# Mamo1031/Multimodal-MTRSSM

Measured on AMD Instinct MI355X. Metric: seq-steps/s (BxT) MoPoE-MRSSM train step, higher is better.
Workload: dtype bf16x2-split, fp32 accumulate; 1 GPU; BASELINE configs[1]: MoPoE-MRSSM train step, B=64/GPU T=50 deter=200 stoch=30, vision 1x64x64 + audio 1x128x32 + action 4; global_batch=64, seq_len=50, parallelism=dp1, hidden=200, embed=256, categoricals_x_classes=6x5, residual_blocks=3, activation=ELU, optimizer=AdamW lr 1e-3 + clip 10 (fused HIP), params=4151600, streams=1, launch=eager (host enqueues every launch), backend=none, rccl_ranks=0, collective_ranks=0, noise=uniforms keyed by global batch row (parallel.GlobalRowNoise)

## Files before the change

include/mtrssm.h:

```cpp
#ifndef MTRSSM_H
#define MTRSSM_H

#include <stddef.h>
#include <stdint.h>

#ifdef __cplusplus
extern "C" {
#endif

#define MTRSSM_VERSION 100

#define MTRSSM_OK 0
#define MTRSSM_EINVAL (-1)
#define MTRSSM_ELAUNCH (-2)
#define MTRSSM_ELDS (-3)

#define MTRSSM_ACT_IDENTITY 0
#define MTRSSM_ACT_RELU 1
#define MTRSSM_ACT_ELU 2
#define MTRSSM_ACT_TANH 3

int mtrssm_version(void);
const char* mtrssm_last_error(void);
const char* mtrssm_last_kernel(void);
// ... 261 lines not shown
  float* d_lv;
  float* d_lph;
  float* d_lqh;
  const int32_t* modality;
} MtrssmMmtrssmBwdIO;

int mtrssm_mmtrssm_rollout_bwd(const MtrssmMmtrssmDims* dims, const MtrssmMmtrssmBwdWeights* w,
                               const MtrssmMmtrssmBwdIO* io, void* stream);

int mtrssm_mmtrssm_wide_supported(const MtrssmMmtrssmDims* dims, int32_t pieces);
int64_t mtrssm_mmtrssm_wide_workspace_bytes(const MtrssmMmtrssmDims* dims, int32_t pieces);
int64_t mtrssm_mmtrssm_wide_bwd_workspace_bytes(const MtrssmMmtrssmDims* dims, int32_t pieces);
int mtrssm_mmtrssm_rollout_fwd_wide(const MtrssmMmtrssmDims* dims, const MtrssmMmtrssmFwdWeights* w, const MtrssmMmtrssmFwdIO* io,
                                    int32_t pieces, void* workspace, int64_t workspace_bytes, void* stream);
int mtrssm_mmtrssm_rollout_bwd_wide(const MtrssmMmtrssmDims* dims, const MtrssmMmtrssmBwdWeights* w, const MtrssmMmtrssmBwdIO* io,
                                    int32_t pieces, void* workspace, int64_t workspace_bytes, void* stream);

typedef struct MtrssmConvGeom {
  int32_t N;
  int32_t C, Hs, Ws;
  int32_t C2;
  int32_t Cpad;
  int32_t KH, KW;
  int32_t SS, TS, OFFY, OFFX;
  int32_t Hq, Wq;
  int32_t OS, QY, QX;
  int32_t Ho, Wo;
  int32_t Cout, CoutPad;
  int32_t pre_act;
  int32_t act;
  int32_t mfma_split;
} MtrssmConvGeom;

int mtrssm_conv_gather_gemm(const MtrssmConvGeom* g, const float* src, const float* src2, const float* wp, const uint16_t* wq,
                            const float* bias, const float* actgrad_in, const float* add_in, float* out, void* stream);
int mtrssm_conv_gather_gemm_pair(const MtrssmConvGeom* ga, const float* srca, const float* src2a, const float* wpa, const uint16_t* wqa,
                                 const float* biasa, const float* actgrada, const float* adda, float* outa,
                                 const MtrssmConvGeom* gb, const float* srcb, const float* src2b, const float* wpb, const uint16_t* wqb,
                                 const float* biasb, const float* actgradb, const float* addb, float* outb, void* stream);
int mtrssm_conv_gather_pair_merges(const MtrssmConvGeom* ga, const MtrssmConvGeom* gb, int32_t has_wq);
int mtrssm_residual_block_fwd_supported(const MtrssmConvGeom* g3);
int mtrssm_residual_block_fwd(const MtrssmConvGeom* ga, const float* xa, const uint16_t* wq3a, const float* b3a, const float* w1a,
                              const float* b1a, float* ha, float* ya, const MtrssmConvGeom* gb, const float* xb, const uint16_t* wq3b,
                              const float* b3b, const float* w1b, const float* b1b, float* hb, float* yb, void* stream);
int mtrssm_pack_conv_weight(const float* w, int32_t O, int32_t I, int32_t KH, int32_t KW, int64_t so, int64_t si, int64_t sh,
                            int64_t sw, int32_t OPad, int32_t IPad, int32_t pieces, float* wp, uint16_t* wq, void* stream);
#define MTRSSM_PACK_DESC_WORDS 16
int mtrssm_pack_conv_weights(const int64_t* table, int32_t count, int32_t blocks_per_weight, void* stream);
int mtrssm_conv_weight_grad(const MtrssmConvGeom* g, const float* a, const float* src, const float* src2,
                            int32_t pre_act_a, float* dwp, float* dbias, void* workspace, int64_t workspace_bytes, void* stream);
int mtrssm_conv_weight_grad_deferred(const MtrssmConvGeom* g, const float* a, const float* src, const float* src2,
                                     int32_t pre_act_a, float* dwp, float* dbias, void* workspace, int64_t workspace_bytes, void* stream);
int mtrssm_conv_weight_grad_reduce(void* stream);
int64_t mtrssm_conv_weight_grad_workspace_bytes(const MtrssmConvGeom* g, int32_t pre_act_a);
int mtrssm_unpack_conv_grads(const int64_t* table, int32_t count, int32_t blocks_per_entry, void* stream);
int mtrssm_convt_quad_supported(const MtrssmConvGeom* g4);
int mtrssm_convt_quad(const MtrssmConvGeom* ga4, const float* srca, const uint16_t* const* wqa4, const float* biasa, const float* actgrada,
                      float* outa, const MtrssmConvGeom* gb4, const float* srcb, const uint16_t* const* wqb4, const float* biasb,
                      const float* actgradb, float* outb, void* stream);
int mtrssm_convt_k4s2_thin(int32_t N, int32_t C, int32_t Hs, int32_t Ws, int32_t Cout, const float* src, const float* w,
                           const float* bias, int32_t pre_act, int32_t act, float* out, void* stream);
int mtrssm_convt_k4s2_band_supported(int32_t N, int32_t C, int32_t Hs, int32_t Ws, int32_t Cout);
int mtrssm_convt_k4s2_band(int32_t N, int32_t C, int32_t Hs, int32_t Ws, int32_t Cout, const float* src, const float* w,
                           const float* bias, int32_t pre_act, int32_t act, float* out, void* stream);
int mtrssm_conv_tgather_thin(int32_t N, int32_t O, int32_t Hs, int32_t Ws, int32_t Cout, int32_t KH, int32_t KW, int32_t stride, int32_t pad,
                             int32_t Ho, int32_t Wo, const float* y, const float* w, const float* bias, int32_t pre_act, int32_t act,
                             const float* actgrad_in, const float* add_in, float* out, void* stream);
int mtrssm_channel_sum(const float* x, int32_t N, int32_t C, int32_t HW, float* out, void* stream);

int mtrssm_episode_gather(const float* store, const int64_t* idx, const float* noise, int64_t n_episodes, int64_t B, int64_t T,
                          int64_t Tfull, int64_t E, float std_, float* input, float* target, void* stream);
int mtrssm_episode_gather_window(const float* store, const int64_t* idx, const int32_t* start, const float* noise, int64_t n_episodes,
                                 int64_t B, int64_t T, int64_t Tfull, int64_t E, float std_, float* input, float* target, void* stream);

#define MTRSSM_STATE_MAX 6
typedef struct MtrssmStateTable {
  int32_t count;
  int32_t width[MTRSSM_STATE_MAX];
  int64_t src_stride[MTRSSM_STATE_MAX];
  const float* src[MTRSSM_STATE_MAX];
  const float* alt[MTRSSM_STATE_MAX];
  float* dst[MTRSSM_STATE_MAX];
} MtrssmStateTable;
int mtrssm_state_select(const MtrssmStateTable* table, const uint8_t* reset, int64_t B, void* stream);
int mtrssm_state_save(const MtrssmStateTable* table, int64_t B, int64_t steps, void* stream);

int mtrssm_elbo_combine_fwd(const float* nll_a, const float* nll_v, const float* kl0, const float* kl1, int64_t n, float c0, float c1,
                            float* o_recon, float* o_k0, float* o_k1, float* o_loss, void* stream);
int mtrssm_elbo_combine_bwd(const float* g_recon, const float* g_k0, const float* g_k1, const float* g_loss, int64_t n, float c0, float c1,
                            float* g_nll_a, float* g_nll_v, float* g_kl0, float* g_kl1, void* stream);
int mtrssm_categorical_sample_fwd(const float* logits, const float* u, int64_t rows, int32_t K, int32_t C, float* logp, float* probs,
                                  float* onehot, void* stream);
int mtrssm_categorical_sample_bwd(const float* probs, const float* g_probs, const float* g_logp, int64_t rows, int32_t K, int32_t C,
                                  float* d_logits, void* stream);
int mtrssm_gaussian_nll_fwd(const float* pred, const float* target, int64_t frames, int64_t event, int32_t act,
                            float* out, void* stream);
int mtrssm_gaussian_nll_bwd(const float* pred, const float* target, const float* g_out,
                            int64_t frames, int64_t event, int32_t act, float* g_pred, void* stream);

int mtrssm_gaussian_nll_masked_fwd(const float* pred, const float* target, const float* present, const float* count,
                                   int64_t frames, int64_t event, int32_t act, float* out, void* stream);
int mtrssm_gaussian_nll_masked_bwd(const float* pred, const float* target, const float* present, const float* count,
                                   const float* g_out, int64_t frames, int64_t event, int32_t act, float* g_pred, void* stream);

int mtrssm_modality_dropout(const float* u, int64_t b_global, int64_t steps, int64_t span, float p_audio, float p_vision,
                            int64_t row0, int64_t b_local, int32_t* codes, float* present_audio, float* present_vision,
// ... 34 lines not shown
```

multimodal_mtrssm_amd/_lib.py:

```python

from __future__ import annotations

import ctypes as C
import os
from pathlib import Path

import torch
from torch import Tensor

_HERE = Path(__file__).resolve().parent
LIB_PATH = _HERE / "libmtrssm_hip.so"

ACT_IDS = {"Identity": 0, "ReLU": 1, "ELU": 2, "Tanh": 3}

_f = C.c_float
_i = C.c_int32
_p = C.c_void_p


def _struct(name: str, fields: list[tuple[str, type]]) -> type:
    return type(name, (C.Structure,), {"_fields_": fields})


def _ptrs(*names: str) -> list[tuple[str, type]]:
# ... 39 lines not shown
    "sv_l1", "sv_h1", "sv_la", "sv_lv",
    "g_deter_l", "g_deter_h", "g_hidden_l", "g_hidden_h", "g_post_stoch_l", "g_post_stoch_h", "g_prior_stoch_l",
    "g_prior_stoch_h", "g_post_logits_l", "g_post_logits_h", "g_prior_logits_l", "g_prior_logits_h", "g_kl_l", "g_kl_h",
    "g_deter_l0", "g_deter_h0", "g_hidden_l0", "g_hidden_h0", "g_stoch_l0", "g_stoch_h0",
    "d_ul", "d_uh", "d_zl1", "d_zh1", "d_lpl", "d_la", "d_lv", "d_lph", "d_lqh", "modality"))

ConvGeom = _struct("MtrssmConvGeom", [(n, _i) for n in (
    "N", "C", "Hs", "Ws", "C2", "Cpad", "KH", "KW", "SS", "TS", "OFFY", "OFFX", "Hq", "Wq", "OS", "QY", "QX", "Ho", "Wo",
    "Cout", "CoutPad", "pre_act", "act", "mfma_split")])

Gemm = _struct("MtrssmGemm", _ptrs("A", "B", "C", "bias", "zgrad", "colsum") + [(n, _i) for n in (
    "M", "N", "R", "lda", "ldb", "ldc", "ldz", "a_rmajor", "b_rmajor", "act_a", "act_b", "act_out", "act_z", "accumulate", "split_r")]
    + [("tickets", _p), ("n_tickets", _i), ("mfma_split", _i)])

STATE_MAX = 6
StateTable = _struct("MtrssmStateTable", [
    ("count", _i), ("width", _i * STATE_MAX), ("src_stride", C.c_int64 * STATE_MAX), ("src", _p * STATE_MAX), ("alt", _p * STATE_MAX),
    ("dst", _p * STATE_MAX)])

SYMBOLS: dict[str, tuple[type | None, list[type]]] = {
    "mtrssm_version": (C.c_int, []),
    "mtrssm_last_error": (C.c_char_p, []),
    "mtrssm_last_kernel": (C.c_char_p, []),
    "mtrssm_mrssm_rollout_fwd": (C.c_int, [C.POINTER(MrssmDims), C.POINTER(MrssmFwdWeights), C.POINTER(MrssmFwdIO), _p]),
    "mtrssm_mrssm_cluster_supported": (C.c_int, [C.POINTER(MrssmDims)]),
    "mtrssm_mrssm_cluster_workspace_bytes": (C.c_int64, [C.POINTER(MrssmDims)]),
    "mtrssm_mrssm_rollout_fwd_cluster": (C.c_int, [C.POINTER(MrssmDims), C.POINTER(MrssmClusterWeights), C.POINTER(MrssmFwdIO), _p, C.c_int64, _p]),
    "mtrssm_mrssm_cluster_bwd_workspace_bytes": (C.c_int64, [C.POINTER(MrssmDims)]),
    "mtrssm_mrssm_rollout_bwd_cluster": (C.c_int, [C.POINTER(MrssmDims), C.POINTER(MrssmClusterWeights), C.POINTER(MrssmBwdIO), _p, C.c_int64, _p]),
    "mtrssm_mrssm_wide_supported": (C.c_int, [C.POINTER(MrssmDims), _i]),
    "mtrssm_mrssm_wide_workspace_bytes": (C.c_int64, [C.POINTER(MrssmDims), _i]),
    "mtrssm_mrssm_wide_bwd_workspace_bytes": (C.c_int64, [C.POINTER(MrssmDims), _i]),
    "mtrssm_mrssm_rollout_fwd_wide": (C.c_int, [C.POINTER(MrssmDims), C.POINTER(MrssmClusterWeights), C.POINTER(MrssmFwdIO), _i, _p, C.c_int64, _p]),
    "mtrssm_mrssm_rollout_bwd_wide": (C.c_int, [C.POINTER(MrssmDims), C.POINTER(MrssmClusterWeights), C.POINTER(MrssmBwdIO), _i, _p, C.c_int64, _p]),
    "mtrssm_mrssm_rollout_bwd": (C.c_int, [C.POINTER(MrssmDims), C.POINTER(MrssmBwdWeights), C.POINTER(MrssmBwdIO), _p]),
    "mtrssm_mmtrssm_rollout_fwd": (C.c_int, [C.POINTER(MmtrssmDims), C.POINTER(MmtrssmFwdWeights), C.POINTER(MmtrssmFwdIO), _p]),
    "mtrssm_mmtrssm_rollout_bwd": (C.c_int, [C.POINTER(MmtrssmDims), C.POINTER(MmtrssmBwdWeights), C.POINTER(MmtrssmBwdIO), _p]),
    "mtrssm_mmtrssm_wide_supported": (C.c_int, [C.POINTER(MmtrssmDims), _i]),
    "mtrssm_mmtrssm_wide_workspace_bytes": (C.c_int64, [C.POINTER(MmtrssmDims), _i]),
    "mtrssm_mmtrssm_wide_bwd_workspace_bytes": (C.c_int64, [C.POINTER(MmtrssmDims), _i]),
    "mtrssm_mmtrssm_rollout_fwd_wide": (C.c_int, [C.POINTER(MmtrssmDims), C.POINTER(MmtrssmFwdWeights), C.POINTER(MmtrssmFwdIO), _i, _p, C.c_int64, _p]),
    "mtrssm_mmtrssm_rollout_bwd_wide": (C.c_int, [C.POINTER(MmtrssmDims), C.POINTER(MmtrssmBwdWeights), C.POINTER(MmtrssmBwdIO), _i, _p, C.c_int64, _p]),
    "mtrssm_conv_gather_gemm": (C.c_int, [C.POINTER(ConvGeom), _p, _p, _p, _p, _p, _p, _p, _p, _p]),
    "mtrssm_conv_gather_gemm_pair": (C.c_int, [C.POINTER(ConvGeom), _p, _p, _p, _p, _p, _p, _p, _p,
                                               C.POINTER(ConvGeom), _p, _p, _p, _p, _p, _p, _p, _p, _p]),
    "mtrssm_conv_gather_pair_merges": (C.c_int, [C.POINTER(ConvGeom), C.POINTER(ConvGeom), _i]),
    "mtrssm_residual_block_fwd_supported": (C.c_int, [C.POINTER(ConvGeom)]),
    "mtrssm_residual_block_fwd": (C.c_int, [C.POINTER(ConvGeom), _p, _p, _p, _p, _p, _p, _p, C.POINTER(ConvGeom), _p, _p, _p, _p, _p, _p, _p, _p]),
    "mtrssm_pack_conv_weight": (C.c_int, [_p, _i, _i, _i, _i, C.c_int64, C.c_int64, C.c_int64, C.c_int64, _i, _i, _i, _p, _p, _p]),
    "mtrssm_pack_conv_weights": (C.c_int, [_p, _i, _i, _p]),
    "mtrssm_unpack_conv_grads": (C.c_int, [_p, _i, _i, _p]),
    "mtrssm_conv_weight_grad": (C.c_int, [C.POINTER(ConvGeom), _p, _p, _p, _i, _p, _p, _p, C.c_int64, _p]),
    "mtrssm_conv_weight_grad_deferred": (C.c_int, [C.POINTER(ConvGeom), _p, _p, _p, _i, _p, _p, _p, C.c_int64, _p]),
    "mtrssm_conv_weight_grad_reduce": (C.c_int, [_p]),
    "mtrssm_conv_weight_grad_workspace_bytes": (C.c_int64, [C.POINTER(ConvGeom), _i]),
    "mtrssm_channel_sum": (C.c_int, [_p, _i, _i, _i, _p, _p]),
    "mtrssm_convt_k4s2_thin": (C.c_int, [_i, _i, _i, _i, _i, _p, _p, _p, _i, _i, _p, _p]),
    "mtrssm_convt_k4s2_band_supported": (C.c_int, [_i, _i, _i, _i, _i]),
    "mtrssm_convt_k4s2_band": (C.c_int, [_i, _i, _i, _i, _i, _p, _p, _p, _i, _i, _p, _p]),
    "mtrssm_convt_quad_supported": (C.c_int, [C.POINTER(ConvGeom)]),
    "mtrssm_convt_quad": (C.c_int, [C.POINTER(ConvGeom), _p, C.POINTER(C.c_void_p), _p, _p, _p, C.POINTER(ConvGeom), _p, C.POINTER(C.c_void_p),
                                    _p, _p, _p, _p]),
    "mtrssm_conv_tgather_thin": (C.c_int, [_i] * 11 + [_p, _p, _p, _i, _i, _p, _p, _p, _p]),
    "mtrssm_episode_gather": (C.c_int, [_p, _p, _p, C.c_int64, C.c_int64, C.c_int64, C.c_int64, C.c_int64, _f, _p, _p, _p]),
    "mtrssm_episode_gather_window": (C.c_int, [_p, _p, _p, _p, C.c_int64, C.c_int64, C.c_int64, C.c_int64, C.c_int64, _f, _p, _p, _p]),
    "mtrssm_state_select": (C.c_int, [C.POINTER(StateTable), _p, C.c_int64, _p]),
    "mtrssm_state_save": (C.c_int, [C.POINTER(StateTable), C.c_int64, C.c_int64, _p]),
    "mtrssm_elbo_combine_fwd": (C.c_int, [_p, _p, _p, _p, C.c_int64, C.c_float, C.c_float, _p, _p, _p, _p, _p]),
    "mtrssm_elbo_combine_bwd": (C.c_int, [_p, _p, _p, _p, C.c_int64, C.c_float, C.c_float, _p, _p, _p, _p, _p]),
    "mtrssm_categorical_sample_fwd": (C.c_int, [_p, _p, C.c_int64, _i, _i, _p, _p, _p, _p]),
    "mtrssm_categorical_sample_bwd": (C.c_int, [_p, _p, _p, C.c_int64, _i, _i, _p, _p]),
    "mtrssm_gaussian_nll_fwd": (C.c_int, [_p, _p, C.c_int64, C.c_int64, _i, _p, _p]),
    "mtrssm_gaussian_nll_bwd": (C.c_int, [_p, _p, _p, C.c_int64, C.c_int64, _i, _p, _p]),
    "mtrssm_gaussian_nll_masked_fwd": (C.c_int, [_p, _p, _p, _p, C.c_int64, C.c_int64, _i, _p, _p]),
    "mtrssm_gaussian_nll_masked_bwd": (C.c_int, [_p, _p, _p, _p, _p, C.c_int64, C.c_int64, _i, _p, _p]),
    "mtrssm_modality_dropout": (C.c_int, [_p, C.c_int64, C.c_int64, C.c_int64, _f, _f, C.c_int64, C.c_int64, _p, _p, _p, _p, _p, _p]),
    "mtrssm_sumsq": (C.c_int, [_p, C.c_int64, _p, _p]),
    "mtrssm_adamw_step": (C.c_int, [_p, _p, _p, _p, C.c_int64, _p, _f, _f, _f, _f, _f, _f, _f, _i, _p]),
    "mtrssm_gemm": (C.c_int, [C.POINTER(Gemm), _p]),
    "mtrssm_gemm_group": (C.c_int, [C.POINTER(Gemm), _i, _p]),
    "mtrssm_clear": (C.c_int, [_p, C.c_int64, _p]),
    "mtrssm_adamw_prepare": (C.c_int, [_p, C.c_int64, _p, _p, _p, _f, _f, _p]),
    "mtrssm_adamw_apply": (C.c_int, [_p, _p, _p, _p, _p, C.c_int64, _p, _p, _p, _f, _f, _f, _f, _f, _f, _p]),
}

_LIB: C.CDLL | None = None


class MtrssmLibraryError(RuntimeError):
    """The HIP library is missing or a kernel call failed.  There is no fallback path."""


def load() -> C.CDLL:
    global _LIB
    if _LIB is not None:
        return _LIB
    path = Path(os.environ.get("MTRSSM_LIB", LIB_PATH))
    if not path.exists():
        msg = (f"{path} not found: build it with `make -C multimodal_mtrssm_amd/csrc` (or __graft_entry__.build()). "
               "multimodal_mtrssm_amd has no CPU or eager fallback for the rollout path.")
        raise MtrssmLibraryError(msg)
    lib = C.CDLL(str(path))
    for name, (res, args) in SYMBOLS.items():
        fn = getattr(lib, name)
        fn.restype = res
        fn.argtypes = args
# ... 99 lines not shown
```

multimodal_mtrssm_amd/conv.py:

```python

from __future__ import annotations

import ctypes as C
import os
import weakref

import torch
from torch import Tensor

from multimodal_mtrssm_amd import _lib
from multimodal_mtrssm_amd.linear import grad_target, grad_target_owner


def _pad_to(n: int, m: int) -> int:
    return (n + m - 1) // m * m


def _pads(cout: int, cin: int) -> tuple[int, int]:
    return _pad_to(cout, 64 if cout > 32 else 32), _pad_to(cin, 16)


_PACK_BUFFERS: dict[tuple, tuple[Tensor, Tensor | None]] = {}

PAIR_LAUNCH = os.environ.get("MTRSSM_PAIR_LAUNCH", "1") != "0"
# ... 413 lines not shown
        _PLAN.pinned += 1


def unpin_scratch() -> None:
    _PLAN.pinned = max(0, _PLAN.pinned - 1)


_WGRAD_WS: dict[tuple, Tensor] = {}
_WGRAD_WS_RETIRED: list[Tensor] = []
_WGRAD_NEED: dict[tuple, int] = {}


DEFER_WGRAD_REDUCE = os.environ.get("MTRSSM_DEFER_WGRAD_REDUCE", "1") != "0"
_WGRAD_SLOTS: dict[tuple, list[Tensor]] = {}
_WGRAD_SLOT_NEXT: dict[tuple, int] = {}


def _reduce_deferred() -> None:
    for (device, stream), used in list(_WGRAD_SLOT_NEXT.items()):
        if used:
            _WGRAD_SLOT_NEXT[(device, stream)] = 0
            _lib.check(_lib.TIMERS.call("mtrssm_conv_weight_grad_reduce", _lib.load().mtrssm_conv_weight_grad_reduce, C.c_void_p(stream)),
                       "mtrssm_conv_weight_grad_reduce")


def _wgrad_workspace(geom: C.Structure, pre_act_a: int, device: torch.device, *, own: bool = False) -> Tensor | None:
    gkey = (tuple(getattr(geom, n) for n, _ in geom._fields_), pre_act_a)
    need = _WGRAD_NEED.get(gkey)
    if need is None:
        need = _WGRAD_NEED[gkey] = max(0, int(_lib.load().mtrssm_conv_weight_grad_workspace_bytes(C.byref(geom), pre_act_a)))
    if need == 0:
        return None
    key = (device, torch.cuda.current_stream(device).cuda_stream)
    if own:
        slots = _WGRAD_SLOTS.setdefault(key, [])
        k = _WGRAD_SLOT_NEXT.get(key, 0)
        _WGRAD_SLOT_NEXT[key] = k + 1
        if k == len(slots):
            slots.append(torch.empty((need + 3) // 4 + 64, device=device, dtype=torch.float32))
        elif slots[k].numel() * 4 < need:
            _WGRAD_WS_RETIRED.append(slots[k])
            slots[k] = torch.empty((need + 3) // 4 + 64, device=device, dtype=torch.float32)
        return slots[k]
    ws = _WGRAD_WS.get(key)
    if ws is None or ws.numel() * 4 < need:
        if ws is not None:
            _WGRAD_WS_RETIRED.append(ws)
        ws = _WGRAD_WS[key] = torch.empty((need + 3) // 4 + 64, device=device, dtype=torch.float32)
    return ws


def _weight_grad(a: Tensor, src: Tensor, coords: Tensor | None, kh: int, kw: int, stride: int, pad: int, pre_act_a: bool,
                 pre_act_src: bool, act: int, *, want_bias: bool = False, weight: Tensor | None = None,
                 bias: Tensor | None = None) -> tuple[Tensor | None, Tensor | None]:
    lib = _lib.load()
    n, o, hq, wq = a.shape
    _, c, hs, ws = src.shape
    c2 = 0 if coords is None else coords.shape[0]
    opad, ipad = _pads(o, c + c2)
    sunk = _GRAD_SINK.target(weight, o, c + c2, kh * kw, opad, ipad)
    dwp = sunk if sunk is not None else _zeros(opad * kh * kw * ipad, a.device).view(opad, kh * kw, ipad)
    dbias = bias_sunk = None
    if want_bias:
        bias_sunk = grad_target(bias) if bias is not None and bias.is_contiguous() else None
        dbias = bias_sunk if bias_sunk is not None else _zeros(o, a.device)
    geom = _geom(N=n, C=c, Hs=hs, Ws=ws, C2=c2, Cpad=ipad, KH=kh, KW=kw, SS=stride, TS=1, OFFY=-pad, OFFX=-pad, Hq=hq, Wq=wq,
                 OS=1, QY=0, QX=0, Ho=hq, Wo=wq, Cout=o, CoutPad=opad, pre_act=int(pre_act_src), act=act)
    flops = 2.0 * n * hq * wq * o * kh * kw * (c + c2)
    nbytes = 4.0 * (a.numel() + src.numel())
    defer = DEFER_WGRAD_REDUCE and sunk is not None and (not want_bias or bias_sunk is not None)
    ws = _wgrad_workspace(geom, int(pre_act_a), a.device, own=defer)
    entry = lib.mtrssm_conv_weight_grad_deferred if defer and ws is not None else lib.mtrssm_conv_weight_grad
    _lib.check(_lib.TIMERS.call(
        "mtrssm_conv_weight_grad", entry, C.byref(geom), _lib.ptr(a), _lib.ptr(src), _lib.ptr(coords),
        int(pre_act_a), _lib.ptr(dwp), _lib.ptr(dbias), _lib.raw_ptr(ws), 0 if ws is None else ws.numel() * 4, _lib.stream_ptr(a.device),
        flops=flops, nbytes=nbytes), "mtrssm_conv_weight_grad")
    g_w = None if sunk is not None else dwp[:o, :, : c + c2].reshape(o, kh, kw, c + c2).permute(0, 3, 1, 2)
    return g_w, (None if bias_sunk is not None else dbias)


def _channel_sum(x: Tensor, bias: Tensor | None = None) -> Tensor | None:
    lib = _lib.load()
    n, c, h, w = x.shape
    sunk = grad_target(bias) if bias is not None and bias.is_contiguous() else None
    out = sunk if sunk is not None else _zeros(c, x.device)
    _lib.check(_lib.TIMERS.call("mtrssm_channel_sum", lib.mtrssm_channel_sum, _lib.ptr(x), n, c, h * w, _lib.ptr(out),
                                _lib.stream_ptr(x.device)), "mtrssm_channel_sum")
    return None if sunk is not None else out


class _Conv2d(torch.autograd.Function):
    @staticmethod
    def forward(ctx, x, weight, bias, coords, stride, pad, pre_act, act):
        x, weight = x.contiguous(), weight.contiguous()
        bias = None if bias is None else bias.contiguous()
        coords = None if coords is None else coords.contiguous()
        out = _conv_forward_gather(x, coords, weight, bias, stride, pad, pre_act, act)
        ctx.save_for_backward(x, weight, coords if coords is not None else x.new_zeros(0))
        ctx.cfg = (stride, pad, pre_act, act, coords is not None, bias is not None)
        ctx.bias = bias
        return out

    @staticmethod
    def backward(ctx, g_out):
        x, weight, coords = ctx.saved_tensors
        stride, pad, pre_act, act, has_coords, has_bias = ctx.cfg
        coords = coords if has_coords else None
        g_out = g_out.contiguous()
        kh, kw = weight.shape[2:]
        c = x.shape[1]
        g_x = None
        if ctx.needs_input_grad[0]:
            g_x = _conv_transposed_gather(g_out, weight[:, :c], None, stride, pad, (x.shape[2], x.shape[3]), False, act,
                                          actgrad_in=x if pre_act else None)
        g_w = g_b = None
        want_b = has_bias and ctx.needs_input_grad[2]
        if ctx.needs_input_grad[1]:
            g_w, g_b = _weight_grad(g_out, x, coords, kh, kw, stride, pad, False, pre_act, act, want_bias=want_b, weight=weight,
                                    bias=ctx.bias)
        elif want_b:
            g_b = _channel_sum(g_out, ctx.bias)
        return g_x, g_w, g_b, None, None, None, None, None


class _ConvTranspose2d(torch.autograd.Function):
    @staticmethod
    def forward(ctx, x, weight, bias, stride, pad, out_pad, pre_act, act):
        x, weight = x.contiguous(), weight.contiguous()
        bias = None if bias is None else bias.contiguous()
        kh, kw = weight.shape[2:]
        ho = (x.shape[2] - 1) * stride - 2 * pad + kh + out_pad
        wo = (x.shape[3] - 1) * stride - 2 * pad + kw + out_pad
        out = _conv_transposed_gather(x, weight, bias, stride, pad, (ho, wo), pre_act, act)
        ctx.save_for_backward(x, weight)
        ctx.cfg = (stride, pad, pre_act, act, bias is not None)
        ctx.bias = bias
        return out

    @staticmethod
    def backward(ctx, g_out):
        x, weight = ctx.saved_tensors
        stride, pad, pre_act, act, has_bias = ctx.cfg
        g_out = g_out.contiguous()
        kh, kw = weight.shape[2:]
        g_x = None
        if ctx.needs_input_grad[0]:
            g_x = _conv_forward_gather(g_out, None, weight, None, stride, pad, False, act, actgrad_in=x if pre_act else None)
        g_w = None
        if ctx.needs_input_grad[1]:
            g_w, _ = _weight_grad(x, g_out, None, kh, kw, stride, pad, pre_act, False, act, weight=weight)
        g_b = _channel_sum(g_out, ctx.bias) if has_bias and ctx.needs_input_grad[2] else None
        return g_x, g_w, g_b, None, None, None, None, None


RESBLOCK_FUSE = True


def _residual_job(x: Tensor, w3: Tensor, b3: Tensor, w1: Tensor, b1: Tensor, act: int, sub: int = 0) -> tuple | None:
    if not RESBLOCK_FUSE or w3.shape[2:] != (3, 3) or w1.shape[2:] != (1, 1) or w1.shape[:2] != (x.shape[1], w3.shape[0]):
        return None
    n, c, hs, ws = x.shape
    o = w3.shape[0]
    wp, wq = pack_weight(w3, sub)
    if wq is None:
        return None
    geom = _geom(N=n, C=c, Hs=hs, Ws=ws, C2=0, Cpad=wp.shape[2], KH=3, KW=3, SS=1, TS=1, OFFY=-1, OFFX=-1, Hq=hs, Wq=ws, OS=1, QY=0,
                 QX=0, Ho=hs, Wo=ws, Cout=o, CoutPad=wp.shape[0], pre_act=1, act=act)
    if not _lib.load().mtrssm_residual_block_fwd_supported(C.byref(geom)):
        return None
    h = torch.empty(n, o, hs, ws, device=x.device, dtype=torch.float32)
    return (geom, x, wq, b3, w1, b1, h, torch.empty_like(x))


def _residual_launch(ja: tuple, jb: tuple | None) -> None:
    def work(job: tuple) -> tuple[float, float]:
        g = job[0]
        pixels = g.N * g.Hq * g.Wq
        return 2.0 * pixels * g.Cout * (9 * g.C + g.C), 4.0 * pixels * (2 * g.C + g.Cout)

    def args(job: tuple | None) -> tuple:
        if job is None:
            return (None,) * 8
        geom, x, wq, b3, w1, b1, h, y = job
        return (C.byref(geom), _lib.ptr(x), _lib.raw_ptr(wq), _lib.ptr(b3), _lib.ptr(w1), _lib.ptr(b1), _lib.ptr(h), _lib.ptr(y))

    fa, ba = work(ja)
    fb, bb = work(jb) if jb is not None else (0.0, 0.0)
    lib = _lib.load()
    _lib.check(_lib.TIMERS.call("mtrssm_residual_block_fwd", lib.mtrssm_residual_block_fwd, *args(ja), *args(jb),
                                _lib.stream_ptr(ja[1].device), flops=fa + fb, nbytes=ba + bb), "mtrssm_residual_block_fwd")


class _ResidualBlock(torch.autograd.Function):

    @staticmethod
    def forward(ctx, x, w3, b3, w1, b1, act):
        x, w3, b3, w1, b1 = (t.contiguous() for t in (x, w3, b3, w1, b1))
        p3, p1 = w3.shape[2] // 2, w1.shape[2] // 2
        job = _residual_job(x, w3, b3, w1, b1, act)
        if job is not None:
            _residual_launch(job, None)
            h, y = job[6], job[7]
        else:
            h = _conv_forward_gather(x, None, w3, b3, 1, p3, True, act)
            y = _conv_forward_gather(h, None, w1, b1, 1, p1, True, act, add_in=x)
        ctx.save_for_backward(x, h, w3, w1)
        ctx.act, ctx.biases = act, (b3, b1)
        return y

    @staticmethod
    def backward(ctx, g_y):
        x, h, w3, w1 = ctx.saved_tensors
        act = ctx.act
        g_y = g_y.contiguous()
        p3, p1 = w3.shape[2] // 2, w1.shape[2] // 2
        g_h = _conv_transposed_gather(g_y, w1, None, 1, p1, (h.shape[2], h.shape[3]), False, act, actgrad_in=h)
        b3, b1 = ctx.biases
        g_w1, g_b1 = _weight_grad(g_y, h, None, w1.shape[2], w1.shape[3], 1, p1, False, True, act, want_bias=True, weight=w1, bias=b1)
        g_x = None
        if ctx.needs_input_grad[0]:
            g_x = _conv_transposed_gather(g_h, w3, None, 1, p3, (x.shape[2], x.shape[3]), False, act, actgrad_in=x, add_in=g_y)
        g_w3, g_b3 = _weight_grad(g_h, x, None, w3.shape[2], w3.shape[3], 1, p3, False, True, act, want_bias=True, weight=w3, bias=b3)
        return g_x, g_w3, g_b3, g_w1, g_b1, None


class _PairResidualBlock(torch.autograd.Function):

    @staticmethod
    def forward(ctx, xa, w3a, b3a, w1a, b1a, xv, w3v, b3v, w1v, b1v, act):
        xa, w3a, b3a, w1a, b1a, xv, w3v, b3v, w1v, b1v = (t.contiguous() for t in (xa, w3a, b3a, w1a, b1a, xv, w3v, b3v, w1v, b1v))
        p3, p1 = w3a.shape[2] // 2, w1a.shape[2] // 2
        ja = _residual_job(xa, w3a, b3a, w1a, b1a, act)
        jv = _residual_job(xv, w3v, b3v, w1v, b1v, act, sub=1) if ja is not None else None
        if ja is not None and jv is not None:
            _residual_launch(ja, jv)
            ha, ya, hv, yv = ja[6], ja[7], jv[6], jv[7]
        else:
            ha, hv = paired(lambda: _conv_forward_gather(xa, None, w3a, b3a, 1, p3, True, act),
                            lambda: _conv_forward_gather(xv, None, w3v, b3v, 1, p3, True, act))
            ya, yv = paired(lambda: _conv_forward_gather(ha, None, w1a, b1a, 1, p1, True, act, add_in=xa),
                            lambda: _conv_forward_gather(hv, None, w1v, b1v, 1, p1, True, act, add_in=xv))
        ctx.save_for_backward(xa, ha, w3a, w1a, xv, hv, w3v, w1v)
        ctx.act, ctx.biases = act, (b3a, b1a, b3v, b1v)
        return ya, yv

    @staticmethod
    def backward(ctx, g_ya, g_yv):
        xa, ha, w3a, w1a, xv, hv, w3v, w1v = ctx.saved_tensors
        act = ctx.act
        g_ya, g_yv = g_ya.contiguous(), g_yv.contiguous()
        p3, p1 = w3a.shape[2] // 2, w1a.shape[2] // 2
        g_ha, g_hv = paired(lambda: _conv_transposed_gather(g_ya, w1a, None, 1, p1, (ha.shape[2], ha.shape[3]), False, act, actgrad_in=ha),
                            lambda: _conv_transposed_gather(g_yv, w1v, None, 1, p1, (hv.shape[2], hv.shape[3]), False, act, actgrad_in=hv))
        b3a, b1a, b3v, b1v = ctx.biases
        g_w1a, g_b1a = _weight_grad(g_ya, ha, None, w1a.shape[2], w1a.shape[3], 1, p1, False, True, act, want_bias=True, weight=w1a, bias=b1a)
        g_w1v, g_b1v = _weight_grad(g_yv, hv, None, w1v.shape[2], w1v.shape[3], 1, p1, False, True, act, want_bias=True, weight=w1v, bias=b1v)
        g_xa, g_xv = paired(
            lambda: _conv_transposed_gather(g_ha, w3a, None, 1, p3, (xa.shape[2], xa.shape[3]), False, act, actgrad_in=xa, add_in=g_ya),
            lambda: _conv_transposed_gather(g_hv, w3v, None, 1, p3, (xv.shape[2], xv.shape[3]), False, act, actgrad_in=xv, add_in=g_yv))
        g_w3a, g_b3a = _weight_grad(g_ha, xa, None, w3a.shape[2], w3a.shape[3], 1, p3, False, True, act, want_bias=True, weight=w3a, bias=b3a)
        g_w3v, g_b3v = _weight_grad(g_hv, xv, None, w3v.shape[2], w3v.shape[3], 1, p3, False, True, act, want_bias=True, weight=w3v, bias=b3v)
        return g_xa, g_w3a, g_b3a, g_w1a, g_b1a, g_xv, g_w3v, g_b3v, g_w1v, g_b1v, None


def residual_block_pair(xa: Tensor, pa: tuple[Tensor, Tensor, Tensor, Tensor], xv: Tensor, pv: tuple[Tensor, Tensor, Tensor, Tensor],
                        *, act: int) -> tuple[Tensor, Tensor]:
    return _PairResidualBlock.apply(xa, *pa, xv, *pv, int(act))


def residual_block(x: Tensor, w3: Tensor, b3: Tensor, w1: Tensor, b1: Tensor, *, act: int) -> Tensor:
    return _ResidualBlock.apply(x, w3, b3, w1, b1, int(act))


class _BranchCtx:

    def __init__(self, needs: tuple = ()) -> None:
        self.needs_input_grad = needs
        self.saved_tensors: tuple = ()
        self.cfg: tuple = ()

    def save_for_backward(self, *tensors: Tensor) -> None:
        self.saved_tensors = tensors


def _pair_function(base: type) -> type:

    class _Pair(torch.autograd.Function):
        @staticmethod
        def forward(ctx, n, *args):
            ca, cb = _BranchCtx(), _BranchCtx()
            ya, yb = paired(lambda: base.forward(ca, *args[:n]), lambda: base.forward(cb, *args[n:]))
            ctx.n, ctx.na, ctx.cfgs = n, len(ca.saved_tensors), (ca.cfg, cb.cfg)
            ctx.biases = (getattr(ca, "bias", None), getattr(cb, "bias", None))
            ctx.save_for_backward(*ca.saved_tensors, *cb.saved_tensors)
            return ya, yb

        @staticmethod
        def backward(ctx, ga, gb):
            saved, needs = ctx.saved_tensors, ctx.needs_input_grad[1:]
            ca, cb = _BranchCtx(needs[: ctx.n]), _BranchCtx(needs[ctx.n :])
            ca.saved_tensors, cb.saved_tensors = saved[: ctx.na], saved[ctx.na :]
            ca.cfg, cb.cfg = ctx.cfgs
            ca.bias, cb.bias = ctx.biases
            ra, rb = paired(lambda: base.backward(ca, ga), lambda: base.backward(cb, gb))
            return (None, *ra, *rb)

    _Pair.__name__ = f"_Pair{base.__name__}"
    return _Pair

# ... 26 lines not shown
```

multimodal_mtrssm_amd/csrc/capi.hip:

```cpp
#include <stdarg.h>
#include <stdio.h>

#include "scan_common.h"

namespace mtrssm {

static thread_local char g_err[512] = "";
static thread_local const char* g_kernel = "";

void set_last_kernel(const char* name) { g_kernel = name; }

void set_error(const char* fmt, ...) {
  va_list ap;
  va_start(ap, fmt);
  vsnprintf(g_err, sizeof(g_err), fmt, ap);
  va_end(ap);
}

int mrssm_fwd_launch(const MtrssmMrssmDims*, const MtrssmMrssmFwdWeights*, const MtrssmMrssmFwdIO*, hipStream_t);
int mrssm_bwd_launch(const MtrssmMrssmDims*, const MtrssmMrssmBwdWeights*, const MtrssmMrssmBwdIO*, hipStream_t);
int mmtrssm_fwd_launch(const MtrssmMmtrssmDims*, const MtrssmMmtrssmFwdWeights*, const MtrssmMmtrssmFwdIO*, hipStream_t);
int mmtrssm_bwd_launch(const MtrssmMmtrssmDims*, const MtrssmMmtrssmBwdWeights*, const MtrssmMmtrssmBwdIO*, hipStream_t);
int conv_gather_gemm_launch(const MtrssmConvGeom*, const float*, const float*, const float*, const unsigned short*, const float*, const float*, const float*, float*, hipStream_t);
int episode_gather_launch(const float*, const int64_t*, const float*, int64_t, int64_t, int64_t, int64_t, int64_t, float, float*, float*, hipStream_t);
int episode_gather_window_launch(const float*, const int64_t*, const int32_t*, const float*, int64_t, int64_t, int64_t, int64_t, int64_t, float, float*,
                                 float*, hipStream_t);
int state_select_launch(const MtrssmStateTable*, const unsigned char*, int64_t, hipStream_t);
int state_save_launch(const MtrssmStateTable*, int64_t, int64_t, hipStream_t);
int conv_gather_gemm_pair_launch(const MtrssmConvGeom*, const float*, const float*, const float*, const unsigned short*, const float*, const float*, const float*, float*,
                                 const MtrssmConvGeom*, const float*, const float*, const float*, const unsigned short*, const float*, const float*, const float*, float*, hipStream_t);
int conv_residual_fwd_supported(const MtrssmConvGeom*);
int conv_residual_fwd_launch(const MtrssmConvGeom*, const float*, const unsigned short*, const float*, const float*, const float*, float*, float*,
                             const MtrssmConvGeom*, const float*, const unsigned short*, const float*, const float*, const float*, float*, float*, hipStream_t);
int pack_conv_weight_launch(const float*, int, int, int, int, long, long, long, long, int, int, int, float*, unsigned short*, hipStream_t);
int pack_conv_weights_launch(const int64_t*, int, int, hipStream_t);
int conv_gather_pair_merges(const MtrssmConvGeom*, const MtrssmConvGeom*, bool);
int conv_weight_grad_launch(const MtrssmConvGeom*, const float*, const float*, const float*, int, float*, float*, void*, size_t, size_t*, hipStream_t);
int conv_weight_grad_deferred_launch(const MtrssmConvGeom*, const float*, const float*, const float*, int, float*, float*, void*, size_t, hipStream_t);
int conv_weight_grad_reduce_flush(hipStream_t);
int channel_sum_launch(const float*, int, int, int, float*, hipStream_t);
int convt_k4s2_band_supported(int, int, int, int, int);
int convt_k4s2_band_launch(int, int, int, int, int, const float*, const float*, const float*, int, int, float*, hipStream_t);
int convt_k4s2_thin_launch(int, int, int, int, int, const float*, const float*, const float*, int, int, float*, hipStream_t);
int conv_convt_quad_supported(const MtrssmConvGeom*);
int conv_convt_quad_launch(const MtrssmConvGeom*, const float*, const unsigned short* const*, const float*, const float*, float*,
                           const MtrssmConvGeom*, const float*, const unsigned short* const*, const float*, const float*, float*, hipStream_t);
int conv_tgather_thin_launch(int, int, int, int, int, int, int, int, int, int, int, const float*, const float*, const float*, int, int, const float*,
                             const float*, float*, hipStream_t);
int categorical_sample_fwd_launch(const float*, const float*, int64_t, int, int, float*, float*, float*, hipStream_t);
int categorical_sample_bwd_launch(const float*, const float*, const float*, int64_t, int, int, float*, hipStream_t);
int elbo_combine_fwd_launch(const float*, const float*, const float*, const float*, int64_t, float, float, float*, float*, float*, float*, hipStream_t);
int elbo_combine_bwd_launch(const float*, const float*, const float*, const float*, int64_t, float, float, float*, float*, float*, float*, hipStream_t);
int nll_fwd_launch(const float*, const float*, int64_t, int64_t, int, float*, hipStream_t);
int nll_bwd_launch(const float*, const float*, const float*, int64_t, int64_t, int, float*, hipStream_t);
int nll_masked_fwd_launch(const float*, const float*, const float*, const float*, int64_t, int64_t, int, float*, hipStream_t);
int nll_masked_bwd_launch(const float*, const float*, const float*, const float*, const float*, int64_t, int64_t, int, float*, hipStream_t);
int modality_dropout_launch(const float*, int64_t, int64_t, int64_t, float, float, int64_t, int64_t, int32_t*, float*, float*, unsigned char*, float*,
                            hipStream_t);
int sumsq_launch(const float*, int64_t, float*, hipStream_t);
int adamw_launch(float*, const float*, float*, float*, int64_t, const float*, float, float, float, float, float, float, float, int, hipStream_t);
int gemm_launch(const MtrssmGemm*, hipStream_t);
int gemm_group_launch(const MtrssmGemm*, int, hipStream_t);
int debug_set_cluster_profile(void*);
int debug_set_resident_profile(void*);
int debug_set_wide_profile(void*);
int debug_set_mmt_profile(void*);
int mrssm_cluster_supported(const MtrssmMrssmDims*);
size_t mrssm_cluster_workspace_bytes(const MtrssmMrssmDims*);
size_t mrssm_cluster_bwd_workspace_bytes(const MtrssmMrssmDims*);
int mrssm_bwd_cluster_launch(const MtrssmMrssmDims*, const MtrssmMrssmClusterWeights*, const MtrssmMrssmBwdIO*, void*, size_t, hipStream_t);
int mrssm_fwd_cluster_launch(const MtrssmMrssmDims*, const MtrssmMrssmClusterWeights*, const MtrssmMrssmFwdIO*, void*, size_t, hipStream_t);
int unpack_conv_grads_launch(const int64_t*, int, int, hipStream_t);
int mrssm_wide_supported(const MtrssmMrssmDims*, int);
size_t mrssm_wide_workspace_bytes(const MtrssmMrssmDims*, int);
size_t mrssm_wide_bwd_workspace_bytes(const MtrssmMrssmDims*, int);
int mrssm_wide_fwd_launch(const MtrssmMrssmDims*, const MtrssmMrssmClusterWeights*, const MtrssmMrssmFwdIO*, int, void*, size_t, hipStream_t);
int mrssm_wide_bwd_launch(const MtrssmMrssmDims*, const MtrssmMrssmClusterWeights*, const MtrssmMrssmBwdIO*, int, void*, size_t, hipStream_t);
int adamw_prepare_launch(const float*, int64_t, float*, float*, const int*, float, float, hipStream_t);
int adamw_apply_launch(float*, const float*, float*, float*, const unsigned char*, int64_t, const float*, const float*, const int*, float, float, float,
                       float, float, float, hipStream_t);

int mmtrssm_wide_supported(const MtrssmMmtrssmDims*, int);
size_t mmtrssm_wide_workspace_bytes(const MtrssmMmtrssmDims*, int);
size_t mmtrssm_wide_bwd_workspace_bytes(const MtrssmMmtrssmDims*, int);
int mmtrssm_wide_fwd_launch(const MtrssmMmtrssmDims*, const MtrssmMmtrssmFwdWeights*, const MtrssmMmtrssmFwdIO*, int, void*, size_t, hipStream_t);
int mmtrssm_wide_bwd_launch(const MtrssmMmtrssmDims*, const MtrssmMmtrssmBwdWeights*, const MtrssmMmtrssmBwdIO*, int, void*, size_t, hipStream_t);

int device_cu_count() {
  static int cached[64] = {0};
  int dev = 0;
  if (hipGetDevice(&dev) != hipSuccess) { (void)hipGetLastError(); return 0; }
  if (dev < 0 || dev >= 64) return 0;
// ... 133 lines not shown
                            weight_decay, static_cast<hipStream_t>(stream));
}
MTRSSM_API int mtrssm_conv_gather_gemm(const MtrssmConvGeom* g, const float* src, const float* src2, const float* wp, const uint16_t* wq,
                                       const float* bias, const float* actgrad_in, const float* add_in, float* out, void* stream) {
  return conv_gather_gemm_launch(g, src, src2, wp, wq, bias, actgrad_in, add_in, out, static_cast<hipStream_t>(stream));
}
MTRSSM_API int mtrssm_episode_gather(const float* store, const int64_t* idx, const float* noise, int64_t n_episodes, int64_t B, int64_t T,
                                     int64_t Tfull, int64_t E, float std_, float* input, float* target, void* stream) {
  return episode_gather_launch(store, idx, noise, n_episodes, B, T, Tfull, E, std_, input, target, static_cast<hipStream_t>(stream));
}
MTRSSM_API int mtrssm_episode_gather_window(const float* store, const int64_t* idx, const int32_t* start, const float* noise, int64_t n_episodes,
                                            int64_t B, int64_t T, int64_t Tfull, int64_t E, float std_, float* input, float* target, void* stream) {
  return episode_gather_window_launch(store, idx, start, noise, n_episodes, B, T, Tfull, E, std_, input, target, static_cast<hipStream_t>(stream));
}
MTRSSM_API int mtrssm_state_select(const MtrssmStateTable* table, const uint8_t* reset, int64_t B, void* stream) {
  return state_select_launch(table, reset, B, static_cast<hipStream_t>(stream));
}
MTRSSM_API int mtrssm_state_save(const MtrssmStateTable* table, int64_t B, int64_t steps, void* stream) {
  return state_save_launch(table, B, steps, static_cast<hipStream_t>(stream));
}
MTRSSM_API int mtrssm_conv_gather_gemm_pair(const MtrssmConvGeom* ga, const float* srca, const float* src2a, const float* wpa, const uint16_t* wqa,
                                            const float* biasa, const float* actgrada, const float* adda, float* outa,
                                            const MtrssmConvGeom* gb, const float* srcb, const float* src2b, const float* wpb, const uint16_t* wqb,
                                            const float* biasb, const float* actgradb, const float* addb, float* outb, void* stream) {
  return conv_gather_gemm_pair_launch(ga, srca, src2a, wpa, wqa, biasa, actgrada, adda, outa, gb, srcb, src2b, wpb, wqb, biasb, actgradb, addb,
                                      outb, static_cast<hipStream_t>(stream));
}
MTRSSM_API int mtrssm_residual_block_fwd_supported(const MtrssmConvGeom* g3) { return conv_residual_fwd_supported(g3) != 0; }
MTRSSM_API int mtrssm_residual_block_fwd(const MtrssmConvGeom* ga, const float* xa, const uint16_t* wq3a, const float* b3a, const float* w1a,
                                         const float* b1a, float* ha, float* ya, const MtrssmConvGeom* gb, const float* xb, const uint16_t* wq3b,
                                         const float* b3b, const float* w1b, const float* b1b, float* hb, float* yb, void* stream) {
  return conv_residual_fwd_launch(ga, xa, wq3a, b3a, w1a, b1a, ha, ya, gb, xb, wq3b, b3b, w1b, b1b, hb, yb, static_cast<hipStream_t>(stream));
}
MTRSSM_API int mtrssm_pack_conv_weight(const float* w, int32_t O, int32_t I, int32_t KH, int32_t KW, int64_t so, int64_t si, int64_t sh,
                                       int64_t sw, int32_t OPad, int32_t IPad, int32_t pieces, float* wp, uint16_t* wq, void* stream) {
  return pack_conv_weight_launch(w, O, I, KH, KW, so, si, sh, sw, OPad, IPad, pieces, wp, wq, static_cast<hipStream_t>(stream));
}
MTRSSM_API int mtrssm_conv_gather_pair_merges(const MtrssmConvGeom* ga, const MtrssmConvGeom* gb, int32_t has_wq) {
  return conv_gather_pair_merges(ga, gb, has_wq != 0);
}
MTRSSM_API int mtrssm_pack_conv_weights(const int64_t* table, int32_t count, int32_t blocks_per_weight, void* stream) {
  return pack_conv_weights_launch(table, count, blocks_per_weight, static_cast<hipStream_t>(stream));
}
MTRSSM_API int mtrssm_conv_weight_grad(const MtrssmConvGeom* g, const float* a, const float* src, const float* src2, int32_t pre_act_a,
                                       float* dwp, float* dbias, void* workspace, int64_t workspace_bytes, void* stream) {
  return conv_weight_grad_launch(g, a, src, src2, pre_act_a, dwp, dbias, workspace, workspace_bytes < 0 ? 0 : (size_t)workspace_bytes, nullptr,
                                 static_cast<hipStream_t>(stream));
}
MTRSSM_API int mtrssm_conv_weight_grad_deferred(const MtrssmConvGeom* g, const float* a, const float* src, const float* src2, int32_t pre_act_a,
                                               float* dwp, float* dbias, void* workspace, int64_t workspace_bytes, void* stream) {
  return conv_weight_grad_deferred_launch(g, a, src, src2, pre_act_a, dwp, dbias, workspace, workspace_bytes < 0 ? 0 : (size_t)workspace_bytes,
                                          static_cast<hipStream_t>(stream));
}
MTRSSM_API int mtrssm_conv_weight_grad_reduce(void* stream) { return conv_weight_grad_reduce_flush(static_cast<hipStream_t>(stream)); }
MTRSSM_API int64_t mtrssm_conv_weight_grad_workspace_bytes(const MtrssmConvGeom* g, int32_t pre_act_a) {
  size_t need = 0;
  if (conv_weight_grad_launch(g, nullptr, nullptr, nullptr, pre_act_a, nullptr, nullptr, nullptr, 0, &need, nullptr) != MTRSSM_OK) return -1;
  return (int64_t)need;
}
MTRSSM_API int mtrssm_channel_sum(const float* x, int32_t N, int32_t C, int32_t HW, float* out, void* stream) {
  return channel_sum_launch(x, N, C, HW, out, static_cast<hipStream_t>(stream));
}
MTRSSM_API int mtrssm_conv_tgather_thin(int32_t N, int32_t O, int32_t Hs, int32_t Ws, int32_t Cout, int32_t KH, int32_t KW, int32_t stride,
                                        int32_t pad, int32_t Ho, int32_t Wo, const float* y, const float* w, const float* bias, int32_t pre_act,
                                        int32_t act, const float* actgrad_in, const float* add_in, float* out, void* stream) {
  return conv_tgather_thin_launch(N, O, Hs, Ws, Cout, KH, KW, stride, pad, Ho, Wo, y, w, bias, pre_act, act, actgrad_in, add_in, out,
                                  static_cast<hipStream_t>(stream));
}
MTRSSM_API int mtrssm_convt_quad_supported(const MtrssmConvGeom* g4) { return conv_convt_quad_supported(g4); }
MTRSSM_API int mtrssm_convt_quad(const MtrssmConvGeom* ga4, const float* srca, const uint16_t* const* wqa4, const float* biasa,
                                 const float* actgrada, float* outa, const MtrssmConvGeom* gb4, const float* srcb,
                                 const uint16_t* const* wqb4, const float* biasb, const float* actgradb, float* outb, void* stream) {
  return conv_convt_quad_launch(ga4, srca, reinterpret_cast<const unsigned short* const*>(wqa4), biasa, actgrada, outa, gb4, srcb,
                                reinterpret_cast<const unsigned short* const*>(wqb4), biasb, actgradb, outb,
                                static_cast<hipStream_t>(stream));
}
MTRSSM_API int mtrssm_convt_k4s2_band_supported(int32_t N, int32_t C, int32_t Hs, int32_t Ws, int32_t Cout) {
  return convt_k4s2_band_supported(N, C, Hs, Ws, Cout);
}
MTRSSM_API int mtrssm_convt_k4s2_band(int32_t N, int32_t C, int32_t Hs, int32_t Ws, int32_t Cout, const float* src, const float* w,
                                     const float* bias, int32_t pre_act, int32_t act, float* out, void* stream) {
  return convt_k4s2_band_launch(N, C, Hs, Ws, Cout, src, w, bias, pre_act, act, out, static_cast<hipStream_t>(stream));
}
MTRSSM_API int mtrssm_convt_k4s2_thin(int32_t N, int32_t C, int32_t Hs, int32_t Ws, int32_t Cout, const float* src, const float* w,
                                      const float* bias, int32_t pre_act, int32_t act, float* out, void* stream) {
  return convt_k4s2_thin_launch(N, C, Hs, Ws, Cout, src, w, bias, pre_act, act, out, static_cast<hipStream_t>(stream));
}
```

multimodal_mtrssm_amd/csrc/conv.hip:

```cpp
#include <map>
#include <mutex>
#include <unordered_map>
#include <utility>

#include "scan_common.h"

namespace mtrssm {

void set_error(const char* fmt, ...);
void set_last_kernel(const char* name);

using f32x16 = __attribute__((ext_vector_type(16))) float;

constexpr int kKC = 16;
constexpr int kTP = 128;
constexpr int kConvThreads = 256;

__device__ __forceinline__ float act_grad_from_in(float x, int act) {
  switch (act) {
    case MTRSSM_ACT_RELU: return x > 0.f ? 1.f : 0.f;
    case MTRSSM_ACT_ELU: return x > 0.f ? 1.f : expf(x);
    case MTRSSM_ACT_TANH: { const float t = tanhf(x); return 1.f - t * t; }
    default: return 1.f;
  }
// ... 534 lines not shown
      const int n = (int)(pe / plane_q);
      const int rem = (int)(pe - (long)n * plane_q);
      const int oy = rem / g.Wq, ox = rem - oy * g.Wq;
      const size_t plane_o = (size_t)g.Ho * g.Wo;
      const size_t base = (size_t)n * g.Cout * plane_o + (size_t)(oy * g.OS + g.QY) * g.Wo + (ox * g.OS + g.QX);
#pragma unroll
      for (int j = 0; j < NT; ++j) {
#pragma unroll
        for (int r = 0; r < 16; ++r) {
          const int co = co0 + j * 32 + (r & 3) + 8 * (r >> 2) + 4 * kl;
          if (co < g.Cout) {
            float v = acc[i][j][r] + (bias ? bias[co] : 0.f);
            const size_t o = base + (size_t)co * plane_o;
            if (actgrad_in) v *= act_grad_from_in(actgrad_in[o], g.act);
            if (add_in) v += add_in[o];
            out[o] = v;
          }
        }
      }
    }
  }
}

}
#include "conv_split.h"
#include "conv_resident.h"
#include "conv_s2_band.h"
#include "conv_wgrad_resident.h"

namespace mtrssm {

static int launched(const char* who);
enum ReduceVariant { kRedRes64, kRedRes32, kRed1x1_64, kRed1x1_128, kRedThin, kRedThinT, kRedS2, kRedT4, kRedT4b, kRedS2c };
struct ReduceJob {
  const float4* part;
  float* dwp;
  float* dbias;
  int S, cpad, variant, gx, gy;
  __host__ int variant_gy() const { return gy; }
};
constexpr int kReduceBatchMax = 48;
struct ReduceBatch {
  int count;
  int first[kReduceBatchMax + 1];
  ReduceJob job[kReduceBatchMax];
};
__device__ __forceinline__ void wgrad_reduce_dispatch(const ReduceJob& j, int bx, int by) {
  switch (j.variant) {
    case kRedRes64: wgrad_reduce_partials_body<64>(j.part, j.S, j.cpad, j.dwp, j.dbias, bx, by); break;
    case kRedRes32: wgrad_reduce_partials_body<32>(j.part, j.S, j.cpad, j.dwp, j.dbias, bx, by); break;
    case kRed1x1_64: wgrad_reduce_partials1x1_body<64>(j.part, j.S, j.cpad, j.dwp, j.dbias, bx, by); break;
    case kRed1x1_128: wgrad_reduce_partials1x1_body<128>(j.part, j.S, j.cpad, j.dwp, j.dbias, bx, by); break;
    case kRedThin: wgrad_reduce_partials_thin_body(j.part, j.S, j.cpad, j.dwp, j.dbias, bx, by); break;
    case kRedThinT: wgrad_reduce_partials_thint_body(j.part, j.S, j.cpad, j.dwp, bx, by); break;
    case kRedS2: wgrad_reduce_partials_s2_body(j.part, j.S, j.cpad, j.dwp, j.dbias, bx, by); break;
    case kRedT4: wgrad_reduce_partials_t4_body(j.part, j.S, j.cpad, j.dwp, bx, by); break;
    case kRedT4b: wgrad_reduce_partials_t4b_body(j.part, j.S, j.cpad, j.dwp, bx, by); break;
    default: wgrad_reduce_partials_s2c_body(j.part, j.S, j.cpad, j.dwp, j.dbias, bx, by); break;
  }
}
__global__ __launch_bounds__(256) void wgrad_reduce_batch_kernel(const ReduceBatch b) {
  int j = 0;
  while (j + 1 < b.count && (int)blockIdx.x >= b.first[j + 1]) ++j;
  const int lb = (int)blockIdx.x - b.first[j], gx = b.job[j].gx;
  wgrad_reduce_dispatch(b.job[j], lb % gx, lb / gx);
}

static thread_local bool tl_defer_reduce = false;
static std::mutex g_reduce_mutex;
static std::map<std::pair<int, hipStream_t>, std::vector<ReduceJob>> g_reduce_jobs;
static std::pair<int, hipStream_t> reduce_key(hipStream_t stream) {
  int dev = 0;
  (void)hipGetDevice(&dev);
  return {dev, stream};
}

static int reduce_flush_locked(std::vector<ReduceJob>& jobs, hipStream_t stream) {
  size_t at = 0;
  while (at < jobs.size()) {
    ReduceBatch b{};
    int blocks = 0;
    while (at < jobs.size() && b.count < kReduceBatchMax) {
      b.first[b.count] = blocks;
      b.job[b.count] = jobs[at];
      blocks += jobs[at].gx * jobs[at].variant_gy();
      ++b.count;
      ++at;
    }
    b.first[b.count] = blocks;
    set_last_kernel("mtrssm::wgrad_reduce_batch_kernel");
    hipLaunchKernelGGL(wgrad_reduce_batch_kernel, dim3((unsigned)blocks), dim3(256), 0, stream, b);
  }
  jobs.clear();
  return launched("conv_weight_grad_reduce");
}

int conv_weight_grad_reduce_flush(hipStream_t stream) {
  std::lock_guard<std::mutex> lock(g_reduce_mutex);
  auto it = g_reduce_jobs.find(reduce_key(stream));
  if (it == g_reduce_jobs.end() || it->second.empty()) return MTRSSM_OK;
  return reduce_flush_locked(it->second, stream);
}

static int reduce_now_or_later(int variant, dim3 rgrid, const float* part, int S, int cpad, float* dwp, float* dbias, hipStream_t stream) {
  ReduceJob j{reinterpret_cast<const float4*>(part), dwp, dbias, S, cpad, variant, (int)rgrid.x, (int)rgrid.y};
  if (tl_defer_reduce) {
    std::lock_guard<std::mutex> lock(g_reduce_mutex);
    auto& jobs = g_reduce_jobs[reduce_key(stream)];
    for (const ReduceJob& o : jobs)
      if (o.dwp == dwp || o.part == j.part) {
// ... 1057 lines not shown
    GatherProblem p{};
    p.g = *g; p.src = x; p.wq = wq; p.bias = b3; p.out = h; p.w1 = w1; p.b1 = b1; p.out2 = y;
    p.nx = g->N;
    return p;
  };
  const GatherProblem pa = problem(ga, xa, wq3a, b3a, w1a, b1a, ha, ya);
  GatherProblem none{};
  none.nx = 0;
  if (!gb) return residual_fwd_one_grid(pa, none, ka, stream);
  const GatherProblem pb = problem(gb, xb, wq3b, b3b, w1b, b1b, hb, yb);
  if (ka == kb) return residual_fwd_one_grid(pa, pb, ka, stream);
  if (int rc = residual_fwd_one_grid(pa, none, ka, stream)) return rc;
  return residual_fwd_one_grid(pb, none, kb, stream);
}

int channel_sum_launch(const float* x, int N, int C, int HW, float* out, hipStream_t stream);

static bool wgrad_resident_enabled() {
  static const bool on = [] { const char* e = getenv("MTRSSM_WGRAD_RESIDENT"); return !(e && e[0] == '0'); }();
  return on;
}
static bool wgrad_resident_c32() {
  static const bool on = [] { const char* e = getenv("MTRSSM_WGRAD_RESIDENT_C32"); return !(e && e[0] == '0'); }();
  return on;
}
static bool wgrad_1x1_staged_enabled() {
  static const bool on = [] { const char* e = getenv("MTRSSM_WGRAD_1X1_STAGED"); return !(e && e[0] == '0'); }();
  return on;
}
static bool wgrad_s2_staged_enabled() {
  static const bool on = [] { const char* e = getenv("MTRSSM_WGRAD_S2_STAGED"); return !(e && e[0] == '0'); }();
  return on;
}
static bool wgrad_partials_enabled() {
  static const bool on = [] { const char* e = getenv("MTRSSM_WGRAD_PARTIALS"); return !(e && e[0] == '0'); }();
  return on;
}
#define MTRSSM_WGRAD_PART(bytes_expr)                                                                                              \
  float* part = nullptr;                                                                                                         \
  {                                                                                                                              \
    const size_t need_ = (bytes_expr);                                                                                           \
    if (query) { *query = wgrad_partials_enabled() ? need_ : 0; return MTRSSM_OK; }                                              \
    if (wgrad_partials_enabled() && workspace && workspace_bytes >= need_) part = static_cast<float*>(workspace);                \
  }
#define MTRSSM_WGRAD_NO_PART \
  if (query) { *query = 0; return MTRSSM_OK; }
static bool no_direct_wgrad() {
  static const bool off = getenv("MTRSSM_NO_DIRECT_WGRAD") != nullptr;
  return off;
}

int conv_weight_grad_launch(const MtrssmConvGeom* g, const float* a, const float* src, const float* src2, int pre_act_a,
                            float* dwp, float* dbias, void* workspace, size_t workspace_bytes, size_t* query, hipStream_t stream);
int conv_weight_grad_deferred_launch(const MtrssmConvGeom* g, const float* a, const float* src, const float* src2, int pre_act_a,
                                     float* dwp, float* dbias, void* workspace, size_t workspace_bytes, hipStream_t stream) {
  tl_defer_reduce = true;
  const int rc = conv_weight_grad_launch(g, a, src, src2, pre_act_a, dwp, dbias, workspace, workspace_bytes, nullptr, stream);
  tl_defer_reduce = false;
  return rc;
}

int conv_weight_grad_launch(const MtrssmConvGeom* g, const float* a, const float* src, const float* src2, int pre_act_a,
                            float* dwp, float* dbias, void* workspace, size_t workspace_bytes, size_t* query, hipStream_t stream) {
  if (int rc = check_geom(g, "conv_weight_grad")) return rc;
  if (!query && (!a || !src || !dwp || (g->C2 > 0 && !src2))) { set_error("conv_weight_grad: null pointer"); return MTRSSM_EINVAL; }
  if (workspace && ((uintptr_t)workspace & 255)) { set_error("conv_weight_grad: workspace must be 256-byte aligned"); return MTRSSM_EINVAL; }
  if (dbias && pre_act_a) { set_error("conv_weight_grad: the fused bias gradient sums the RAW a tensor; pass dbias only with pre_act_a = 0"); return MTRSSM_EINVAL; }
  if (g->OS != 1 || g->QY != 0 || g->QX != 0 || g->KH * g->KW <= 0) { set_error("conv_weight_grad: needs a plain (OS=1) geometry with taps"); return MTRSSM_EINVAL; }
  const long ptot = (long)g->N * g->Hq * g->Wq;
  const int taps = g->KH * g->KW;
  const int ctot = g->C + g->C2;
  if ((g->mfma_split == 1 || g->mfma_split == 2) && taps == 1 && g->SS == 1 && g->OFFY == 0 && g->OFFX == 0 && g->C2 == 0 && g->Hs == g->Hq &&
      g->Ws == g->Wq && g->Hq * g->Wq == 64 && (g->C == 64 || g->C == 128) && g->Cout % 64 == 0 && g->Cout <= 65535 * 64 && g->Cpad >= g->C &&
      !pre_act_a && (g->act == MTRSSM_ACT_IDENTITY || g->act == MTRSSM_ACT_ELU || g->act == MTRSSM_ACT_RELU) && !((uintptr_t)a & 15) &&
      !((uintptr_t)src & 15) && wgrad_1x1_staged_enabled()) {
    const int cogroups = g->Cout / 64;
    int wgs = cu_count() / cogroups;
    if (wgs < 1) wgs = 1;
    if (wgs > g->N) wgs = g->N;
    const int per = (g->N + wgs - 1) / wgs;
    const dim3 grid((unsigned)((g->N + per - 1) / per), cogroups);
    MTRSSM_WGRAD_PART((size_t)grid.x * cogroups * kWg1x1SetFloats * sizeof(float))
#define MTRSSM_WG1_LAUNCH(SP_, C_)                                                                                              \
  {                                                                                                                             \
    static bool attr_done_dev[64] = {}; bool& attr_done = attr_done_dev[device_slot()];        \
    constexpr int lds_b = wg1x1_lds_bytes<SP_, C_>();                                                                           \
    if (!attr_done) {                                                                                                           \
      (void)hipFuncSetAttribute(reinterpret_cast<const void*>(conv1x1_wgrad_staged_kernel<SP_, C_>),                            \
                                hipFuncAttributeMaxDynamicSharedMemorySize, lds_b);                                             \
      attr_done = true;                                                                                                         \
    }                                                                                                                           \
    set_last_kernel("mtrssm::conv1x1_wgrad_staged_kernel<" #SP_ ", " #C_ ">");                                                  \
    hipLaunchKernelGGL((conv1x1_wgrad_staged_kernel<SP_, C_>), grid, dim3(512), lds_b, stream, *g, a, src, dwp, part, dbias,    \
                       per);                                                                                                    \
  }
    const int sp = g->mfma_split;
    if (g->C == 64) { if (sp == 2) MTRSSM_WG1_LAUNCH(2, 64) else MTRSSM_WG1_LAUNCH(1, 64) }
    else { if (sp == 2) MTRSSM_WG1_LAUNCH(2, 128) else MTRSSM_WG1_LAUNCH(1, 128) }
#undef MTRSSM_WG1_LAUNCH
    if (part) {
      const dim3 rgrid((unsigned)(2 * (g->C / 32) * 256 / 32 + (dbias ? 1 : 0)), cogroups);
      if (int rc = reduce_now_or_later(g->C == 64 ? kRed1x1_64 : kRed1x1_128, rgrid, part, (int)grid.x, g->Cpad, dwp, dbias, stream)) return rc;
    }
    return launched("conv_weight_grad(1x1 staged)");
  }
  if (g->mfma_split >= 1 && taps == 1 && g->SS == 1 && g->OFFY == 0 && g->OFFX == 0 && g->C2 == 0 && g->Hs == g->Hq && g->Ws == g->Wq &&
      (g->Hq * g->Wq) % 16 == 0 && g->Cout <= 128 && g->C <= 128 && g->C >= 8 && !((uintptr_t)a & 15) && !((uintptr_t)src & 15) &&
      ptot < (1L << 31)) {
    MTRSSM_WGRAD_NO_PART
    const int tiles_co = (g->Cout + 31) / 32, tiles_ci = (g->C + 31) / 32;
    const int total = (int)(ptot / 16);
    int splits = 256;
    if (splits > total) splits = total;
    const int per = (total + splits - 1) / splits;
    const dim3 grid((unsigned)((total + per - 1) / per));
    const dim3 block(64 * tiles_co * tiles_ci);
// ... 58 lines not shown
    if (splits > total) splits = total;
    const int per = (total + splits - 1) / splits;
    const dim3 grid((unsigned)((total + per - 1) / per), cogroups);
    const dim3 block(64 * nt);
    const int sp = g->mfma_split;
#define MTRSSM_W33_LAUNCH(SP_, W_)                                                                                               \
  {                                                                                                                             \
    set_last_kernel("mtrssm::conv3x3_weight_grad_split_kernel<" #SP_ ", " #W_ ">");                                              \
    hipLaunchKernelGGL((conv3x3_weight_grad_split_kernel<SP_, W_>), grid, block, 0, stream, *g, a, src, pre_act_a, dwp, dbias, tiles_ci, per); \
  }
    if (g->Wq == 8) { if (sp == 3) MTRSSM_W33_LAUNCH(3, 8) else if (sp == 2) MTRSSM_W33_LAUNCH(2, 8) else MTRSSM_W33_LAUNCH(1, 8) }
    else { if (sp == 3) MTRSSM_W33_LAUNCH(3, 4) else if (sp == 2) MTRSSM_W33_LAUNCH(2, 4) else MTRSSM_W33_LAUNCH(1, 4) }
#undef MTRSSM_W33_LAUNCH
    return launched("conv_weight_grad(3x3 split)");
  }
  if ((g->mfma_split == 1 || g->mfma_split == 2) && g->KH == 3 && g->KW == 3 && g->SS == 2 && g->TS == 1 && g->OFFY == -1 && g->OFFX == -1 &&
      g->C == 1 && g->C2 == 2 && g->Cout == 8 && g->Hq * g->Wq == 1024 && (g->Wq == 32 || g->Wq == 16) && g->Hs == 2 * g->Hq && g->Ws == 2 * g->Wq &&
      g->Cpad >= 3 && !pre_act_a && (g->act == MTRSSM_ACT_IDENTITY || g->act == MTRSSM_ACT_ELU || g->act == MTRSSM_ACT_RELU || !g->pre_act) &&
      !((uintptr_t)a & 15) && !((uintptr_t)src & 15) && !((uintptr_t)src2 & 15) && wgrad_s2_staged_enabled()) {
    int wgs = cu_count();
    if (wgs > g->N) wgs = g->N;
    const int per = (g->N + wgs - 1) / wgs;
    const dim3 grid((unsigned)((g->N + per - 1) / per));
    MTRSSM_WGRAD_PART((size_t)grid.x * kWgThinSetFloats * sizeof(float))
#define MTRSSM_WGTHIN_LAUNCH(SP_, W_)                                                                                            \
  {                                                                                                                             \
    static bool attr_done_dev[64] = {}; bool& attr_done = attr_done_dev[device_slot()];        \
    constexpr int lds_b = wgthin_lds_bytes<SP_, W_>();                                                                          \
    if (!attr_done) {                                                                                                           \
      (void)hipFuncSetAttribute(reinterpret_cast<const void*>(conv3x3s2_thin_wgrad_staged_kernel<SP_, W_>),                      \
                                hipFuncAttributeMaxDynamicSharedMemorySize, lds_b);                                             \
      attr_done = true;                                                                                                         \
    }                                                                                                                           \
    set_last_kernel("mtrssm::conv3x3s2_thin_wgrad_staged_kernel<" #SP_ ", " #W_ ">");                                            \
    hipLaunchKernelGGL((conv3x3s2_thin_wgrad_staged_kernel<SP_, W_>), grid, dim3(512), lds_b, stream, *g, a, src, src2, dwp,     \
                       part, dbias, per);                                                                                       \
  }
    const int sp = g->mfma_split;
    if (g->Wq == 32) { if (sp == 2) MTRSSM_WGTHIN_LAUNCH(2, 32) else MTRSSM_WGTHIN_LAUNCH(1, 32) }
    else { if (sp == 2) MTRSSM_WGTHIN_LAUNCH(2, 16) else MTRSSM_WGTHIN_LAUNCH(1, 16) }
#undef MTRSSM_WGTHIN_LAUNCH
    if (part)
      if (int rc = reduce_now_or_later(kRedThin, dim3(dbias ? 9 : 8), part, (int)grid.x, g->Cpad, dwp, dbias, stream)) return rc;
    return launched("conv_weight_grad(3x3 s2 thin staged)");
  }
  if ((g->mfma_split == 1 || g->mfma_split == 2) && g->KH == 4 && g->KW == 4 && g->SS == 2 && g->TS == 1 && g->OFFY == -1 && g->OFFX == -1 &&
      g->C == 1 && g->C2 == 0 && g->Cout == 16 && g->Hq * g->Wq == 1024 && (g->Wq == 32 || g->Wq == 16) && g->Hs == 2 * g->Hq && g->Ws == 2 * g->Wq &&
      g->Cpad >= 1 && !g->pre_act && !dbias && (g->act == MTRSSM_ACT_IDENTITY || g->act == MTRSSM_ACT_ELU || g->act == MTRSSM_ACT_RELU || !pre_act_a) &&
      !((uintptr_t)a & 15) && !((uintptr_t)src & 15) && wgrad_s2_staged_enabled()) {
    int wgs = cu_count();
    if (wgs > g->N) wgs = g->N;
    const int per = (g->N + wgs - 1) / wgs;
    const dim3 grid((unsigned)((g->N + per - 1) / per));
    MTRSSM_WGRAD_PART((size_t)grid.x * kWgThinTSetFloats * sizeof(float))
#define MTRSSM_WGTHINT_LAUNCH(SP_, W_)                                                                                           \
  {                                                                                                                             \
    static bool attr_done_dev[64] = {}; bool& attr_done = attr_done_dev[device_slot()];        \
    constexpr int lds_b = wgthint_lds_bytes<SP_, W_>();                                                                         \
    if (!attr_done) {                                                                                                           \
      (void)hipFuncSetAttribute(reinterpret_cast<const void*>(convt4s2_thin_wgrad_staged_kernel<SP_, W_>),                       \
                                hipFuncAttributeMaxDynamicSharedMemorySize, lds_b);                                             \
      attr_done = true;                                                                                                         \
    }                                                                                                                           \
    set_last_kernel("mtrssm::convt4s2_thin_wgrad_staged_kernel<" #SP_ ", " #W_ ">");                                             \
    hipLaunchKernelGGL((convt4s2_thin_wgrad_staged_kernel<SP_, W_>), grid, dim3(512), lds_b, stream, *g, a, src, pre_act_a, dwp, \
                       part, per);                                                                                              \
  }
    const int sp = g->mfma_split;
    if (g->Wq == 32) { if (sp == 2) MTRSSM_WGTHINT_LAUNCH(2, 32) else MTRSSM_WGTHINT_LAUNCH(1, 32) }
    else { if (sp == 2) MTRSSM_WGTHINT_LAUNCH(2, 16) else MTRSSM_WGTHINT_LAUNCH(1, 16) }
#undef MTRSSM_WGTHINT_LAUNCH
    if (part)
      if (int rc = reduce_now_or_later(kRedThinT, dim3(16), part, (int)grid.x, g->Cpad, dwp, nullptr, stream)) return rc;
    return launched("conv_weight_grad(k4 s2 thin staged)");
  }
  if (g->mfma_split >= 1 && g->Cout <= 32 && taps * ctot <= 32 && g->Wq >= 8 && (g->Wq & (g->Wq - 1)) == 0 && (g->Hq * g->Wq) % 16 == 0 &&
      !((uintptr_t)a & 15) && ptot < (1L << 31) && (long)g->N * g->C * g->Hs * g->Ws < (1L << 40) && !no_direct_wgrad()) {
    MTRSSM_WGRAD_NO_PART
    int log2_wq = 0;
    while ((1 << log2_wq) < g->Wq) ++log2_wq;
    const int total = (int)(ptot / 16);
    int waves = 4096;
    if (waves > total) waves = total;
    const int per = (total + waves - 1) / waves;
    waves = (total + per - 1) / per;
    const dim3 grid((unsigned)((waves + 15) / 16));
    const int sp = g->mfma_split;
    set_last_kernel(sp == 3 ? "mtrssm::conv_weight_grad_thin_split_kernel<3>" : sp == 2 ? "mtrssm::conv_weight_grad_thin_split_kernel<2>" : "mtrssm::conv_weight_grad_thin_split_kernel<1>");
    if (sp == 3) hipLaunchKernelGGL((conv_weight_grad_thin_split_kernel<3>), grid, dim3(1024), 0, stream, *g, a, src, src2, pre_act_a, dwp, dbias, per, log2_wq);
    else if (sp == 2) hipLaunchKernelGGL((conv_weight_grad_thin_split_kernel<2>), grid, dim3(1024), 0, stream, *g, a, src, src2, pre_act_a, dwp, dbias, per, log2_wq);
    else hipLaunchKernelGGL((conv_weight_grad_thin_split_kernel<1>), grid, dim3(1024), 0, stream, *g, a, src, src2, pre_act_a, dwp, dbias, per, log2_wq);
    return launched("conv_weight_grad(thin split)");
  }
  if ((g->mfma_split == 1 || g->mfma_split == 2) && g->KH == 3 && g->KW == 3 && g->SS == 2 && g->TS == 1 && g->OFFY == -1 && g->OFFX == -1 &&
      g->C2 == 0 && g->C == 8 && g->Cout == 16 && g->Hq * g->Wq == 256 && (g->Wq == 16 || g->Wq == 8) && g->Hs == 2 * g->Hq && g->Ws == 2 * g->Wq &&
      g->Cpad >= 8 && !pre_act_a && (g->act == MTRSSM_ACT_IDENTITY || g->act == MTRSSM_ACT_ELU || g->act == MTRSSM_ACT_RELU) &&
      !((uintptr_t)a & 15) && !((uintptr_t)src & 15) && wgrad_s2_staged_enabled()) {
    int wgs = cu_count();
    if (wgs > g->N) wgs = g->N;
    const int per = (g->N + wgs - 1) / wgs;
    const dim3 grid((unsigned)((g->N + per - 1) / per));
    MTRSSM_WGRAD_PART((size_t)grid.x * kWgS2SetFloats * sizeof(float))
#define MTRSSM_WGS2_LAUNCH(SP_, W_)                                                                                              \
  {                                                                                                                             \
    static bool attr_done_dev[64] = {}; bool& attr_done = attr_done_dev[device_slot()];        \
    constexpr int lds_b = wgs2_lds_bytes<SP_, W_>();                                                                            \
    if (!attr_done) {                                                                                                           \
      (void)hipFuncSetAttribute(reinterpret_cast<const void*>(conv3x3s2_wgrad_staged_kernel<SP_, W_>),                           \
                                hipFuncAttributeMaxDynamicSharedMemorySize, lds_b);                                             \
      attr_done = true;                                                                                                         \
    }                                                                                                                           \
    set_last_kernel("mtrssm::conv3x3s2_wgrad_staged_kernel<" #SP_ ", " #W_ ">");                                                 \
    hipLaunchKernelGGL((conv3x3s2_wgrad_staged_kernel<SP_, W_>), grid, dim3(512), lds_b, stream, *g, a, src, dwp, part, dbias,   \
                       per);                                                                                                    \
  }
    const int sp = g->mfma_split;
    if (g->Wq == 16) { if (sp == 2) MTRSSM_WGS2_LAUNCH(2, 16) else MTRSSM_WGS2_LAUNCH(1, 16) }
    else { if (sp == 2) MTRSSM_WGS2_LAUNCH(2, 8) else MTRSSM_WGS2_LAUNCH(1, 8) }
#undef MTRSSM_WGS2_LAUNCH
    if (part)
      if (int rc = reduce_now_or_later(kRedS2, dim3(dbias ? 49 : 48), part, (int)grid.x, g->Cpad, dwp, dbias, stream)) return rc;
    return launched("conv_weight_grad(3x3 s2 staged)");
  }
  if ((g->mfma_split == 1 || g->mfma_split == 2) && g->KH == 4 && g->KW == 4 && g->SS == 2 && g->TS == 1 && g->OFFY == -1 && g->OFFX == -1 &&
      g->C2 == 0 && g->C == 16 && g->Cout == 32 && g->Hq * g->Wq == 256 && (g->Wq == 16 || g->Wq == 8) && g->Hs == 2 * g->Hq && g->Ws == 2 * g->Wq &&
      g->Cpad >= 16 && !g->pre_act && !dbias && (g->act == MTRSSM_ACT_IDENTITY || g->act == MTRSSM_ACT_ELU || g->act == MTRSSM_ACT_RELU || !pre_act_a) &&
      !((uintptr_t)a & 15) && !((uintptr_t)src & 15) && wgrad_s2_staged_enabled()) {
    int wgs = cu_count();
    if (wgs > g->N) wgs = g->N;
    const int per = (g->N + wgs - 1) / wgs;
    const dim3 grid((unsigned)((g->N + per - 1) / per));
    MTRSSM_WGRAD_PART((size_t)grid.x * kWgT4SetFloats * sizeof(float))
#define MTRSSM_WGT4_LAUNCH(SP_, W_)                                                                                              \
  {                                                                                                                             \
    static bool attr_done_dev[64] = {}; bool& attr_done = attr_done_dev[device_slot()];        \
    constexpr int lds_b = wgt4_lds_bytes<SP_, W_>();                                                                            \
    if (!attr_done) {                                                                                                           \
      (void)hipFuncSetAttribute(reinterpret_cast<const void*>(convt4s2_wgrad_staged_kernel<SP_, W_>),                            \
                                hipFuncAttributeMaxDynamicSharedMemorySize, lds_b);                                             \
      attr_done = true;                                                                                                         \
    }                                                                                                                           \
    set_last_kernel("mtrssm::convt4s2_wgrad_staged_kernel<" #SP_ ", " #W_ ">");                                                  \
    hipLaunchKernelGGL((convt4s2_wgrad_staged_kernel<SP_, W_>), grid, dim3(512), lds_b, stream, *g, a, src, pre_act_a, dwp,      \
                       part, per);                                                                                              \
  }
    const int sp = g->mfma_split;
    if (g->Wq == 16) { if (sp == 2) MTRSSM_WGT4_LAUNCH(2, 16) else MTRSSM_WGT4_LAUNCH(1, 16) }
    else { if (sp == 2) MTRSSM_WGT4_LAUNCH(2, 8) else MTRSSM_WGT4_LAUNCH(1, 8) }
#undef MTRSSM_WGT4_LAUNCH
    if (part)
      if (int rc = reduce_now_or_later(kRedT4, dim3(kWgT4SetFloats / 4 / 8), part, (int)grid.x, g->Cpad, dwp, nullptr, stream)) return rc;
    return launched("conv_weight_grad(k4 s2 staged)");
  }
  if ((g->mfma_split == 1 || g->mfma_split == 2) && g->KH == 4 && g->KW == 4 && g->SS == 2 && g->TS == 1 && g->OFFY == -1 && g->OFFX == -1 &&
      g->C2 == 0 && g->C == 32 && g->Cout == 64 && g->Hq * g->Wq == 64 && (g->Wq == 8 || g->Wq == 4) && g->Hs == 2 * g->Hq && g->Ws == 2 * g->Wq &&
      g->Cpad >= 32 && !g->pre_act && !dbias && (g->act == MTRSSM_ACT_IDENTITY || g->act == MTRSSM_ACT_ELU || g->act == MTRSSM_ACT_RELU || !pre_act_a) &&
      !((uintptr_t)a & 15) && !((uintptr_t)src & 15) && wgrad_s2_staged_enabled()) {
    int wgs = cu_count();
    if (wgs > g->N) wgs = g->N;
    const int per = (g->N + wgs - 1) / wgs;
    const dim3 grid((unsigned)((g->N + per - 1) / per));
    MTRSSM_WGRAD_PART((size_t)grid.x * kWgT4bSetFloats * sizeof(float))
#define MTRSSM_WGT4B_LAUNCH(SP_, W_)                                                                                             \
  {                                                                                                                             \
    static bool attr_done_dev[64] = {}; bool& attr_done = attr_done_dev[device_slot()];        \
    constexpr int lds_b = wgt4b_lds_bytes<SP_, W_>();                                                                           \
    if (!attr_done) {                                                                                                           \
      (void)hipFuncSetAttribute(reinterpret_cast<const void*>(convt4s2b_wgrad_staged_kernel<SP_, W_>),                           \
                                hipFuncAttributeMaxDynamicSharedMemorySize, lds_b);                                             \
      attr_done = true;                                                                                                         \
    }                                                                                                                           \
    set_last_kernel("mtrssm::convt4s2b_wgrad_staged_kernel<" #SP_ ", " #W_ ">");                                                 \
    hipLaunchKernelGGL((convt4s2b_wgrad_staged_kernel<SP_, W_>), grid, dim3(512), lds_b, stream, *g, a, src, pre_act_a, dwp,     \
                       part, per);                                                                                              \
  }
    const int sp = g->mfma_split;
    if (g->Wq == 8) { if (sp == 2) MTRSSM_WGT4B_LAUNCH(2, 8) else MTRSSM_WGT4B_LAUNCH(1, 8) }
    else { if (sp == 2) MTRSSM_WGT4B_LAUNCH(2, 4) else MTRSSM_WGT4B_LAUNCH(1, 4) }
#undef MTRSSM_WGT4B_LAUNCH
    if (part)
      if (int rc = reduce_now_or_later(kRedT4b, dim3(kWgT4bSetFloats / 4 / 8), part, (int)grid.x, g->Cpad, dwp, nullptr, stream)) return rc;
    return launched("conv_weight_grad(k4 s2 staged, 64 rows)");
  }
  if ((g->mfma_split == 1 || g->mfma_split == 2) && g->KH == 3 && g->KW == 3 && g->SS == 2 && g->TS == 1 && g->OFFY == -1 && g->OFFX == -1 &&
      g->C2 == 0 && g->C == 16 && g->Cout == 32 && g->Hq * g->Wq == 64 && (g->Wq == 8 || g->Wq == 4) && g->Hs == 2 * g->Hq && g->Ws == 2 * g->Wq &&
      g->Cpad >= 16 && !pre_act_a && (g->act == MTRSSM_ACT_IDENTITY || g->act == MTRSSM_ACT_ELU || g->act == MTRSSM_ACT_RELU) &&
      !((uintptr_t)a & 15) && !((uintptr_t)src & 15) && wgrad_s2_staged_enabled()) {
    int wgs = cu_count();
    if (wgs > g->N) wgs = g->N;
    const int per = (g->N + wgs - 1) / wgs;
    const dim3 grid((unsigned)((g->N + per - 1) / per));
    MTRSSM_WGRAD_PART((size_t)grid.x * kWgS2cSetFloats * sizeof(float))
#define MTRSSM_WGS2C_LAUNCH(SP_, W_)                                                                                             \
  {                                                                                                                             \
    set_last_kernel("mtrssm::conv3x3s2c_wgrad_staged_kernel<" #SP_ ", " #W_ ">");                                                \
    hipLaunchKernelGGL((conv3x3s2c_wgrad_staged_kernel<SP_, W_>), grid, dim3(512), wgs2c_lds_bytes<SP_>(), stream, *g, a, src,   \
                       dwp, part, dbias, per);                                                                                  \
  }
    const int sp = g->mfma_split;
    if (g->Wq == 8) { if (sp == 2) MTRSSM_WGS2C_LAUNCH(2, 8) else MTRSSM_WGS2C_LAUNCH(1, 8) }
    else { if (sp == 2) MTRSSM_WGS2C_LAUNCH(2, 4) else MTRSSM_WGS2C_LAUNCH(1, 4) }
#undef MTRSSM_WGS2C_LAUNCH
    if (part)
      if (int rc = reduce_now_or_later(kRedS2c, dim3(dbias ? 161 : 160), part, (int)grid.x, g->Cpad, dwp, dbias, stream)) return rc;
    return launched("conv_weight_grad(3x3 s2 staged, 16 -> 32)");
  }
  MTRSSM_WGRAD_NO_PART
  if (g->TS == 1 && g->Wq <= kGP && kGP % g->Wq == 0) {
    const PatchGeom pg(*g, kGP);
    const bool tiles = (g->Hq % pg.rpg == 0) || (pg.rpg % g->Hq == 0);
    const int nq = (taps * ctot + 31) / 32;
    const int tco = g->Cout > 32 ? 64 : 32;
    const size_t lds = (2 * ((size_t)tco * kLDA + (size_t)ctot * pg.ps) + kGP) * sizeof(float);
    const int n_out = g->Cout * taps * ctot;
    const size_t lds_thin = (2 * ((size_t)g->Cout * kLDA + (size_t)ctot * pg.ps) + kGP + ((pg.ps_raw + 63) & ~63)) * sizeof(float);
    const bool mfma_ok = nq <= 4 * kMaxQ && lds <= 150 * 1024;
    (void)mfma_ok;
    if (tiles && n_out <= kThinOut * kConvThreads && lds_thin <= 64 * 1024 && ptot < (1L << 31) && pg.ps_raw < 1024 && pg.ipg < 1024 &&
        !(g->mfma_split >= 1 && ctot >= 8 && (g->Hq * g->Wq) % 8 == 0)) {
      const long groups = (ptot + kGP - 1) / kGP;
      long splits = 2048;
      if (splits > groups) splits = groups;
      { set_last_kernel("mtrssm::conv_weight_grad_thin_kernel"); hipLaunchKernelGGL(conv_weight_grad_thin_kernel, dim3((unsigned)splits), dim3(kConvThreads), lds_thin, stream, *g, a, src, src2, pre_act_a, dwp, dbias); }
      return launched("conv_weight_grad(thin)");
    }
    if (tiles && g->mfma_split >= 1 && (g->Hq * g->Wq) % 8 == 0 && ctot <= 128 && !((uintptr_t)a & 15)) {
      const int sp = g->mfma_split;
      int cp2 = 16;
      while (cp2 < ctot) cp2 *= 2;
      const int nhalf = taps * (cp2 / 16);
      const int tco_s = g->Cout > 32 ? 64 : 32;
      const int nblk = (pg.ps_raw + 63) / 64;
      const size_t lds_1 = (size_t)sp * ((size_t)tco_s * kWgLdaB + (size_t)pg.ps_raw * cp2 * 2);
      const int nbuf = 2 * lds_1 + (size_t)nblk * 64 * sizeof(int) <= 156 * 1024 || nblk * (cp2 / 8) <= 16 ? 2 : 1;
// ... 265 lines not shown
```

multimodal_mtrssm_amd/csrc/conv_wgrad_resident.h:

```cpp
#pragma once

namespace mtrssm {

template <int W>
__host__ __device__ constexpr int wgres_pitch() { return (64 / W + 1) * 2 * W; }
constexpr int kWgresAPitch = 144;
template <int SPLIT, int C, int W>
__host__ __device__ constexpr int wgres_xbuf_bytes() { return SPLIT * C * wgres_pitch<W>() + 16; }
template <int SPLIT>
__host__ __device__ constexpr int wgres_abuf_bytes() { return SPLIT * 64 * kWgresAPitch; }
template <int SPLIT, int C, int W>
__host__ __device__ constexpr int wgres_lds_bytes() { return 2 * (wgres_xbuf_bytes<SPLIT, C, W>() + wgres_abuf_bytes<SPLIT>()); }
__host__ __device__ constexpr int wgres_tile_floats(int c) { return 2 * (c / 32) * 9 * 1024; }
__host__ __device__ constexpr int wgres_set_floats(int c) { return wgres_tile_floats(c) + 64; }
constexpr int kWg1x1SetFloats = 8 * 1024 + 64;

using wg_bf16x2 = __attribute__((ext_vector_type(2))) __bf16;
using wg_f32x2 = __attribute__((ext_vector_type(2))) float;
using wg_f32x4 = __attribute__((ext_vector_type(4))) float;
template <int SPLIT>
__device__ __forceinline__ void wg_split_pair(const float f0, const float f1, unsigned (&d)[SPLIT]) {
  d[0] = __builtin_bit_cast(unsigned, __builtin_convertvector(wg_f32x2{f0, f1}, wg_bf16x2));
  if constexpr (SPLIT >= 2) {
    const float r0 = f0 - __builtin_bit_cast(float, d[0] << 16), r1 = f1 - __builtin_bit_cast(float, d[0] & 0xffff0000u);
// ... 445 lines not shown
                                                                       float* __restrict__ dwp, float* __restrict__ dbias, const int bx, const int by) {
  constexpr int NTILE = 2 * (C / 32), KS = 8 / NTILE, TILE4 = 256, SET4 = kWg1x1SetFloats / 4;
  constexpr int NL = 32, NG = 8;
  __shared__ float4 red[NG][NL];
  const int li = threadIdx.x & (NL - 1), sg = threadIdx.x / NL;
  const int f = bx * NL + li;
  const bool bias = f >= NTILE * TILE4;
  const int tile = f / TILE4, ft = f - tile * TILE4;
  const float4* const p = part + (size_t)by * S * SET4 + (bias ? (size_t)(8 * TILE4 + (f - NTILE * TILE4 < 16 ? f - NTILE * TILE4 : 15)) : (size_t)tile * TILE4 + ft);
  float4 acc4[4];
#pragma unroll
  for (int u = 0; u < 4; ++u) acc4[u] = make_float4(0.f, 0.f, 0.f, 0.f);
  const int ks = bias ? 1 : KS;
  const int slices = S * ks;
  int i = sg;
  for (; i + 3 * NG < slices; i += 4 * NG) {
#pragma unroll
    for (int u = 0; u < 4; ++u) {
      const int ii = i + NG * u;
      const float4 v = p[(size_t)(ii / ks) * SET4 + (size_t)(ii % ks) * (NTILE * TILE4)];
      acc4[u].x += v.x; acc4[u].y += v.y; acc4[u].z += v.z; acc4[u].w += v.w;
    }
  }
  for (; i < slices; i += NG) {
    const float4 v = p[(size_t)(i / ks) * SET4 + (size_t)(i % ks) * (NTILE * TILE4)];
    acc4[0].x += v.x; acc4[0].y += v.y; acc4[0].z += v.z; acc4[0].w += v.w;
  }
  red[sg][li] = make_float4((acc4[0].x + acc4[1].x) + (acc4[2].x + acc4[3].x), (acc4[0].y + acc4[1].y) + (acc4[2].y + acc4[3].y),
                            (acc4[0].z + acc4[1].z) + (acc4[2].z + acc4[3].z), (acc4[0].w + acc4[1].w) + (acc4[2].w + acc4[3].w));
  __syncthreads();
  if (sg == 0) {
    float4 v = red[0][li];
#pragma unroll
    for (int k = 1; k < NG; ++k) { v.x += red[k][li].x; v.y += red[k][li].y; v.z += red[k][li].z; v.w += red[k][li].w; }
    if (bias) {
      if (f - NTILE * TILE4 < 16) {
        float* const o = dbias + by * 64 + 4 * (f - NTILE * TILE4);
        o[0] += v.x; o[1] += v.y; o[2] += v.z; o[3] += v.w;
      }
      return;
    }
    const int lane = ft & 63, gq = ft >> 6, il = lane & 31, kl = lane >> 5;
    const int tco = tile & 1, tci = tile >> 1;
    float* const o = dwp + (size_t)(by * 64 + tco * 32 + 8 * gq + 4 * kl) * cpad + tci * 32 + il;
    o[0] += v.x; o[cpad] += v.y; o[2 * (size_t)cpad] += v.z; o[3 * (size_t)cpad] += v.w;
  }
}
template <int C>
__global__ __launch_bounds__(256) void wgrad_reduce_partials1x1_kernel(const float4* __restrict__ part, const int S, const int cpad,
                                                                       float* __restrict__ dwp, float* __restrict__ dbias) {
  wgrad_reduce_partials1x1_body<C>(part, S, cpad, dwp, dbias, (int)blockIdx.x, (int)blockIdx.y);
}

constexpr int kWgS2SetFloats = 8 * 2 * 64 * 4 + 16;
template <int WO>
__host__ __device__ constexpr int wgs2_cip() { return (((256 / WO * 2 + 1) * (2 * WO)) / 16 | 1) * 16; }
template <int SPLIT, int WO>
__host__ __device__ constexpr int wgs2_lds_bytes() { return 2 * SPLIT * (2 * 8 * wgs2_cip<WO>() + 16 * 528); }

template <int SPLIT, int WO>
__global__ __launch_bounds__(512, 1) void conv3x3s2_wgrad_staged_kernel(
    const MtrssmConvGeom g, const float* __restrict__ a, const float* __restrict__ src, float* __restrict__ dwp,
    float* __restrict__ part, float* __restrict__ dbias, const int frames_per_wg) {
  static_assert(SPLIT == 1 || SPLIT == 2, "one or two bf16 pieces");
  static_assert(WO == 16 || WO == 8, "output plane 16x16 or 32x8");
  constexpr int NT = 512, C = 8, CO = 16, HO = 256 / WO, HS = 2 * HO, WS = 2 * WO;
  constexpr int ROWB = WS;
  constexpr int CIP = wgs2_cip<WO>();
  constexpr int XCOPY = C * CIP;
  constexpr int AP = 528, APB = CO * AP;
  constexpr int BUFB = SPLIT * (2 * XCOPY + APB);
  constexpr int XI = C * HS * WS / 4 / NT, AI = CO * 256 / 4 / NT, NI = XI + AI;
  extern __shared__ __attribute__((aligned(16))) unsigned char wgs2_lds[];
  unsigned char* const lds = wgs2_lds;
  const int tid = threadIdx.x, lane = tid & 63, wave = tid >> 6;
  const int il = lane & 31, kl = lane >> 5;
  const int ct = wave & 3, kh = wave >> 2;
  const int n0 = blockIdx.x * frames_per_wg;
  const int n1 = n0 + frames_per_wg < g.N ? n0 + frames_per_wg : g.N;
  if (n0 >= n1) return;
  const int nlast = n1 - 1;

  const bool act_elu = g.act == MTRSSM_ACT_ELU, act_relu = g.act == MTRSSM_ACT_RELU, pre = g.pre_act != 0;
  auto act_sel = [&](float x) __attribute__((always_inline)) {
    float e = __expf(x) - 1.f;
    asm volatile("" : "+v"(e));
    const float neg = act_elu ? e : (act_relu ? 0.f : x);
    return (x > 0.f || !pre) ? x : neg;
  };

  for (int o = tid * 16; o < 2 * BUFB; o += NT * 16) *reinterpret_cast<uint4*>(lds + o) = make_uint4(0u, 0u, 0u, 0u);

  const float4* const xsrc = reinterpret_cast<const float4*>(src) + tid;
  const float4* const asrc = reinterpret_cast<const float4*>(a) + tid;
  constexpr size_t xfr = (size_t)C * HS * WS / 4, afr = (size_t)CO * 256 / 4;
  float bsum[AI];
#pragma unroll
  for (int j = 0; j < AI; ++j) bsum[j] = 0.f;
  wg_f32x4 raw[3][NI];
  auto raw_load = [&](const int rs, const int n) __attribute__((always_inline)) {
#pragma unroll
    for (int it = 0; it < NI; ++it) {
      const float4* const ptr = it < AI ? asrc + (size_t)n * afr + NT * it : xsrc + (size_t)n * xfr + NT * (it - AI);
      asm volatile("global_load_dwordx4 %0, %1, off" : "=v"(raw[rs][it]) : "v"(ptr));
    }
  };
// ... 119 lines not shown
  __shared__ float4 red[NG][NL];
  const int li = threadIdx.x & (NL - 1), sg = threadIdx.x / NL;
  const int f = bx * NL + li;
  const bool bias = f >= 384;
  if (bias && f >= 388) {
    red[sg][li] = make_float4(0.f, 0.f, 0.f, 0.f);
  }
  const int ct = f >> 7, rem = f & 127;
  float4 acc4[2];
  acc4[0] = acc4[1] = make_float4(0.f, 0.f, 0.f, 0.f);
  if (!(bias && f >= 388)) {
    const int ks = bias ? 1 : 2;
    const int slices = S * ks;
    const float4* const p = part + (bias ? (size_t)(8 * 128 + (f - 384)) : (size_t)ct * 128 + rem);
    int i = sg;
    for (; i + NG < slices; i += 2 * NG) {
#pragma unroll
      for (int u = 0; u < 2; ++u) {
        const int ii = i + NG * u;
        const float4 v = p[(size_t)(ii / ks) * SET4 + (size_t)(ii % ks) * (4 * 128)];
        acc4[u].x += v.x; acc4[u].y += v.y; acc4[u].z += v.z; acc4[u].w += v.w;
      }
    }
    for (; i < slices; i += NG) {
      const float4 v = p[(size_t)(i / ks) * SET4 + (size_t)(i % ks) * (4 * 128)];
      acc4[0].x += v.x; acc4[0].y += v.y; acc4[0].z += v.z; acc4[0].w += v.w;
    }
    red[sg][li] = make_float4(acc4[0].x + acc4[1].x, acc4[0].y + acc4[1].y, acc4[0].z + acc4[1].z, acc4[0].w + acc4[1].w);
  }
  __syncthreads();
  if (sg == 0) {
    float4 v = red[0][li];
#pragma unroll
    for (int k = 1; k < NG; ++k) { v.x += red[k][li].x; v.y += red[k][li].y; v.z += red[k][li].z; v.w += red[k][li].w; }
    if (bias) {
      if (f < 388) { float* const o = dbias + 4 * (f - 384); o[0] += v.x; o[1] += v.y; o[2] += v.z; o[3] += v.w; }
      return;
    }
    const int half = rem >> 6, lane = rem & 63, il = lane & 31, kl = lane >> 5;
    const int col = ct * 32 + il;
    if (col < 72) {
      const int tap = col >> 3, ci = col & 7, row = 8 * half + 4 * kl;
      float* const o = dwp + ((size_t)row * 9 + tap) * cpad + ci;
      const size_t rs = (size_t)9 * cpad;
      o[0] += v.x; o[rs] += v.y; o[2 * rs] += v.z; o[3 * rs] += v.w;
    }
  }
}
__global__ __launch_bounds__(256) void wgrad_reduce_partials_s2_kernel(const float4* __restrict__ part, const int S, const int cpad,
                                                                       float* __restrict__ dwp, float* __restrict__ dbias) {
  wgrad_reduce_partials_s2_body(part, S, cpad, dwp, dbias, (int)blockIdx.x, (int)blockIdx.y);
}

constexpr int kWgT4SetFloats = 8 * 4 * 64 * 4;
template <int WO>
__host__ __device__ constexpr int wgt4_cip() { return (((256 / WO * 2 + 2) * (2 * WO)) / 16 | 1) * 16; }
template <int SPLIT, int WO>
__host__ __device__ constexpr int wgt4_lds_bytes() { return SPLIT * (2 * 16 * wgt4_cip<WO>() + 32 * 528); }

template <int SPLIT, int WO>
__global__ __launch_bounds__(512, 1) void convt4s2_wgrad_staged_kernel(
    const MtrssmConvGeom g, const float* __restrict__ a, const float* __restrict__ src, const int pre_act_a, float* __restrict__ dwp,
    float* __restrict__ part, const int frames_per_wg) {
  static_assert(SPLIT == 1 || SPLIT == 2, "one or two bf16 pieces");
  static_assert(WO == 16 || WO == 8, "input plane 16x16 or 32x8");
  constexpr int NT = 512, C = 16, CO = 32, HO = 256 / WO, HS = 2 * HO, WS = 2 * WO;
  constexpr int ROWB = WS;
  constexpr int CIP = wgt4_cip<WO>();
  constexpr int XCOPY = C * CIP;
  constexpr int AP = 528, APB = CO * AP;
  constexpr int XI = C * HS * WS / 4 / NT, AI = CO * 256 / 4 / NT, NI = XI + AI;
  extern __shared__ __attribute__((aligned(16))) unsigned char wgt4_lds[];
  unsigned char* const lds = wgt4_lds;
  const int tid = threadIdx.x, lane = tid & 63, wave = tid >> 6;
  const int il = lane & 31, kl = lane >> 5;
  const int n0 = blockIdx.x * frames_per_wg;
  const int n1 = n0 + frames_per_wg < g.N ? n0 + frames_per_wg : g.N;
  if (n0 >= n1) return;
  const int nlast = n1 - 1;

  const bool act_elu = g.act == MTRSSM_ACT_ELU, act_relu = g.act == MTRSSM_ACT_RELU, pre = pre_act_a != 0;
  auto act_sel = [&](float x) __attribute__((always_inline)) {
    float e = __expf(x) - 1.f;
    asm volatile("" : "+v"(e));
    const float neg = act_elu ? e : (act_relu ? 0.f : x);
    return (x > 0.f || !pre) ? x : neg;
  };

  for (int o = tid * 16; o < wgt4_lds_bytes<SPLIT, WO>(); o += NT * 16) *reinterpret_cast<uint4*>(lds + o) = make_uint4(0u, 0u, 0u, 0u);

  const float4* const xsrc = reinterpret_cast<const float4*>(src) + tid;
  const float4* const asrc = reinterpret_cast<const float4*>(a) + tid;
  constexpr size_t xfr = (size_t)C * HS * WS / 4, afr = (size_t)CO * 256 / 4;
  wg_f32x4 raw[3][NI];
  auto raw_load = [&](const int rs, const int n) __attribute__((always_inline)) {
#pragma unroll
    for (int it = 0; it < NI; ++it) {
      const float4* const ptr = it < AI ? asrc + (size_t)n * afr + NT * it : xsrc + (size_t)n * xfr + NT * (it - AI);
      asm volatile("global_load_dwordx4 %0, %1, off" : "=v"(raw[rs][it]) : "v"(ptr));
    }
  };
  auto raw_wait = [&](const int rs) __attribute__((always_inline)) {
    static_assert(NI == 12, "twelve items");
    asm volatile("s_waitcnt vmcnt(24)" : "+v"(raw[rs][0]), "+v"(raw[rs][1]), "+v"(raw[rs][2]), "+v"(raw[rs][3]), "+v"(raw[rs][4]), "+v"(raw[rs][5]),
                 "+v"(raw[rs][6]), "+v"(raw[rs][7]), "+v"(raw[rs][8]), "+v"(raw[rs][9]), "+v"(raw[rs][10]), "+v"(raw[rs][11]));
  };
  auto stage = [&](const int rs) __attribute__((always_inline)) {
#pragma unroll
    for (int it = 0; it < NI; ++it) {
      const wg_f32x4 v = raw[rs][it];
      if (it < AI) {
        unsigned d0[SPLIT], d1[SPLIT];
        wg_split_pair<SPLIT>(act_sel(v.x), act_sel(v.y), d0);
        wg_split_pair<SPLIT>(act_sel(v.z), act_sel(v.w), d1);
        const int f = tid + NT * it;
        const unsigned o = (unsigned)(SPLIT * 2 * XCOPY) + (unsigned)((f >> 6) * AP + (f & 63) * 8);
#pragma unroll
        for (int p = 0; p < SPLIT; ++p) *reinterpret_cast<uint2*>(lds + o + p * APB) = make_uint2(d0[p], d1[p]);
      } else {
        unsigned de[SPLIT], dd[SPLIT];
        wg_split_pair<SPLIT>(v.x, v.z, de);
        wg_split_pair<SPLIT>(v.y, v.w, dd);
        const int f = tid + NT * (it - AI);
        const int co = f / (HS * WS / 4), rem = f - co * (HS * WS / 4), row = rem / (WS / 4), c4 = rem - row * (WS / 4);
        const unsigned o = (unsigned)(co * CIP + (row + 1) * ROWB + c4 * 4);
#pragma unroll
        for (int p = 0; p < SPLIT; ++p) {
          *reinterpret_cast<unsigned*>(lds + o + p * 2 * XCOPY) = de[p];
          *reinterpret_cast<unsigned*>(lds + o + p * 2 * XCOPY + XCOPY) = dd[p];
        }
      }
    }
  };

  const int col = wave * 32 + il;
  const int tap = col >> 4, co = col & 15, ky = tap >> 2, kx = tap & 3;
  const bool odd = kx == 0 || kx == 2;
  const unsigned lane_b = (unsigned)((odd ? XCOPY : 0) + co * CIP + ky * ROWB + (WO == 16 ? kl * 16 : kl * 2 * ROWB));
  constexpr unsigned kStepB = WO == 16 ? 2 * ROWB : 4 * ROWB;
  const unsigned lane_a = (unsigned)(SPLIT * 2 * XCOPY + il * AP + kl * 16);
  f32x16 acc;
#pragma unroll
  for (int r = 0; r < 16; ++r) acc[r] = 0.f;

  raw_load(0, n0);
  raw_load(1, n0 + 1 < nlast ? n0 + 1 : nlast);
  auto frame = [&](const int n, const int rs) __attribute__((always_inline)) {
    raw_load((rs + 2) % 3, n + 2 < nlast ? n + 2 : nlast);
    raw_wait(rs);
    lds_barrier();
    stage(rs);
    lds_barrier();
#pragma unroll
    for (int s = 0; s < 16; ++s) {
      u32x4 qa[SPLIT], qb[SPLIT];
#pragma unroll
      for (int p = 0; p < SPLIT; ++p) {
        qa[p] = *reinterpret_cast<const u32x4*>(lds + lane_a + (unsigned)(p * APB) + (unsigned)(s * 32));
        const unsigned bo = lane_b + (unsigned)(p * 2 * XCOPY) + (unsigned)s * kStepB;
        const u32x4 f = *reinterpret_cast<const u32x4*>(lds + bo);
        unsigned prev = 0u, next = 0u;
        if (WO == 16) {
          prev = kl ? (unsigned)*reinterpret_cast<const unsigned short*>(lds + bo - 2) : 0u;
          next = kl ? 0u : (unsigned)*reinterpret_cast<const unsigned short*>(lds + bo + 16);
        }
        const u32x4 shr = u32x4{(f.x << 16) | prev, __builtin_amdgcn_alignbit(f.y, f.x, 16), __builtin_amdgcn_alignbit(f.z, f.y, 16), __builtin_amdgcn_alignbit(f.w, f.z, 16)};
        const u32x4 shl = u32x4{__builtin_amdgcn_alignbit(f.y, f.x, 16), __builtin_amdgcn_alignbit(f.z, f.y, 16), __builtin_amdgcn_alignbit(f.w, f.z, 16), (f.w >> 16) | (next << 16)};
        qb[p] = kx == 0 ? shr : (kx == 3 ? shl : f);
      }
#pragma unroll
      for (int ord = SPLIT - 1; ord >= 0; --ord)
#pragma unroll
        for (int sa = 0; sa <= ord; ++sa)
          acc = __builtin_amdgcn_mfma_f32_32x32x16_bf16(__builtin_bit_cast(bf16x8, qa[sa]), __builtin_bit_cast(bf16x8, qb[ord - sa]), acc, 0, 0, 0);
    }
  };
#pragma unroll 1
  for (int n = n0; n < n1; n += 3) {
    frame(n, 0);
    if (n + 1 < n1) frame(n + 1, 1);
    if (n + 2 < n1) frame(n + 2, 2);
  }
  asm volatile("s_waitcnt vmcnt(0)" ::: "memory");

  if (part) {
    float4* const ps = reinterpret_cast<float4*>(part) + (size_t)blockIdx.x * (kWgT4SetFloats / 4) + (size_t)wave * 256 + lane;
#pragma unroll
    for (int gq = 0; gq < 4; ++gq) ps[gq * 64] = make_float4(acc[4 * gq], acc[4 * gq + 1], acc[4 * gq + 2], acc[4 * gq + 3]);
  } else {
#pragma unroll
    for (int r = 0; r < 16; ++r) {
      const int row = (r & 3) + 8 * (r >> 2) + 4 * kl;
      atomicAdd(&dwp[((size_t)row * 16 + tap) * g.Cpad + co], acc[r]);
    }
  }
}

__device__ __forceinline__ void wgrad_reduce_partials_t4_body(const float4* __restrict__ part, const int S, const int cpad,
                                                                       float* __restrict__ dwp, const int bx, const int by) {
  constexpr int SET4 = kWgT4SetFloats / 4, NL = 8, NG = 32;
  __shared__ float4 red[NG][NL];
  const int li = threadIdx.x & (NL - 1), sg = threadIdx.x / NL;
  const int f = bx * NL + li;
  const float4* const p = part + f;
  float4 acc4[4];
#pragma unroll
  for (int u = 0; u < 4; ++u) acc4[u] = make_float4(0.f, 0.f, 0.f, 0.f);
  int s = sg;
  for (; s + 3 * NG < S; s += 4 * NG) {
#pragma unroll
    for (int u = 0; u < 4; ++u) {
      const float4 v = p[(size_t)(s + NG * u) * SET4];
      acc4[u].x += v.x; acc4[u].y += v.y; acc4[u].z += v.z; acc4[u].w += v.w;
    }
  }
  for (; s < S; s += NG) {
    const float4 v = p[(size_t)s * SET4];
    acc4[0].x += v.x; acc4[0].y += v.y; acc4[0].z += v.z; acc4[0].w += v.w;
  }
  red[sg][li] = make_float4((acc4[0].x + acc4[1].x) + (acc4[2].x + acc4[3].x), (acc4[0].y + acc4[1].y) + (acc4[2].y + acc4[3].y),
                            (acc4[0].z + acc4[1].z) + (acc4[2].z + acc4[3].z), (acc4[0].w + acc4[1].w) + (acc4[2].w + acc4[3].w));
  __syncthreads();
  if (sg == 0) {
    float4 v = red[0][li];
#pragma unroll
    for (int k = 1; k < NG; ++k) { v.x += red[k][li].x; v.y += red[k][li].y; v.z += red[k][li].z; v.w += red[k][li].w; }
    const int lane = f & 63, gq = (f >> 6) & 3, wave = f >> 8, il = lane & 31, kl = lane >> 5;
    const int col = wave * 32 + il, tap = col >> 4, co = col & 15, row = 8 * gq + 4 * kl;
    float* const o = dwp + ((size_t)row * 16 + tap) * cpad + co;
    const size_t rs = (size_t)16 * cpad;
    o[0] += v.x; o[rs] += v.y; o[2 * rs] += v.z; o[3 * rs] += v.w;
  }
}
__global__ __launch_bounds__(256) void wgrad_reduce_partials_t4_kernel(const float4* __restrict__ part, const int S, const int cpad,
                                                                       float* __restrict__ dwp) {
  wgrad_reduce_partials_t4_body(part, S, cpad, dwp, (int)blockIdx.x, (int)blockIdx.y);
}

constexpr int kWgT4bSetFloats = 8 * 4 * 4 * 64 * 4;
template <int WO>
__host__ __device__ constexpr int wgt4b_cip() { return (((64 / WO * 2 + 2) * (2 * WO)) / 16 | 1) * 16; }
template <int SPLIT, int WO>
__host__ __device__ constexpr int wgt4b_lds_bytes() { return SPLIT * (2 * 32 * wgt4b_cip<WO>() + 64 * kWgresAPitch); }

template <int SPLIT, int WO>
__global__ __launch_bounds__(512, 1) void convt4s2b_wgrad_staged_kernel(
    const MtrssmConvGeom g, const float* __restrict__ a, const float* __restrict__ src, const int pre_act_a, float* __restrict__ dwp,
    float* __restrict__ part, const int frames_per_wg) {
  static_assert(SPLIT == 1 || SPLIT == 2, "one or two bf16 pieces");
  static_assert(WO == 8 || WO == 4, "input plane 8x8 or 16x4");
  constexpr int NT = 512, C = 32, CO = 64, HO = 64 / WO, HS = 2 * HO, WS = 2 * WO;
  constexpr int ROWB = WS;
  constexpr int CIP = wgt4b_cip<WO>();
  constexpr int XCOPY = C * CIP;
  constexpr int AP = kWgresAPitch, APB = CO * AP;
  constexpr int XI = C * HS * WS / 4 / NT, AI = CO * 64 / 4 / NT, NI = XI + AI;
  extern __shared__ __attribute__((aligned(16))) unsigned char wgt4b_lds[];
  unsigned char* const lds = wgt4b_lds;
  const int tid = threadIdx.x, lane = tid & 63, wave = tid >> 6;
  const int il = lane & 31, kl = lane >> 5;
  const int n0 = blockIdx.x * frames_per_wg;
  const int n1 = n0 + frames_per_wg < g.N ? n0 + frames_per_wg : g.N;
  if (n0 >= n1) return;
  const int nlast = n1 - 1;

  const bool act_elu = g.act == MTRSSM_ACT_ELU, act_relu = g.act == MTRSSM_ACT_RELU, pre = pre_act_a != 0;
  auto act_sel = [&](float x) __attribute__((always_inline)) {
    float e = __expf(x) - 1.f;
    asm volatile("" : "+v"(e));
    const float neg = act_elu ? e : (act_relu ? 0.f : x);
    return (x > 0.f || !pre) ? x : neg;
  };

  for (int o = tid * 16; o < wgt4b_lds_bytes<SPLIT, WO>(); o += NT * 16) *reinterpret_cast<uint4*>(lds + o) = make_uint4(0u, 0u, 0u, 0u);

  const float4* const xsrc = reinterpret_cast<const float4*>(src) + tid;
  const float4* const asrc = reinterpret_cast<const float4*>(a) + tid;
  constexpr size_t xfr = (size_t)C * HS * WS / 4, afr = (size_t)CO * 64 / 4;
  wg_f32x4 raw[3][NI];
  auto raw_load = [&](const int rs, const int n) __attribute__((always_inline)) {
#pragma unroll
    for (int it = 0; it < NI; ++it) {
      const float4* const ptr = it < AI ? asrc + (size_t)n * afr + NT * it : xsrc + (size_t)n * xfr + NT * (it - AI);
      asm volatile("global_load_dwordx4 %0, %1, off" : "=v"(raw[rs][it]) : "v"(ptr));
    }
  };
  auto raw_wait = [&](const int rs) __attribute__((always_inline)) {
    static_assert(NI == 6, "six items");
    asm volatile("s_waitcnt vmcnt(12)" : "+v"(raw[rs][0]), "+v"(raw[rs][1]), "+v"(raw[rs][2]), "+v"(raw[rs][3]), "+v"(raw[rs][4]), "+v"(raw[rs][5]));
  };
  auto stage = [&](const int rs) __attribute__((always_inline)) {
#pragma unroll
    for (int it = 0; it < NI; ++it) {
      const wg_f32x4 v = raw[rs][it];
      if (it < AI) {
        unsigned d0[SPLIT], d1[SPLIT];
        wg_split_pair<SPLIT>(act_sel(v.x), act_sel(v.y), d0);
        wg_split_pair<SPLIT>(act_sel(v.z), act_sel(v.w), d1);
        const int f = tid + NT * it;
        const unsigned o = (unsigned)(SPLIT * 2 * XCOPY) + (unsigned)((f >> 4) * AP + (f & 15) * 8);
#pragma unroll
        for (int p = 0; p < SPLIT; ++p) *reinterpret_cast<uint2*>(lds + o + p * APB) = make_uint2(d0[p], d1[p]);
      } else {
        unsigned de[SPLIT], dd[SPLIT];
        wg_split_pair<SPLIT>(v.x, v.z, de);
        wg_split_pair<SPLIT>(v.y, v.w, dd);
        const int f = tid + NT * (it - AI);
        const int co = f / (HS * WS / 4), rem = f - co * (HS * WS / 4), row = rem / (WS / 4), c4 = rem - row * (WS / 4);
        const unsigned o = (unsigned)(co * CIP + (row + 1) * ROWB + c4 * 4);
#pragma unroll
        for (int p = 0; p < SPLIT; ++p) {
          *reinterpret_cast<unsigned*>(lds + o + p * 2 * XCOPY) = de[p];
          *reinterpret_cast<unsigned*>(lds + o + p * 2 * XCOPY + XCOPY) = dd[p];
        }
      }
    }
  };

  const int ky = wave >> 1;
  const bool hi = (wave & 1) != 0;
  const unsigned lane_b = (unsigned)(il * CIP + ky * ROWB + kl * (WO == 8 ? 2 * ROWB : 4 * ROWB));
  constexpr unsigned kStepB = WO == 8 ? 4 * ROWB : 8 * ROWB;
  const unsigned lane_a = (unsigned)(SPLIT * 2 * XCOPY + il * AP + kl * 16);
  f32x16 acc[4];
#pragma unroll
  for (int t = 0; t < 4; ++t)
#pragma unroll
    for (int r = 0; r < 16; ++r) acc[t][r] = 0.f;
  auto ab = [](const unsigned h, const unsigned l) __attribute__((always_inline)) { return __builtin_amdgcn_alignbit(h, l, 16); };
  auto shr1 = [&](const u32x4 f) __attribute__((always_inline)) {
    return WO == 8 ? u32x4{f.x << 16, ab(f.y, f.x), ab(f.z, f.y), ab(f.w, f.z)} : u32x4{f.x << 16, ab(f.y, f.x), f.z << 16, ab(f.w, f.z)};
  };
  auto shl1 = [&](const u32x4 f) __attribute__((always_inline)) {
    return WO == 8 ? u32x4{ab(f.y, f.x), ab(f.z, f.y), ab(f.w, f.z), f.w >> 16} : u32x4{ab(f.y, f.x), f.y >> 16, ab(f.w, f.z), f.w >> 16};
  };
  auto read_frag = [&](const unsigned off) __attribute__((always_inline)) {
    if (WO == 8) return *reinterpret_cast<const u32x4*>(lds + off);
    const uint2 r0 = *reinterpret_cast<const uint2*>(lds + off), r1 = *reinterpret_cast<const uint2*>(lds + off + 2 * ROWB);
    return u32x4{r0.x, r0.y, r1.x, r1.y};
  };

  raw_load(0, n0);
  raw_load(1, n0 + 1 < nlast ? n0 + 1 : nlast);
  auto frame = [&](const int n, const int rs) __attribute__((always_inline)) {
    raw_load((rs + 2) % 3, n + 2 < nlast ? n + 2 : nlast);
    raw_wait(rs);
    lds_barrier();
    stage(rs);
    lds_barrier();
#pragma unroll
    for (int s = 0; s < 4; ++s) {
      u32x4 qa[2][SPLIT], qb[2][SPLIT];
#pragma unroll
      for (int p = 0; p < SPLIT; ++p) {
        qa[0][p] = *reinterpret_cast<const u32x4*>(lds + lane_a + (unsigned)(p * APB) + (unsigned)(s * 32));
        qa[1][p] = *reinterpret_cast<const u32x4*>(lds + lane_a + (unsigned)(32 * AP + p * APB) + (unsigned)(s * 32));
        const unsigned bo = lane_b + (unsigned)(p * 2 * XCOPY) + (unsigned)s * kStepB;
        const u32x4 fe = read_frag(bo), fo = read_frag(bo + XCOPY);
        const u32x4 fos = shr1(fo), fes = shl1(fe);
        qb[0][p] = hi ? fo : fos;
        qb[1][p] = hi ? fes : fe;
      }
#pragma unroll
      for (int ord = SPLIT - 1; ord >= 0; --ord)
#pragma unroll
        for (int sa = 0; sa <= ord; ++sa)
#pragma unroll
          for (int t = 0; t < 4; ++t)
            acc[t] = __builtin_amdgcn_mfma_f32_32x32x16_bf16(__builtin_bit_cast(bf16x8, qa[t >> 1][sa]), __builtin_bit_cast(bf16x8, qb[t & 1][ord - sa]), acc[t], 0, 0, 0);
    }
  };
#pragma unroll 1
  for (int n = n0; n < n1; n += 3) {
    frame(n, 0);
    if (n + 1 < n1) frame(n + 1, 1);
    if (n + 2 < n1) frame(n + 2, 2);
  }
  asm volatile("s_waitcnt vmcnt(0)" ::: "memory");

  if (part) {
    float4* const ps = reinterpret_cast<float4*>(part) + (size_t)blockIdx.x * (kWgT4bSetFloats / 4) + (size_t)wave * 1024 + lane;
#pragma unroll
    for (int t = 0; t < 4; ++t)
#pragma unroll
      for (int gq = 0; gq < 4; ++gq) ps[(t * 4 + gq) * 64] = make_float4(acc[t][4 * gq], acc[t][4 * gq + 1], acc[t][4 * gq + 2], acc[t][4 * gq + 3]);
  } else {
#pragma unroll
    for (int t = 0; t < 4; ++t)
#pragma unroll
      for (int r = 0; r < 16; ++r) {
        const int row = (t >> 1) * 32 + (r & 3) + 8 * (r >> 2) + 4 * kl;
        atomicAdd(&dwp[((size_t)row * 16 + 2 * wave + (t & 1)) * g.Cpad + il], acc[t][r]);
      }
  }
}

__device__ __forceinline__ void wgrad_reduce_partials_t4b_body(const float4* __restrict__ part, const int S, const int cpad,
                                                                        float* __restrict__ dwp, const int bx, const int by) {
  constexpr int SET4 = kWgT4bSetFloats / 4, NL = 8, NG = 32;
  __shared__ float4 red[NG][NL];
  const int li = threadIdx.x & (NL - 1), sg = threadIdx.x / NL;
  const int f = bx * NL + li;
  const float4* const p = part + f;
  float4 acc4[4];
#pragma unroll
  for (int u = 0; u < 4; ++u) acc4[u] = make_float4(0.f, 0.f, 0.f, 0.f);
  int s = sg;
  for (; s + 3 * NG < S; s += 4 * NG) {
#pragma unroll
    for (int u = 0; u < 4; ++u) {
      const float4 v = p[(size_t)(s + NG * u) * SET4];
      acc4[u].x += v.x; acc4[u].y += v.y; acc4[u].z += v.z; acc4[u].w += v.w;
    }
  }
  for (; s < S; s += NG) {
    const float4 v = p[(size_t)s * SET4];
    acc4[0].x += v.x; acc4[0].y += v.y; acc4[0].z += v.z; acc4[0].w += v.w;
  }
  red[sg][li] = make_float4((acc4[0].x + acc4[1].x) + (acc4[2].x + acc4[3].x), (acc4[0].y + acc4[1].y) + (acc4[2].y + acc4[3].y),
                            (acc4[0].z + acc4[1].z) + (acc4[2].z + acc4[3].z), (acc4[0].w + acc4[1].w) + (acc4[2].w + acc4[3].w));
  __syncthreads();
  if (sg == 0) {
    float4 v = red[0][li];
#pragma unroll
    for (int k = 1; k < NG; ++k) { v.x += red[k][li].x; v.y += red[k][li].y; v.z += red[k][li].z; v.w += red[k][li].w; }
    const int lane = f & 63, gq = (f >> 6) & 3, t = (f >> 8) & 3, wave = f >> 10, il = lane & 31, kl = lane >> 5;
    const int tap = 2 * wave + (t & 1), row = (t >> 1) * 32 + 8 * gq + 4 * kl;
    float* const o = dwp + ((size_t)row * 16 + tap) * cpad + il;
    const size_t rs = (size_t)16 * cpad;
    o[0] += v.x; o[rs] += v.y; o[2 * rs] += v.z; o[3 * rs] += v.w;
  }
}
__global__ __launch_bounds__(256) void wgrad_reduce_partials_t4b_kernel(const float4* __restrict__ part, const int S, const int cpad,
                                                                        float* __restrict__ dwp) {
  wgrad_reduce_partials_t4b_body(part, S, cpad, dwp, (int)blockIdx.x, (int)blockIdx.y);
}

constexpr int kWgThinSetFloats = 8 * 64 * 4 + 8;
template <int WO>
__host__ __device__ constexpr int wgthin_cip() { return (((1024 / WO * 2 + 1) * (2 * WO)) / 16 | 1) * 16; }
template <int SPLIT, int WO>
__host__ __device__ constexpr int wgthin_lds_bytes() { return SPLIT * (2 * 3 * wgthin_cip<WO>() + 8 * 2064) + 128; }

template <int SPLIT, int WO>
__global__ __launch_bounds__(512, 1) void conv3x3s2_thin_wgrad_staged_kernel(
    const MtrssmConvGeom g, const float* __restrict__ a, const float* __restrict__ src, const float* __restrict__ coords,
    float* __restrict__ dwp, float* __restrict__ part, float* __restrict__ dbias, const int frames_per_wg) {
  static_assert(SPLIT == 1 || SPLIT == 2, "one or two bf16 pieces");
  static_assert(WO == 32 || WO == 16, "output plane 32x32 or 64x16");
  constexpr int NT = 512, CH = 3, CO = 8, HO = 1024 / WO, HS = 2 * HO, WS = 2 * WO;
  constexpr int ROWB = WS;
  constexpr int CIP = wgthin_cip<WO>();
  constexpr int XCOPY = CH * CIP;
  constexpr int AP = 2064, APB = CO * AP;
  constexpr int XI = HS * WS / 4 / NT, AI = CO * 1024 / 4 / NT, NI = XI + AI;
  constexpr int LDSB = SPLIT * (2 * XCOPY + APB);
  extern __shared__ __attribute__((aligned(16))) unsigned char wgthin_lds[];
  unsigned char* const lds = wgthin_lds;
  const int tid = threadIdx.x, lane = tid & 63, wave = tid >> 6;
  const int il = lane & 31, kl = lane >> 5;
  const int n0 = blockIdx.x * frames_per_wg;
  const int n1 = n0 + frames_per_wg < g.N ? n0 + frames_per_wg : g.N;
  if (n0 >= n1) return;
  const int nlast = n1 - 1;

  const bool act_elu = g.act == MTRSSM_ACT_ELU, act_relu = g.act == MTRSSM_ACT_RELU, pre = g.pre_act != 0;
  auto act_sel = [&](float x) __attribute__((always_inline)) {
    float e = __expf(x) - 1.f;
    asm volatile("" : "+v"(e));
    const float neg = act_elu ? e : (act_relu ? 0.f : x);
    return (x > 0.f || !pre) ? x : neg;
  };

  for (int o = tid * 16; o < wgthin_lds_bytes<SPLIT, WO>(); o += NT * 16) *reinterpret_cast<uint4*>(lds + o) = make_uint4(0u, 0u, 0u, 0u);

  auto stage_src = [&](const float4 v, const int ch, const int f) __attribute__((always_inline)) {
    unsigned de[SPLIT], dd[SPLIT];
    wg_split_pair<SPLIT>(act_sel(v.x), act_sel(v.z), de);
    wg_split_pair<SPLIT>(act_sel(v.y), act_sel(v.w), dd);
    const int row = f / (WS / 4), c4 = f - row * (WS / 4);
    const unsigned o = (unsigned)(ch * CIP + (row + 1) * ROWB + c4 * 4);
#pragma unroll
    for (int p = 0; p < SPLIT; ++p) {
      *reinterpret_cast<unsigned*>(lds + o + p * 2 * XCOPY) = de[p];
      *reinterpret_cast<unsigned*>(lds + o + p * 2 * XCOPY + XCOPY) = dd[p];
    }
  };

// ... 117 lines not shown
}

__device__ __forceinline__ void wgrad_reduce_partials_thin_body(const float4* __restrict__ part, const int S, const int cpad,
                                                                         float* __restrict__ dwp, float* __restrict__ dbias, const int bx, const int by) {
  constexpr int SET4 = kWgThinSetFloats / 4, NL = 8, NG = 32;
  __shared__ float4 red[NG][NL];
  const int li = threadIdx.x & (NL - 1), sg = threadIdx.x / NL;
  const int f = bx * NL + li;
  const bool bias = f >= 64;
  float4 acc4[2];
  acc4[0] = acc4[1] = make_float4(0.f, 0.f, 0.f, 0.f);
  if (!(bias && f >= 66)) {
    const int ks = bias ? 1 : 8;
    const int slices = S * ks;
    const float4* const p = part + (bias ? (size_t)(8 * 64 + (f - 64)) : (size_t)f);
    int i = sg;
    for (; i + NG < slices; i += 2 * NG) {
#pragma unroll
      for (int u = 0; u < 2; ++u) {
        const int ii = i + NG * u;
        const float4 v = p[(size_t)(ii / ks) * SET4 + (size_t)(ii % ks) * 64];
        acc4[u].x += v.x; acc4[u].y += v.y; acc4[u].z += v.z; acc4[u].w += v.w;
      }
    }
    for (; i < slices; i += NG) {
      const float4 v = p[(size_t)(i / ks) * SET4 + (size_t)(i % ks) * 64];
      acc4[0].x += v.x; acc4[0].y += v.y; acc4[0].z += v.z; acc4[0].w += v.w;
    }
  }
  red[sg][li] = make_float4(acc4[0].x + acc4[1].x, acc4[0].y + acc4[1].y, acc4[0].z + acc4[1].z, acc4[0].w + acc4[1].w);
  __syncthreads();
  if (sg == 0) {
    float4 v = red[0][li];
#pragma unroll
    for (int k = 1; k < NG; ++k) { v.x += red[k][li].x; v.y += red[k][li].y; v.z += red[k][li].z; v.w += red[k][li].w; }
    if (bias) {
      if (f < 66) { float* const o = dbias + 4 * (f - 64); o[0] += v.x; o[1] += v.y; o[2] += v.z; o[3] += v.w; }
      return;
    }
    const int il = f & 31, kl = f >> 5;
    if (il < 27) {
      const int tap = il / 3, ch = il - 3 * tap;
      float* const o = dwp + ((size_t)(4 * kl) * 9 + tap) * cpad + ch;
      const size_t rs = (size_t)9 * cpad;
      o[0] += v.x; o[rs] += v.y; o[2 * rs] += v.z; o[3 * rs] += v.w;
    }
  }
}
__global__ __launch_bounds__(256) void wgrad_reduce_partials_thin_kernel(const float4* __restrict__ part, const int S, const int cpad,
                                                                         float* __restrict__ dwp, float* __restrict__ dbias) {
  wgrad_reduce_partials_thin_body(part, S, cpad, dwp, dbias, (int)blockIdx.x, (int)blockIdx.y);
}

constexpr int kWgThinTSetFloats = 8 * 2 * 64 * 4;
template <int WO>
__host__ __device__ constexpr int wgthint_cip() { return (((1024 / WO * 2 + 2) * (2 * WO)) / 16 | 1) * 16; }
template <int SPLIT, int WO>
__host__ __device__ constexpr int wgthint_lds_bytes() { return SPLIT * (2 * wgthint_cip<WO>() + 16 * 2064); }

template <int SPLIT, int WO>
__global__ __launch_bounds__(512, 1) void convt4s2_thin_wgrad_staged_kernel(
    const MtrssmConvGeom g, const float* __restrict__ a, const float* __restrict__ src, const int pre_act_a, float* __restrict__ dwp,
    float* __restrict__ part, const int frames_per_wg) {
  static_assert(SPLIT == 1 || SPLIT == 2, "one or two bf16 pieces");
  static_assert(WO == 32 || WO == 16, "input plane 32x32 or 64x16");
  constexpr int NT = 512, CO = 16, HO = 1024 / WO, HS = 2 * HO, WS = 2 * WO;
  constexpr int ROWB = WS;
  constexpr int XCOPY = wgthint_cip<WO>();
  constexpr int AP = 2064, APB = CO * AP;
  constexpr int XI = HS * WS / 4 / NT, AI = CO * 1024 / 4 / NT, NI = XI + AI;
  extern __shared__ __attribute__((aligned(16))) unsigned char wgthint_lds[];
  unsigned char* const lds = wgthint_lds;
  const int tid = threadIdx.x, lane = tid & 63, wave = tid >> 6;
  const int il = lane & 31, kl = lane >> 5;
  const int n0 = blockIdx.x * frames_per_wg;
  const int n1 = n0 + frames_per_wg < g.N ? n0 + frames_per_wg : g.N;
  if (n0 >= n1) return;
  const int nlast = n1 - 1;

  const bool act_elu = g.act == MTRSSM_ACT_ELU, act_relu = g.act == MTRSSM_ACT_RELU, pre = pre_act_a != 0;
  auto act_sel = [&](float x) __attribute__((always_inline)) {
    float e = __expf(x) - 1.f;
    asm volatile("" : "+v"(e));
    const float neg = act_elu ? e : (act_relu ? 0.f : x);
    return (x > 0.f || !pre) ? x : neg;
  };

  for (int o = tid * 16; o < wgthint_lds_bytes<SPLIT, WO>(); o += NT * 16) *reinterpret_cast<uint4*>(lds + o) = make_uint4(0u, 0u, 0u, 0u);

  const float4* const xsrc = reinterpret_cast<const float4*>(src) + tid;
  const float4* const asrc = reinterpret_cast<const float4*>(a) + tid;
  constexpr size_t xfr = (size_t)HS * WS / 4, afr = (size_t)CO * 1024 / 4;
  wg_f32x4 raw[3][NI];
  auto raw_load = [&](const int rs, const int n) __attribute__((always_inline)) {
#pragma unroll
    for (int it = 0; it < NI; ++it) {
      const float4* const ptr = it < AI ? asrc + (size_t)n * afr + NT * it : xsrc + (size_t)n * xfr + NT * (it - AI);
      asm volatile("global_load_dwordx4 %0, %1, off" : "=v"(raw[rs][it]) : "v"(ptr));
    }
  };
  auto raw_wait = [&](const int rs) __attribute__((always_inline)) {
    static_assert(NI == 10, "ten items");
    asm volatile("s_waitcnt vmcnt(20)" : "+v"(raw[rs][0]), "+v"(raw[rs][1]), "+v"(raw[rs][2]), "+v"(raw[rs][3]), "+v"(raw[rs][4]), "+v"(raw[rs][5]),
                 "+v"(raw[rs][6]), "+v"(raw[rs][7]), "+v"(raw[rs][8]), "+v"(raw[rs][9]));
  };
  auto stage = [&](const int rs) __attribute__((always_inline)) {
#pragma unroll
    for (int it = 0; it < NI; ++it) {
      const wg_f32x4 v = raw[rs][it];
      if (it < AI) {
        unsigned d0[SPLIT], d1[SPLIT];
        wg_split_pair<SPLIT>(act_sel(v.x), act_sel(v.y), d0);
        wg_split_pair<SPLIT>(act_sel(v.z), act_sel(v.w), d1);
        const int f = tid + NT * it;
        const unsigned o = (unsigned)(SPLIT * 2 * XCOPY) + (unsigned)((f >> 8) * AP + (f & 255) * 8);
#pragma unroll
        for (int p = 0; p < SPLIT; ++p) *reinterpret_cast<uint2*>(lds + o + p * APB) = make_uint2(d0[p], d1[p]);
      } else {
        unsigned de[SPLIT], dd[SPLIT];
        wg_split_pair<SPLIT>(v.x, v.z, de);
        wg_split_pair<SPLIT>(v.y, v.w, dd);
        const int f = tid + NT * (it - AI);
        const int row = f / (WS / 4), c4 = f - row * (WS / 4);
        const unsigned o = (unsigned)((row + 1) * ROWB + c4 * 4);
#pragma unroll
        for (int p = 0; p < SPLIT; ++p) {
          *reinterpret_cast<unsigned*>(lds + o + p * 2 * XCOPY) = de[p];
          *reinterpret_cast<unsigned*>(lds + o + p * 2 * XCOPY + XCOPY) = dd[p];
        }
      }
    }
  };

  const int tap = il & 15, ky = tap >> 2, kx = tap & 3;
  const bool odd = kx == 0 || kx == 2;
  const unsigned lane_b = (unsigned)((odd ? XCOPY : 0) + ky * ROWB + kl * 16);
  const unsigned lane_a = (unsigned)(SPLIT * 2 * XCOPY + (il & 15) * AP + kl * 16);
  f32x16 acc;
#pragma unroll
  for (int r = 0; r < 16; ++r) acc[r] = 0.f;

  raw_load(0, n0);
  raw_load(1, n0 + 1 < nlast ? n0 + 1 : nlast);
  auto frame = [&](const int n, const int rs) __attribute__((always_inline)) {
    raw_load((rs + 2) % 3, n + 2 < nlast ? n + 2 : nlast);
    raw_wait(rs);
    lds_barrier();
    stage(rs);
    lds_barrier();
#pragma unroll
    for (int ss = 0; ss < 8; ++ss) {
      const int s = wave * 8 + ss;
      const unsigned soff = WO == 32 ? (unsigned)((s >> 1) * 2 * ROWB + (s & 1) * 32) : (unsigned)(s * 2 * ROWB);
      const bool has_prev = WO == 32 ? ((s & 1) | kl) != 0 : kl != 0;
      const bool has_next = WO == 32 ? ((s & 1) & kl) == 0 : kl == 0;
      u32x4 qa[SPLIT], qb[SPLIT];
#pragma unroll
      for (int p = 0; p < SPLIT; ++p) {
        qa[p] = *reinterpret_cast<const u32x4*>(lds + lane_a + (unsigned)(p * APB) + (unsigned)(s * 32));
        const unsigned bo = lane_b + (unsigned)(p * 2 * XCOPY) + soff;
        const u32x4 f = *reinterpret_cast<const u32x4*>(lds + bo);
        const unsigned prev = has_prev ? (unsigned)*reinterpret_cast<const unsigned short*>(lds + bo - 2) : 0u;
        const unsigned next = has_next ? (unsigned)*reinterpret_cast<const unsigned short*>(lds + bo + 16) : 0u;
        const u32x4 shr = u32x4{(f.x << 16) | prev, __builtin_amdgcn_alignbit(f.y, f.x, 16), __builtin_amdgcn_alignbit(f.z, f.y, 16), __builtin_amdgcn_alignbit(f.w, f.z, 16)};
        const u32x4 shl = u32x4{__builtin_amdgcn_alignbit(f.y, f.x, 16), __builtin_amdgcn_alignbit(f.z, f.y, 16), __builtin_amdgcn_alignbit(f.w, f.z, 16), (f.w >> 16) | (next << 16)};
        qb[p] = kx == 0 ? shr : (kx == 3 ? shl : f);
      }
#pragma unroll
      for (int ord = SPLIT - 1; ord >= 0; --ord)
#pragma unroll
        for (int sa = 0; sa <= ord; ++sa)
          acc = __builtin_amdgcn_mfma_f32_32x32x16_bf16(__builtin_bit_cast(bf16x8, qa[sa]), __builtin_bit_cast(bf16x8, qb[ord - sa]), acc, 0, 0, 0);
    }
  };
#pragma unroll 1
  for (int n = n0; n < n1; n += 3) {
    frame(n, 0);
    if (n + 1 < n1) frame(n + 1, 1);
    if (n + 2 < n1) frame(n + 2, 2);
  }
  asm volatile("s_waitcnt vmcnt(0)" ::: "memory");

  if (part) {
    float4* const ps = reinterpret_cast<float4*>(part) + (size_t)blockIdx.x * (kWgThinTSetFloats / 4) + (size_t)wave * 128 + lane;
    ps[0] = make_float4(acc[0], acc[1], acc[2], acc[3]);
    ps[64] = make_float4(acc[4], acc[5], acc[6], acc[7]);
  } else if (il < 16) {
#pragma unroll
    for (int r = 0; r < 8; ++r) atomicAdd(&dwp[((size_t)((r & 3) + 8 * (r >> 2) + 4 * kl) * 16 + tap) * g.Cpad], acc[r]);
  }
}

__device__ __forceinline__ void wgrad_reduce_partials_thint_body(const float4* __restrict__ part, const int S, const int cpad,
                                                                          float* __restrict__ dwp, const int bx, const int by) {
  constexpr int SET4 = kWgThinTSetFloats / 4, NL = 8, NG = 32;
  __shared__ float4 red[NG][NL];
  const int li = threadIdx.x & (NL - 1), sg = threadIdx.x / NL;
  const int f = bx * NL + li;
  const float4* const p = part + f;
  float4 acc4[2];
  acc4[0] = acc4[1] = make_float4(0.f, 0.f, 0.f, 0.f);
  const int slices = S * 8;
  int i = sg;
  for (; i + NG < slices; i += 2 * NG) {
#pragma unroll
    for (int u = 0; u < 2; ++u) {
      const int ii = i + NG * u;
      const float4 v = p[(size_t)(ii >> 3) * SET4 + (size_t)(ii & 7) * 128];
      acc4[u].x += v.x; acc4[u].y += v.y; acc4[u].z += v.z; acc4[u].w += v.w;
    }
  }
  for (; i < slices; i += NG) {
    const float4 v = p[(size_t)(i >> 3) * SET4 + (size_t)(i & 7) * 128];
    acc4[0].x += v.x; acc4[0].y += v.y; acc4[0].z += v.z; acc4[0].w += v.w;
  }
  red[sg][li] = make_float4(acc4[0].x + acc4[1].x, acc4[0].y + acc4[1].y, acc4[0].z + acc4[1].z, acc4[0].w + acc4[1].w);
  __syncthreads();
  if (sg == 0) {
    float4 v = red[0][li];
#pragma unroll
    for (int k = 1; k < NG; ++k) { v.x += red[k][li].x; v.y += red[k][li].y; v.z += red[k][li].z; v.w += red[k][li].w; }
    const int half = f >> 6, lane = f & 63, il = lane & 31, kl = lane >> 5;
    if (il < 16) {
      float* const o = dwp + ((size_t)(8 * half + 4 * kl) * 16 + il) * cpad;
      const size_t rs = (size_t)16 * cpad;
      o[0] += v.x; o[rs] += v.y; o[2 * rs] += v.z; o[3 * rs] += v.w;
    }
  }
}
__global__ __launch_bounds__(256) void wgrad_reduce_partials_thint_kernel(const float4* __restrict__ part, const int S, const int cpad,
                                                                          float* __restrict__ dwp) {
  wgrad_reduce_partials_thint_body(part, S, cpad, dwp, (int)blockIdx.x, (int)blockIdx.y);
}

constexpr int kWgS2cSetFloats = 8 * 4 * 64 * 4 + 32;
template <int SPLIT>
__host__ __device__ constexpr int wgs2c_lds_bytes() { return SPLIT * (2 * 16 * 272 + 32 * kWgresAPitch); }

template <int SPLIT, int WO>
__global__ __launch_bounds__(512, 1) void conv3x3s2c_wgrad_staged_kernel(
    const MtrssmConvGeom g, const float* __restrict__ a, const float* __restrict__ src, float* __restrict__ dwp,
    float* __restrict__ part, float* __restrict__ dbias, const int frames_per_wg) {
  static_assert(SPLIT == 1 || SPLIT == 2, "one or two bf16 pieces");
  static_assert(WO == 8 || WO == 4, "output plane 8x8 or 16x4");
  constexpr int NT = 512, C = 16, CO = 32, HO = 64 / WO, HS = 2 * HO, WS = 2 * WO;
  constexpr int ROWB = WS;
  constexpr int CIP = 272;
  static_assert((HS + 1) * ROWB <= CIP, "channel pitch");
  constexpr int XCOPY = C * CIP;
  constexpr int AP = kWgresAPitch, APB = CO * AP;
  constexpr int XI = C * HS * WS / 4 / NT, AI = CO * 64 / 4 / NT, NI = XI + AI;
  extern __shared__ __attribute__((aligned(16))) unsigned char wgs2c_lds[];
  unsigned char* const lds = wgs2c_lds;
  const int tid = threadIdx.x, lane = tid & 63, wave = tid >> 6;
  const int il = lane & 31, kl = lane >> 5;
  const int n0 = blockIdx.x * frames_per_wg;
  const int n1 = n0 + frames_per_wg < g.N ? n0 + frames_per_wg : g.N;
  if (n0 >= n1) return;
  const int nlast = n1 - 1;

  const bool act_elu = g.act == MTRSSM_ACT_ELU, act_relu = g.act == MTRSSM_ACT_RELU, pre = g.pre_act != 0;
  auto act_sel = [&](float x) __attribute__((always_inline)) {
    float e = __expf(x) - 1.f;
    asm volatile("" : "+v"(e));
    const float neg = act_elu ? e : (act_relu ? 0.f : x);
    return (x > 0.f || !pre) ? x : neg;
  };

  for (int o = tid * 16; o < wgs2c_lds_bytes<SPLIT>(); o += NT * 16) *reinterpret_cast<uint4*>(lds + o) = make_uint4(0u, 0u, 0u, 0u);

  const float4* const xsrc = reinterpret_cast<const float4*>(src) + tid;
  const float4* const asrc = reinterpret_cast<const float4*>(a) + tid;
  constexpr size_t xfr = (size_t)C * HS * WS / 4, afr = (size_t)CO * 64 / 4;
  float bsum = 0.f;
  wg_f32x4 raw[3][NI];
  auto raw_load = [&](const int rs, const int n) __attribute__((always_inline)) {
#pragma unroll
    for (int it = 0; it < NI; ++it) {
      const float4* const ptr = it < AI ? asrc + (size_t)n * afr + NT * it : xsrc + (size_t)n * xfr + NT * (it - AI);
      asm volatile("global_load_dwordx4 %0, %1, off" : "=v"(raw[rs][it]) : "v"(ptr));
    }
  };
  auto raw_wait = [&](const int rs) __attribute__((always_inline)) {
    static_assert(NI == 3, "three items");
    asm volatile("s_waitcnt vmcnt(6)" : "+v"(raw[rs][0]), "+v"(raw[rs][1]), "+v"(raw[rs][2]));
// ... 156 lines not shown
```

Before: 355,700 seq-steps/s.

## Fuse residual 1x1 backward and convT bias reduction into weight-grad kernels

Adds a fused residual-block 1x1 backward kernel that produces the input gradient, weight gradient and bias gradient in one launch, replacing a transposed-gather conv plus a separate weight-grad call. The transposed-conv weight-grad staged kernels also accumulate per-channel sums of the source tensor while staging it, and write them into extra slots of the partials buffer. This removes the separate channel_sum pass over the output gradient and the extra launches. In exchange the partials layouts and reducers become more complex and the change touches several kernels.

```diff
diff --git a/include/mtrssm.h b/include/mtrssm.h
--- a/include/mtrssm.h
+++ b/include/mtrssm.h
@@ -337,6 +337,12 @@
 int mtrssm_conv_weight_grad_deferred(const MtrssmConvGeom* g, const float* a, const float* src, const float* src2,
                                      int32_t pre_act_a, float* dwp, float* dbias, void* workspace, int64_t workspace_bytes, void* stream);
 int mtrssm_conv_weight_grad_reduce(void* stream);
+int mtrssm_conv_weight_grad_src_bias_supported(const MtrssmConvGeom* g, int32_t pre_act_a);
+int mtrssm_residual_bwd1x1_supported(const MtrssmConvGeom* g);
+int mtrssm_residual_bwd1x1(const MtrssmConvGeom* g, const float* gy, const float* h, const uint16_t* wq1t, float* gh, float* dwp,
+                           float* dbias, void* workspace, int64_t workspace_bytes, int32_t defer, void* stream);
+int mtrssm_conv_weight_grad_src_bias(const MtrssmConvGeom* g, const float* a, const float* src, int32_t pre_act_a, float* dwp,
+                                     float* dsrc_bias, void* workspace, int64_t workspace_bytes, int32_t defer, void* stream);
 int64_t mtrssm_conv_weight_grad_workspace_bytes(const MtrssmConvGeom* g, int32_t pre_act_a);
 int mtrssm_unpack_conv_grads(const int64_t* table, int32_t count, int32_t blocks_per_entry, void* stream);
 int mtrssm_convt_quad_supported(const MtrssmConvGeom* g4);
diff --git a/multimodal_mtrssm_amd/_lib.py b/multimodal_mtrssm_amd/_lib.py
--- a/multimodal_mtrssm_amd/_lib.py
+++ b/multimodal_mtrssm_amd/_lib.py
@@ -115,6 +115,10 @@
     "mtrssm_unpack_conv_grads": (C.c_int, [_p, _i, _i, _p]),
     "mtrssm_conv_weight_grad": (C.c_int, [C.POINTER(ConvGeom), _p, _p, _p, _i, _p, _p, _p, C.c_int64, _p]),
     "mtrssm_conv_weight_grad_deferred": (C.c_int, [C.POINTER(ConvGeom), _p, _p, _p, _i, _p, _p, _p, C.c_int64, _p]),
+    "mtrssm_residual_bwd1x1_supported": (C.c_int, [C.POINTER(ConvGeom)]),
+    "mtrssm_residual_bwd1x1": (C.c_int, [C.POINTER(ConvGeom), _p, _p, _p, _p, _p, _p, _p, C.c_int64, _i, _p]),
+    "mtrssm_conv_weight_grad_src_bias_supported": (C.c_int, [C.POINTER(ConvGeom), _i]),
+    "mtrssm_conv_weight_grad_src_bias": (C.c_int, [C.POINTER(ConvGeom), _p, _p, _i, _p, _p, _p, C.c_int64, _i, _p]),
     "mtrssm_conv_weight_grad_reduce": (C.c_int, [_p]),
     "mtrssm_conv_weight_grad_workspace_bytes": (C.c_int64, [C.POINTER(ConvGeom), _i]),
     "mtrssm_channel_sum": (C.c_int, [_p, _i, _i, _i, _p, _p]),
diff --git a/multimodal_mtrssm_amd/conv.py b/multimodal_mtrssm_amd/conv.py
--- a/multimodal_mtrssm_amd/conv.py
+++ b/multimodal_mtrssm_amd/conv.py
@@ -489,7 +489,7 @@
 
 def _weight_grad(a: Tensor, src: Tensor, coords: Tensor | None, kh: int, kw: int, stride: int, pad: int, pre_act_a: bool,
                  pre_act_src: bool, act: int, *, want_bias: bool = False, weight: Tensor | None = None,
-                 bias: Tensor | None = None) -> tuple[Tensor | None, Tensor | None]:
+                 bias: Tensor | None = None, want_src_bias: bool = False) -> tuple[Tensor | None, Tensor | None]:
     lib = _lib.load()
     n, o, hq, wq = a.shape
     _, c, hs, ws = src.shape
@@ -497,22 +497,34 @@
     opad, ipad = _pads(o, c + c2)
     sunk = _GRAD_SINK.target(weight, o, c + c2, kh * kw, opad, ipad)
     dwp = sunk if sunk is not None else _zeros(opad * kh * kw * ipad, a.device).view(opad, kh * kw, ipad)
+    fuse_src_bias = want_src_bias and CONVT_BIAS_FUSE and coords is None and a.data_ptr() % 16 == 0 and src.data_ptr() % 16 == 0
     dbias = bias_sunk = None
-    if want_bias:
+    if want_bias or fuse_src_bias:
         bias_sunk = grad_target(bias) if bias is not None and bias.is_contiguous() else None
-        dbias = bias_sunk if bias_sunk is not None else _zeros(o, a.device)
     geom = _geom(N=n, C=c, Hs=hs, Ws=ws, C2=c2, Cpad=ipad, KH=kh, KW=kw, SS=stride, TS=1, OFFY=-pad, OFFX=-pad, Hq=hq, Wq=wq,
                  OS=1, QY=0, QX=0, Ho=hq, Wo=wq, Cout=o, CoutPad=opad, pre_act=int(pre_act_src), act=act)
     flops = 2.0 * n * hq * wq * o * kh * kw * (c + c2)
     nbytes = 4.0 * (a.numel() + src.numel())
-    defer = DEFER_WGRAD_REDUCE and sunk is not None and (not want_bias or bias_sunk is not None)
+    fuse_src_bias = fuse_src_bias and bool(lib.mtrssm_conv_weight_grad_src_bias_supported(C.byref(geom), int(pre_act_a)))
+    if want_bias or fuse_src_bias:
+        dbias = bias_sunk if bias_sunk is not None else _zeros(c if fuse_src_bias else o, a.device)
+    defer = DEFER_WGRAD_REDUCE and sunk is not None and (dbias is None or bias_sunk is not None)
     ws = _wgrad_workspace(geom, int(pre_act_a), a.device, own=defer)
+    if fuse_src_bias:
+        _lib.check(_lib.TIMERS.call(
+            "mtrssm_conv_weight_grad", lib.mtrssm_conv_weight_grad_src_bias, C.byref(geom), _lib.ptr(a), _lib.ptr(src), int(pre_act_a),
+            _lib.ptr(dwp), _lib.ptr(dbias), _lib.raw_ptr(ws), 0 if ws is None else ws.numel() * 4, int(defer and ws is not None),
+            _lib.stream_ptr(a.device), flops=flops, nbytes=nbytes), "mtrssm_conv_weight_grad_src_bias")
+        g_w = None if sunk is not None else dwp[:o, :, : c + c2].reshape(o, kh, kw, c + c2).permute(0, 3, 1, 2)
+        return g_w, (None if bias_sunk is not None else dbias)
     entry = lib.mtrssm_conv_weight_grad_deferred if defer and ws is not None else lib.mtrssm_conv_weight_grad
     _lib.check(_lib.TIMERS.call(
         "mtrssm_conv_weight_grad", entry, C.byref(geom), _lib.ptr(a), _lib.ptr(src), _lib.ptr(coords),
         int(pre_act_a), _lib.ptr(dwp), _lib.ptr(dbias), _lib.raw_ptr(ws), 0 if ws is None else ws.numel() * 4, _lib.stream_ptr(a.device),
         flops=flops, nbytes=nbytes), "mtrssm_conv_weight_grad")
     g_w = None if sunk is not None else dwp[:o, :, : c + c2].reshape(o, kh, kw, c + c2).permute(0, 3, 1, 2)
+    if want_src_bias:
+        return g_w, _channel_sum(src, bias)
     return g_w, (None if bias_sunk is not None else dbias)
 
 
@@ -583,13 +595,17 @@
         g_x = None
         if ctx.needs_input_grad[0]:
             g_x = _conv_forward_gather(g_out, None, weight, None, stride, pad, False, act, actgrad_in=x if pre_act else None)
-        g_w = None
+        g_w = g_b = None
+        want_b = has_bias and ctx.needs_input_grad[2]
         if ctx.needs_input_grad[1]:
-            g_w, _ = _weight_grad(x, g_out, None, kh, kw, stride, pad, pre_act, False, act, weight=weight)
-        g_b = _channel_sum(g_out, ctx.bias) if has_bias and ctx.needs_input_grad[2] else None
+            g_w, g_b = _weight_grad(x, g_out, None, kh, kw, stride, pad, pre_act, False, act, weight=weight, bias=ctx.bias,
+                                    want_src_bias=want_b)
+        elif want_b:
+            g_b = _channel_sum(g_out, ctx.bias)
         return g_x, g_w, g_b, None, None, None, None, None
 
 
+CONVT_BIAS_FUSE = True
 RESBLOCK_FUSE = True
 
 
@@ -628,6 +644,43 @@
                                 _lib.stream_ptr(ja[1].device), flops=fa + fb, nbytes=ba + bb), "mtrssm_residual_block_fwd")
 
 
+RESBLOCK_BWD1X1_FUSE = True
+
+
+def _bwd1x1_geom(g_y: Tensor, h: Tensor, w1: Tensor, act: int) -> C.Structure | None:
+    if not RESBLOCK_BWD1X1_FUSE or _MFMA_SPLIT != 2 or w1.shape[2:] != (1, 1) or not g_y.is_cuda:
+        return None
+    n, o, hq, wq = g_y.shape
+    c = h.shape[1]
+    if w1.shape[:2] != (o, c) or h.shape != (n, c, hq, wq) or g_y.data_ptr() % 16 or h.data_ptr() % 16:
+        return None
+    opad, ipad = _pads(o, c)
+    geom = _geom(N=n, C=c, Hs=hq, Ws=wq, C2=0, Cpad=ipad, KH=1, KW=1, SS=1, TS=1, OFFY=0, OFFX=0, Hq=hq, Wq=wq, OS=1, QY=0, QX=0,
+                 Ho=hq, Wo=wq, Cout=o, CoutPad=opad, pre_act=1, act=act)
+    return geom if _lib.load().mtrssm_residual_bwd1x1_supported(C.byref(geom)) else None
+
+
+def _bwd1x1_fused(geom: C.Structure, g_y: Tensor, h: Tensor, w1: Tensor, b1: Tensor) -> tuple[Tensor, Tensor | None, Tensor | None]:
+    lib = _lib.load()
+    n, o, hq, wq = g_y.shape
+    c = h.shape[1]
+    _, wq1t = pack_weight(w1.permute(1, 0, 2, 3))
+    sunk = _GRAD_SINK.target(w1, o, c, 1, geom.CoutPad, geom.Cpad)
+    dwp = sunk if sunk is not None else _zeros(geom.CoutPad * geom.Cpad, g_y.device).view(geom.CoutPad, 1, geom.Cpad)
+    bias_sunk = grad_target(b1) if b1.is_contiguous() else None
+    dbias = bias_sunk if bias_sunk is not None else _zeros(o, g_y.device)
+    defer = DEFER_WGRAD_REDUCE and sunk is not None and bias_sunk is not None
+    ws = _wgrad_workspace(geom, 0, g_y.device, own=defer)
+    g_h = torch.empty_like(h)
+    pixels = n * hq * wq
+    _lib.check(_lib.TIMERS.call(
+        "mtrssm_residual_bwd1x1", lib.mtrssm_residual_bwd1x1, C.byref(geom), _lib.ptr(g_y), _lib.ptr(h), _lib.raw_ptr(wq1t), _lib.ptr(g_h),
+        _lib.ptr(dwp), _lib.ptr(dbias), _lib.raw_ptr(ws), 0 if ws is None else ws.numel() * 4, int(defer and ws is not None),
+        _lib.stream_ptr(g_y.device), flops=2.0 * 2.0 * pixels * o * c, nbytes=4.0 * (g_y.numel() + 2 * h.numel())), "mtrssm_residual_bwd1x1")
+    g_w = None if sunk is not None else dwp[:o, :, :c].reshape(o, 1, 1, c).permute(0, 3, 1, 2)
+    return g_h, g_w, (None if bias_sunk is not None else dbias)
+
+
 class _ResidualBlock(torch.autograd.Function):
 
     @staticmethod
@@ -651,9 +704,13 @@
         act = ctx.act
         g_y = g_y.contiguous()
         p3, p1 = w3.shape[2] // 2, w1.shape[2] // 2
-        g_h = _conv_transposed_gather(g_y, w1, None, 1, p1, (h.shape[2], h.shape[3]), False, act, actgrad_in=h)
         b3, b1 = ctx.biases
-        g_w1, g_b1 = _weight_grad(g_y, h, None, w1.shape[2], w1.shape[3], 1, p1, False, True, act, want_bias=True, weight=w1, bias=b1)
+        g1 = _bwd1x1_geom(g_y, h, w1, act)
+        if g1 is not None:
+            g_h, g_w1, g_b1 = _bwd1x1_fused(g1, g_y, h, w1, b1)
+        else:
+            g_h = _conv_transposed_gather(g_y, w1, None, 1, p1, (h.shape[2], h.shape[3]), False, act, actgrad_in=h)
+            g_w1, g_b1 = _weight_grad(g_y, h, None, w1.shape[2], w1.shape[3], 1, p1, False, True, act, want_bias=True, weight=w1, bias=b1)
         g_x = None
         if ctx.needs_input_grad[0]:
             g_x = _conv_transposed_gather(g_h, w3, None, 1, p3, (x.shape[2], x.shape[3]), False, act, actgrad_in=x, add_in=g_y)
@@ -687,11 +744,17 @@
         act = ctx.act
         g_ya, g_yv = g_ya.contiguous(), g_yv.contiguous()
         p3, p1 = w3a.shape[2] // 2, w1a.shape[2] // 2
-        g_ha, g_hv = paired(lambda: _conv_transposed_gather(g_ya, w1a, None, 1, p1, (ha.shape[2], ha.shape[3]), False, act, actgrad_in=ha),
-                            lambda: _conv_transposed_gather(g_yv, w1v, None, 1, p1, (hv.shape[2], hv.shape[3]), False, act, actgrad_in=hv))
         b3a, b1a, b3v, b1v = ctx.biases
-        g_w1a, g_b1a = _weight_grad(g_ya, ha, None, w1a.shape[2], w1a.shape[3], 1, p1, False, True, act, want_bias=True, weight=w1a, bias=b1a)
-        g_w1v, g_b1v = _weight_grad(g_yv, hv, None, w1v.shape[2], w1v.shape[3], 1, p1, False, True, act, want_bias=True, weight=w1v, bias=b1v)
+        g1a = _bwd1x1_geom(g_ya, ha, w1a, act)
+        g1v = _bwd1x1_geom(g_yv, hv, w1v, act) if g1a is not None else None
+        if g1a is not None and g1v is not None:
+            g_ha, g_w1a, g_b1a = _bwd1x1_fused(g1a, g_ya, ha, w1a, b1a)
+            g_hv, g_w1v, g_b1v = _bwd1x1_fused(g1v, g_yv, hv, w1v, b1v)
+        else:
+            g_ha, g_hv = paired(lambda: _conv_transposed_gather(g_ya, w1a, None, 1, p1, (ha.shape[2], ha.shape[3]), False, act, actgrad_in=ha),
+                                lambda: _conv_transposed_gather(g_yv, w1v, None, 1, p1, (hv.shape[2], hv.shape[3]), False, act, actgrad_in=hv))
+            g_w1a, g_b1a = _weight_grad(g_ya, ha, None, w1a.shape[2], w1a.shape[3], 1, p1, False, True, act, want_bias=True, weight=w1a, bias=b1a)
+            g_w1v, g_b1v = _weight_grad(g_yv, hv, None, w1v.shape[2], w1v.shape[3], 1, p1, False, True, act, want_bias=True, weight=w1v, bias=b1v)
         g_xa, g_xv = paired(
             lambda: _conv_transposed_gather(g_ha, w3a, None, 1, p3, (xa.shape[2], xa.shape[3]), False, act, actgrad_in=xa, add_in=g_ya),
             lambda: _conv_transposed_gather(g_hv, w3v, None, 1, p3, (xv.shape[2], xv.shape[3]), False, act, actgrad_in=xv, add_in=g_yv))
diff --git a/multimodal_mtrssm_amd/csrc/capi.hip b/multimodal_mtrssm_amd/csrc/capi.hip
--- a/multimodal_mtrssm_amd/csrc/capi.hip
+++ b/multimodal_mtrssm_amd/csrc/capi.hip
@@ -38,6 +38,11 @@
 int conv_weight_grad_launch(const MtrssmConvGeom*, const float*, const float*, const float*, int, float*, float*, void*, size_t, size_t*, hipStream_t);
 int conv_weight_grad_deferred_launch(const MtrssmConvGeom*, const float*, const float*, const float*, int, float*, float*, void*, size_t, hipStream_t);
 int conv_weight_grad_reduce_flush(hipStream_t);
+int conv_residual_bwd1x1_supported(const MtrssmConvGeom*);
+int conv_residual_bwd1x1_launch(const MtrssmConvGeom*, const float*, const float*, const unsigned short*, float*, float*, float*, void*, size_t, int,
+                                hipStream_t);
+int conv_weight_grad_src_bias_supported(const MtrssmConvGeom*, int);
+int conv_weight_grad_src_bias_launch(const MtrssmConvGeom*, const float*, const float*, int, float*, float*, void*, size_t, int, hipStream_t);
 int channel_sum_launch(const float*, int, int, int, float*, hipStream_t);
 int convt_k4s2_band_supported(int, int, int, int, int);
 int convt_k4s2_band_launch(int, int, int, int, int, const float*, const float*, const float*, int, int, float*, hipStream_t);
@@ -277,6 +282,20 @@
   return conv_weight_grad_deferred_launch(g, a, src, src2, pre_act_a, dwp, dbias, workspace, workspace_bytes < 0 ? 0 : (size_t)workspace_bytes,
                                           static_cast<hipStream_t>(stream));
 }
+MTRSSM_API int mtrssm_residual_bwd1x1_supported(const MtrssmConvGeom* g) { return conv_residual_bwd1x1_supported(g) != 0; }
+MTRSSM_API int mtrssm_residual_bwd1x1(const MtrssmConvGeom* g, const float* gy, const float* h, const uint16_t* wq1t, float* gh, float* dwp,
+                                      float* dbias, void* workspace, int64_t workspace_bytes, int32_t defer, void* stream) {
+  return conv_residual_bwd1x1_launch(g, gy, h, wq1t, gh, dwp, dbias, workspace, workspace_bytes < 0 ? 0 : (size_t)workspace_bytes, defer,
+                                     static_cast<hipStream_t>(stream));
+}
+MTRSSM_API int mtrssm_conv_weight_grad_src_bias_supported(const MtrssmConvGeom* g, int32_t pre_act_a) {
+  return conv_weight_grad_src_bias_supported(g, pre_act_a);
+}
+MTRSSM_API int mtrssm_conv_weight_grad_src_bias(const MtrssmConvGeom* g, const float* a, const float* src, int32_t pre_act_a, float* dwp,
+                                                float* dsrc_bias, void* workspace, int64_t workspace_bytes, int32_t defer, void* stream) {
+  return conv_weight_grad_src_bias_launch(g, a, src, pre_act_a, dwp, dsrc_bias, workspace, workspace_bytes < 0 ? 0 : (size_t)workspace_bytes,
+                                          defer, static_cast<hipStream_t>(stream));
+}
 MTRSSM_API int mtrssm_conv_weight_grad_reduce(void* stream) { return conv_weight_grad_reduce_flush(static_cast<hipStream_t>(stream)); }
 MTRSSM_API int64_t mtrssm_conv_weight_grad_workspace_bytes(const MtrssmConvGeom* g, int32_t pre_act_a) {
   size_t need = 0;
diff --git a/multimodal_mtrssm_amd/csrc/conv.hip b/multimodal_mtrssm_amd/csrc/conv.hip
--- a/multimodal_mtrssm_amd/csrc/conv.hip
+++ b/multimodal_mtrssm_amd/csrc/conv.hip
@@ -610,10 +610,10 @@
     case kRed1x1_64: wgrad_reduce_partials1x1_body<64>(j.part, j.S, j.cpad, j.dwp, j.dbias, bx, by); break;
     case kRed1x1_128: wgrad_reduce_partials1x1_body<128>(j.part, j.S, j.cpad, j.dwp, j.dbias, bx, by); break;
     case kRedThin: wgrad_reduce_partials_thin_body(j.part, j.S, j.cpad, j.dwp, j.dbias, bx, by); break;
-    case kRedThinT: wgrad_reduce_partials_thint_body(j.part, j.S, j.cpad, j.dwp, bx, by); break;
+    case kRedThinT: wgrad_reduce_partials_thint_body(j.part, j.S, j.cpad, j.dwp, j.dbias, bx, by); break;
     case kRedS2: wgrad_reduce_partials_s2_body(j.part, j.S, j.cpad, j.dwp, j.dbias, bx, by); break;
-    case kRedT4: wgrad_reduce_partials_t4_body(j.part, j.S, j.cpad, j.dwp, bx, by); break;
-    case kRedT4b: wgrad_reduce_partials_t4b_body(j.part, j.S, j.cpad, j.dwp, bx, by); break;
+    case kRedT4: wgrad_reduce_partials_t4_body(j.part, j.S, j.cpad, j.dwp, j.dbias, bx, by); break;
+    case kRedT4b: wgrad_reduce_partials_t4b_body(j.part, j.S, j.cpad, j.dwp, j.dbias, bx, by); break;
     default: wgrad_reduce_partials_s2c_body(j.part, j.S, j.cpad, j.dwp, j.dbias, bx, by); break;
   }
 }
@@ -1777,6 +1777,40 @@
 
 int conv_weight_grad_launch(const MtrssmConvGeom* g, const float* a, const float* src, const float* src2, int pre_act_a,
                             float* dwp, float* dbias, void* workspace, size_t workspace_bytes, size_t* query, hipStream_t stream);
+struct WgradSrcBias {
+  float* target = nullptr;
+  bool fused = false;
+};
+int conv_weight_grad_launch_ex(const MtrssmConvGeom* g, const float* a, const float* src, const float* src2, int pre_act_a, float* dwp,
+                               float* dbias, void* workspace, size_t workspace_bytes, size_t* query, WgradSrcBias* sb, hipStream_t stream);
+int conv_weight_grad_launch(const MtrssmConvGeom* g, const float* a, const float* src, const float* src2, int pre_act_a,
+                            float* dwp, float* dbias, void* workspace, size_t workspace_bytes, size_t* query, hipStream_t stream) {
+  return conv_weight_grad_launch_ex(g, a, src, src2, pre_act_a, dwp, dbias, workspace, workspace_bytes, query, nullptr, stream);
+}
+int conv_weight_grad_src_bias_supported(const MtrssmConvGeom* g, int pre_act_a) {
+  WgradSrcBias sb;
+  size_t need = 0;
+  const int rc = conv_weight_grad_launch_ex(g, nullptr, nullptr, nullptr, pre_act_a, nullptr, nullptr, nullptr, 0, &need, &sb, nullptr);
+  return rc == MTRSSM_OK && sb.fused;
+}
+int conv_weight_grad_src_bias_launch(const MtrssmConvGeom* g, const float* a, const float* src, int pre_act_a, float* dwp,
+                                     float* dsrcbias, void* workspace, size_t workspace_bytes, int defer, hipStream_t stream) {
+  if (!dsrcbias) { set_error("conv_weight_grad_src_bias: null dsrc_bias"); return MTRSSM_EINVAL; }
+  if (((uintptr_t)a & 15) || ((uintptr_t)src & 15)) {
+    set_error("conv_weight_grad_src_bias: a and src must be 16-byte aligned");
+    return MTRSSM_EINVAL;
+  }
+  if (!conv_weight_grad_src_bias_supported(g, pre_act_a)) {
+    set_error("conv_weight_grad_src_bias: this geometry's kernel has no fused source sums (query mtrssm_conv_weight_grad_src_bias_supported first)");
+    return MTRSSM_EINVAL;
+  }
+  WgradSrcBias sb;
+  sb.target = dsrcbias;
+  tl_defer_reduce = defer != 0;
+  const int rc = conv_weight_grad_launch_ex(g, a, src, nullptr, pre_act_a, dwp, nullptr, workspace, workspace_bytes, nullptr, &sb, stream);
+  tl_defer_reduce = false;
+  return rc;
+}
 int conv_weight_grad_deferred_launch(const MtrssmConvGeom* g, const float* a, const float* src, const float* src2, int pre_act_a,
                                      float* dwp, float* dbias, void* workspace, size_t workspace_bytes, hipStream_t stream) {
   tl_defer_reduce = true;
@@ -1785,8 +1819,58 @@
   return rc;
 }
 
-int conv_weight_grad_launch(const MtrssmConvGeom* g, const float* a, const float* src, const float* src2, int pre_act_a,
-                            float* dwp, float* dbias, void* workspace, size_t workspace_bytes, size_t* query, hipStream_t stream) {
+int conv_residual_bwd1x1_supported(const MtrssmConvGeom* g) {
+  static const bool on = [] { const char* e = getenv("MTRSSM_BWD1X1_FUSED"); return !(e && e[0] == '0'); }();
+  if (!g || !on || !wgrad_1x1_staged_enabled()) return 0;
+  return g->mfma_split == 2 && g->KH == 1 && g->KW == 1 && g->SS == 1 && g->OFFY == 0 && g->OFFX == 0 && g->C2 == 0 && g->Hs == g->Hq &&
+         g->Ws == g->Wq && g->Hq * g->Wq == 64 && (g->C == 64 || g->C == 128) && g->Cout == 64 && g->Cpad >= g->C && g->N >= 1 &&
+         g->OS == 1 && g->QY == 0 && g->QX == 0 && g->pre_act != 0 &&
+         (g->act == MTRSSM_ACT_IDENTITY || g->act == MTRSSM_ACT_ELU || g->act == MTRSSM_ACT_RELU);
+}
+int conv_residual_bwd1x1_launch(const MtrssmConvGeom* g, const float* gy, const float* h, const unsigned short* wq1t, float* gh, float* dwp,
+                                float* dbias, void* workspace, size_t workspace_bytes, int defer, hipStream_t stream) {
+  if (!conv_residual_bwd1x1_supported(g)) {
+    set_error("residual_bwd1x1: shape without a fused kernel (query mtrssm_residual_bwd1x1_supported first)");
+    return MTRSSM_EINVAL;
+  }
+  if (!gy || !h || !wq1t || !gh || !dwp) { set_error("residual_bwd1x1: null pointer"); return MTRSSM_EINVAL; }
+  if (((uintptr_t)gy & 15) || ((uintptr_t)h & 15) || ((uintptr_t)wq1t & 15) || ((uintptr_t)gh & 3) || ((uintptr_t)workspace & 255)) {
+    set_error("residual_bwd1x1: g_y, h and the weight pieces must be 16-byte aligned, the workspace 256-byte aligned");
+    return MTRSSM_EINVAL;
+  }
+  int wgs = cu_count();
+  if (wgs > g->N) wgs = g->N;
+  const int per = (g->N + wgs - 1) / wgs;
+  const dim3 grid((unsigned)((g->N + per - 1) / per));
+  float* part = nullptr;
+  if (wgrad_partials_enabled() && workspace && workspace_bytes >= (size_t)grid.x * kWg1x1SetFloats * sizeof(float)) part = static_cast<float*>(workspace);
+#define MTRSSM_BW1_LAUNCH(C_)                                                                                                   \
+  {                                                                                                                             \
+    static bool attr_done_dev[64] = {}; bool& attr_done = attr_done_dev[device_slot()];                                         \
+    constexpr int lds_b = bwd1x1_lds_bytes<C_>();                                                                               \
+    if (!attr_done) {                                                                                                           \
+      (void)hipFuncSetAttribute(reinterpret_cast<const void*>(conv1x1_bwd_fused_kernel<C_>),                                    \
+                                hipFuncAttributeMaxDynamicSharedMemorySize, lds_b);                                             \
+      attr_done = true;                                                                                                         \
+    }                                                                                                                           \
+    set_last_kernel("mtrssm::conv1x1_bwd_fused_kernel<" #C_ ">");                                                               \
+    hipLaunchKernelGGL((conv1x1_bwd_fused_kernel<C_>), grid, dim3(512), lds_b, stream, *g, gy, h, wq1t, gh, dwp, part, dbias,   \
+                       per);                                                                                                    \
+  }
+  if (g->C == 64) MTRSSM_BW1_LAUNCH(64) else MTRSSM_BW1_LAUNCH(128)
+#undef MTRSSM_BW1_LAUNCH
+  if (part) {
+    const dim3 rgrid((unsigned)(2 * (g->C / 32) * 256 / 32 + (dbias ? 1 : 0)), 1);
+    tl_defer_reduce = defer != 0;
+    const int rc = reduce_now_or_later(g->C == 64 ? kRed1x1_64 : kRed1x1_128, rgrid, part, (int)grid.x, g->Cpad, dwp, dbias, stream);
+    tl_defer_reduce = false;
+    if (rc) return rc;
+  }
+  return launched("residual_bwd1x1");
+}
+
+int conv_weight_grad_launch_ex(const MtrssmConvGeom* g, const float* a, const float* src, const float* src2, int pre_act_a, float* dwp,
+                               float* dbias, void* workspace, size_t workspace_bytes, size_t* query, WgradSrcBias* sb, hipStream_t stream) {
   if (int rc = check_geom(g, "conv_weight_grad")) return rc;
   if (!query && (!a || !src || !dwp || (g->C2 > 0 && !src2))) { set_error("conv_weight_grad: null pointer"); return MTRSSM_EINVAL; }
   if (workspace && ((uintptr_t)workspace & 255)) { set_error("conv_weight_grad: workspace must be 256-byte aligned"); return MTRSSM_EINVAL; }
@@ -1951,6 +2035,8 @@
     if (wgs > g->N) wgs = g->N;
     const int per = (g->N + wgs - 1) / wgs;
     const dim3 grid((unsigned)((g->N + per - 1) / per));
+    if (sb) sb->fused = true;
+    float* const dsrcbias = sb ? sb->target : nullptr;
     MTRSSM_WGRAD_PART((size_t)grid.x * kWgThinTSetFloats * sizeof(float))
 #define MTRSSM_WGTHINT_LAUNCH(SP_, W_)                                                                                           \
   {                                                                                                                             \
@@ -1963,14 +2049,14 @@
     }                                                                                                                           \
     set_last_kernel("mtrssm::convt4s2_thin_wgrad_staged_kernel<" #SP_ ", " #W_ ">");                                             \
     hipLaunchKernelGGL((convt4s2_thin_wgrad_staged_kernel<SP_, W_>), grid, dim3(512), lds_b, stream, *g, a, src, pre_act_a, dwp, \
-                       part, per);                                                                                              \
+                       part, dsrcbias, per);                                                                                    \
   }
     const int sp = g->mfma_split;
     if (g->Wq == 32) { if (sp == 2) MTRSSM_WGTHINT_LAUNCH(2, 32) else MTRSSM_WGTHINT_LAUNCH(1, 32) }
     else { if (sp == 2) MTRSSM_WGTHINT_LAUNCH(2, 16) else MTRSSM_WGTHINT_LAUNCH(1, 16) }
 #undef MTRSSM_WGTHINT_LAUNCH
     if (part)
-      if (int rc = reduce_now_or_later(kRedThinT, dim3(16), part, (int)grid.x, g->Cpad, dwp, nullptr, stream)) return rc;
+      if (int rc = reduce_now_or_later(kRedThinT, dim3(dsrcbias ? 17 : 16), part, (int)grid.x, g->Cpad, dwp, dsrcbias, stream)) return rc;
     return launched("conv_weight_grad(k4 s2 thin staged)");
   }
   if (g->mfma_split >= 1 && g->Cout <= 32 && taps * ctot <= 32 && g->Wq >= 8 && (g->Wq & (g->Wq - 1)) == 0 && (g->Hq * g->Wq) % 16 == 0 &&
@@ -2029,6 +2115,8 @@
     if (wgs > g->N) wgs = g->N;
     const int per = (g->N + wgs - 1) / wgs;
     const dim3 grid((unsigned)((g->N + per - 1) / per));
+    if (sb) sb->fused = true;
+    float* const dsrcbias = sb ? sb->target : nullptr;
     MTRSSM_WGRAD_PART((size_t)grid.x * kWgT4SetFloats * sizeof(float))
 #define MTRSSM_WGT4_LAUNCH(SP_, W_)                                                                                              \
   {                                                                                                                             \
@@ -2041,14 +2129,14 @@
     }                                                                                                                           \
     set_last_kernel("mtrssm::convt4s2_wgrad_staged_kernel<" #SP_ ", " #W_ ">");                                                  \
     hipLaunchKernelGGL((convt4s2_wgrad_staged_kernel<SP_, W_>), grid, dim3(512), lds_b, stream, *g, a, src, pre_act_a, dwp,      \
-                       part, per);                                                                                              \
+                       part, dsrcbias, per);                                                                                    \
   }
     const int sp = g->mfma_split;
     if (g->Wq == 16) { if (sp == 2) MTRSSM_WGT4_LAUNCH(2, 16) else MTRSSM_WGT4_LAUNCH(1, 16) }
     else { if (sp == 2) MTRSSM_WGT4_LAUNCH(2, 8) else MTRSSM_WGT4_LAUNCH(1, 8) }
 #undef MTRSSM_WGT4_LAUNCH
     if (part)
-      if (int rc = reduce_now_or_later(kRedT4, dim3(kWgT4SetFloats / 4 / 8), part, (int)grid.x, g->Cpad, dwp, nullptr, stream)) return rc;
+      if (int rc = reduce_now_or_later(kRedT4, dim3(kWgT4TileFloats / 4 / 8 + (dsrcbias ? 1 : 0)), part, (int)grid.x, g->Cpad, dwp, dsrcbias, stream)) return rc;
     return launched("conv_weight_grad(k4 s2 staged)");
   }
   if ((g->mfma_split == 1 || g->mfma_split == 2) && g->KH == 4 && g->KW == 4 && g->SS == 2 && g->TS == 1 && g->OFFY == -1 && g->OFFX == -1 &&
@@ -2059,6 +2147,8 @@
     if (wgs > g->N) wgs = g->N;
     const int per = (g->N + wgs - 1) / wgs;
     const dim3 grid((unsigned)((g->N + per - 1) / per));
+    if (sb) sb->fused = true;
+    float* const dsrcbias = sb ? sb->target : nullptr;
     MTRSSM_WGRAD_PART((size_t)grid.x * kWgT4bSetFloats * sizeof(float))
 #define MTRSSM_WGT4B_LAUNCH(SP_, W_)                                                                                             \
   {                                                                                                                             \
@@ -2071,14 +2161,14 @@
     }                                                                                                                           \
     set_last_kernel("mtrssm::convt4s2b_wgrad_staged_kernel<" #SP_ ", " #W_ ">");                                                 \
     hipLaunchKernelGGL((convt4s2b_wgrad_staged_kernel<SP_, W_>), grid, dim3(512), lds_b, stream, *g, a, src, pre_act_a, dwp,     \
-                       part, per);                                                                                              \
+                       part, dsrcbias, per);                                                                                    \
   }
     const int sp = g->mfma_split;
     if (g->Wq == 8) { if (sp == 2) MTRSSM_WGT4B_LAUNCH(2, 8) else MTRSSM_WGT4B_LAUNCH(1, 8) }
     else { if (sp == 2) MTRSSM_WGT4B_LAUNCH(2, 4) else MTRSSM_WGT4B_LAUNCH(1, 4) }
 #undef MTRSSM_WGT4B_LAUNCH
     if (part)
-      if (int rc = reduce_now_or_later(kRedT4b, dim3(kWgT4bSetFloats / 4 / 8), part, (int)grid.x, g->Cpad, dwp, nullptr, stream)) return rc;
+      if (int rc = reduce_now_or_later(kRedT4b, dim3(kWgT4bTileFloats / 4 / 8 + (dsrcbias ? 1 : 0)), part, (int)grid.x, g->Cpad, dwp, dsrcbias, stream)) return rc;
     return launched("conv_weight_grad(k4 s2 staged, 64 rows)");
   }
   if ((g->mfma_split == 1 || g->mfma_split == 2) && g->KH == 3 && g->KW == 3 && g->SS == 2 && g->TS == 1 && g->OFFY == -1 && g->OFFX == -1 &&
diff --git a/multimodal_mtrssm_amd/csrc/conv_wgrad_resident.h b/multimodal_mtrssm_amd/csrc/conv_wgrad_resident.h
--- a/multimodal_mtrssm_amd/csrc/conv_wgrad_resident.h
+++ b/multimodal_mtrssm_amd/csrc/conv_wgrad_resident.h
@@ -521,6 +521,212 @@
   wgrad_reduce_partials1x1_body<C>(part, S, cpad, dwp, dbias, (int)blockIdx.x, (int)blockIdx.y);
 }
 
+template <int C>
+__host__ __device__ constexpr int bwd1x1_lds_bytes() { return wg1x1_lds_bytes<2, C>() + 2 * 2 * 64 * kWgresAPitch; }
+
+template <int C>
+__global__ __launch_bounds__(512, 1) void conv1x1_bwd_fused_kernel(
+    const MtrssmConvGeom g, const float* __restrict__ a, const float* __restrict__ src, const unsigned short* __restrict__ wq,
+    float* __restrict__ gh, float* __restrict__ dwp, float* __restrict__ part, float* __restrict__ dbias, const int frames_per_wg) {
+  static_assert(C == 64 || C == 128, "mid channels");
+  constexpr int SPLIT = 2, NT = 512, P = kWgresAPitch;
+  constexpr int XI = C * 16 / NT, AI = 2, NI = XI + AI;
+  constexpr int NTILE = 2 * (C / 32), KS = 8 / NTILE;
+  constexpr int APB = 64 * P, XPB = C * P;
+  constexpr int BUFB = SPLIT * (APB + XPB);
+  constexpr int PMB = 64 * P, PMBUF = SPLIT * PMB;
+  constexpr int PM0 = 2 * BUFB;
+  extern __shared__ __attribute__((aligned(16))) unsigned char bw1_lds[];
+  unsigned char* const lds = bw1_lds;
+  const int tid = threadIdx.x, lane = tid & 63, wave = tid >> 6;
+  const int il = lane & 31, kl = lane >> 5;
+  const int tile = wave % NTILE, kpart = wave / NTILE;
+  const int tco = tile & 1, tci = tile >> 1;
+  const int n0 = blockIdx.x * frames_per_wg;
+  const int n1 = n0 + frames_per_wg < g.N ? n0 + frames_per_wg : g.N;
+  if (n0 >= n1) return;
+  const int nlast = n1 - 1;
+
+  const bool act_elu = g.act == MTRSSM_ACT_ELU, act_relu = g.act == MTRSSM_ACT_RELU;
+  auto act_sel = [&](float x) __attribute__((always_inline)) {
+    float e = __expf(x) - 1.f;
+    asm volatile("" : "+v"(e));
+    const float neg = act_elu ? e : (act_relu ? 0.f : x);
+    return x > 0.f ? x : neg;
+  };
+
+  const int bct = (wave >> 1) % (C / 32), bhalf = wave & 1;
+  const bool bstore = C == 128 || wave < 4;
+  u32x4 wa[4][2];
+#pragma unroll
+  for (int cb = 0; cb < 4; ++cb)
+#pragma unroll
+    for (int sp = 0; sp < 2; ++sp) {
+      wa[cb][sp] = *reinterpret_cast<const u32x4*>(wq + (size_t)sp * (C * 64) + (size_t)(bct * 32 + il) * 64 + cb * 16 + 8 * kl);
+      asm volatile("" : "+v"(wa[cb][sp]));
+    }
+
+  const float4* const xsrc = reinterpret_cast<const float4*>(src) + tid;
+  const float4* const asrc = reinterpret_cast<const float4*>(a) + tid;
+  constexpr size_t xfr = (size_t)C * 16, afr = (size_t)64 * 16;
+  const unsigned wofs = (unsigned)((tid >> 4) * P + (tid & 15) * 8);
+  const unsigned pofs = (unsigned)(PM0 + 4 * (tid & 15) * P + (tid >> 4) * 2);
+  float bsum[AI];
+#pragma unroll
+  for (int j = 0; j < AI; ++j) bsum[j] = 0.f;
+  wg_f32x4 raw[3][NI];
+  auto raw_load = [&](const int rs, const int n) __attribute__((always_inline)) {
+#pragma unroll
+    for (int it = 0; it < NI; ++it) {
+      const float4* const ptr = it < AI ? asrc + (size_t)n * afr + NT * it : xsrc + (size_t)n * xfr + NT * (it - AI);
+      asm volatile("global_load_dwordx4 %0, %1, off" : "=v"(raw[rs][it]) : "v"(ptr));
+    }
+  };
+  auto raw_wait = [&](const int rs) __attribute__((always_inline)) {
+    if constexpr (NI == 4) asm volatile("s_waitcnt vmcnt(40)" : "+v"(raw[rs][0]), "+v"(raw[rs][1]), "+v"(raw[rs][2]), "+v"(raw[rs][3]));
+    else asm volatile("s_waitcnt vmcnt(44)" : "+v"(raw[rs][0]), "+v"(raw[rs][1]), "+v"(raw[rs][2]), "+v"(raw[rs][3]), "+v"(raw[rs][4]), "+v"(raw[rs][5]));
+  };
+  const float* const hop = src + (size_t)(bct * 32 + 4 * kl) * 64 + bhalf * 32 + il;
+  float* const ghp = gh + (size_t)(bct * 32 + 4 * kl) * 64 + bhalf * 32 + il;
+  float opv[2][16];
+  auto op_load = [&](const int os, const int n) __attribute__((always_inline)) {
+#pragma unroll
+    for (int r = 0; r < 16; ++r) {
+      const float* const ptr = hop + (size_t)n * (C * 64) + ((r & 3) + 8 * (r >> 2)) * 64;
+      asm volatile("global_load_dword %0, %1, off" : "=v"(opv[os][r]) : "v"(ptr));
+    }
+  };
+  auto op_wait = [&](const int os) __attribute__((always_inline)) {
+#define MTRSSM_OPV(os_, b_) "+v"(opv[os_][b_]), "+v"(opv[os_][b_ + 1]), "+v"(opv[os_][b_ + 2]), "+v"(opv[os_][b_ + 3]), "+v"(opv[os_][b_ + 4]), \
+                            "+v"(opv[os_][b_ + 5]), "+v"(opv[os_][b_ + 6]), "+v"(opv[os_][b_ + 7])
+    if constexpr (NI == 4) asm volatile("s_waitcnt vmcnt(24)" : MTRSSM_OPV(os, 0));
+    else asm volatile("s_waitcnt vmcnt(28)" : MTRSSM_OPV(os, 0));
+    asm volatile("" : MTRSSM_OPV(os, 8));
+#undef MTRSSM_OPV
+  };
+  auto stage = [&](const int rs, const unsigned bufoff, const unsigned pmoff) __attribute__((always_inline)) {
+#pragma unroll
+    for (int it = 0; it < NI; ++it) {
+      const wg_f32x4 v = raw[rs][it];
+      unsigned d0[SPLIT], d1[SPLIT];
+      if (it < AI) {
+        bsum[it] += (v.x + v.y) + (v.z + v.w);
+        wg_split_pair<SPLIT>(v.x, v.y, d0);
+        wg_split_pair<SPLIT>(v.z, v.w, d1);
+#pragma unroll
+        for (int p = 0; p < SPLIT; ++p) {
+          unsigned char* const q = lds + pmoff + pofs + (unsigned)(it * 64 + p * PMB);
+          *reinterpret_cast<unsigned short*>(q) = (unsigned short)(d0[p] & 0xffffu);
+          *reinterpret_cast<unsigned short*>(q + P) = (unsigned short)(d0[p] >> 16);
+          *reinterpret_cast<unsigned short*>(q + 2 * P) = (unsigned short)(d1[p] & 0xffffu);
+          *reinterpret_cast<unsigned short*>(q + 3 * P) = (unsigned short)(d1[p] >> 16);
+        }
+      } else {
+        wg_split_pair<SPLIT>(act_sel(v.x), act_sel(v.y), d0);
+        wg_split_pair<SPLIT>(act_sel(v.z), act_sel(v.w), d1);
+      }
+      const unsigned base = it < AI ? (unsigned)(it * 32 * P) : (unsigned)(SPLIT * APB + (it - AI) * 32 * P);
+      const unsigned piece = it < AI ? (unsigned)APB : (unsigned)XPB;
+#pragma unroll
+      for (int p = 0; p < SPLIT; ++p) *reinterpret_cast<uint2*>(lds + bufoff + base + wofs + p * piece) = make_uint2(d0[p], d1[p]);
+    }
+  };
+
+  const unsigned lane_a = (unsigned)((tco * 32 + il) * P + kl * 16);
+  const unsigned lane_b = (unsigned)(SPLIT * APB + (tci * 32 + il) * P + kl * 16);
+  const unsigned lane_p = (unsigned)(PM0 + (bhalf * 32 + il) * P + kl * 16);
+  f32x16 acc;
+#pragma unroll
+  for (int r = 0; r < 16; ++r) acc[r] = 0.f;
+
+  raw_load(0, n0);
+  op_load(0, n0);
+  raw_load(1, n0 + 1 < nlast ? n0 + 1 : nlast);
+  auto frame = [&](const int n, const int rs, const int par) __attribute__((always_inline)) {
+    const unsigned bufoff = par ? (unsigned)BUFB : 0u, pmoff = par ? (unsigned)PMBUF : 0u;
+    op_load(par ^ 1, n + 1 < nlast ? n + 1 : nlast);
+    raw_load((rs + 2) % 3, n + 2 < nlast ? n + 2 : nlast);
+    raw_wait(rs);
+    stage(rs, bufoff, pmoff);
+    lds_barrier();
+#pragma unroll
+    for (int qq = 0; qq < 4 / KS; ++qq) {
+      const int q = kpart * (4 / KS) + qq;
+      u32x4 qa[SPLIT], qb[SPLIT];
+#pragma unroll
+      for (int p = 0; p < SPLIT; ++p) {
+        qa[p] = *reinterpret_cast<const u32x4*>(lds + bufoff + lane_a + (unsigned)(p * APB) + (unsigned)(q * 32));
+        qb[p] = *reinterpret_cast<const u32x4*>(lds + bufoff + lane_b + (unsigned)(p * XPB) + (unsigned)(q * 32));
+      }
+#pragma unroll
+      for (int ord = SPLIT - 1; ord >= 0; --ord)
+#pragma unroll
+        for (int sa = 0; sa <= ord; ++sa)
+          acc = __builtin_amdgcn_mfma_f32_32x32x16_bf16(__builtin_bit_cast(bf16x8, qa[sa]), __builtin_bit_cast(bf16x8, qb[ord - sa]), acc, 0, 0, 0);
+    }
+    f32x16 accb;
+#pragma unroll
+    for (int r = 0; r < 16; ++r) accb[r] = 0.f;
+#pragma unroll
+    for (int cb = 0; cb < 4; ++cb) {
+      const bf16x8 bh = __builtin_bit_cast(bf16x8, *reinterpret_cast<const u32x4*>(lds + pmoff + lane_p + (unsigned)(cb * 32)));
+      const bf16x8 bl = __builtin_bit_cast(bf16x8, *reinterpret_cast<const u32x4*>(lds + pmoff + lane_p + (unsigned)(PMB + cb * 32)));
+      accb = __builtin_amdgcn_mfma_f32_32x32x16_bf16(__builtin_bit_cast(bf16x8, wa[cb][0]), bl, accb, 0, 0, 0);
+      accb = __builtin_amdgcn_mfma_f32_32x32x16_bf16(__builtin_bit_cast(bf16x8, wa[cb][1]), bh, accb, 0, 0, 0);
+      accb = __builtin_amdgcn_mfma_f32_32x32x16_bf16(__builtin_bit_cast(bf16x8, wa[cb][0]), bh, accb, 0, 0, 0);
+    }
+    op_wait(par);
+    if (bstore) {
+      float* const o = ghp + (size_t)n * (C * 64);
+#pragma unroll
+      for (int r = 0; r < 16; ++r) {
+        const float x = opv[par][r];
+        const float e = __expf(x);
+        const float neg = act_elu ? e : (act_relu ? 0.f : 1.f);
+        o[((r & 3) + 8 * (r >> 2)) * 64] = accb[r] * (x > 0.f ? 1.f : neg);
+      }
+    }
+  };
+#pragma unroll 1
+  for (int n = n0; n < n1; n += 6) {
+    frame(n, 0, 0);
+    if (n + 1 < n1) frame(n + 1, 1, 1);
+    if (n + 2 < n1) frame(n + 2, 2, 0);
+    if (n + 3 < n1) frame(n + 3, 0, 1);
+    if (n + 4 < n1) frame(n + 4, 1, 0);
+    if (n + 5 < n1) frame(n + 5, 2, 1);
+  }
+  asm volatile("s_waitcnt vmcnt(0)" ::: "memory");
+
+  if (part) {
+    float4* const ps = reinterpret_cast<float4*>(part) + (size_t)blockIdx.x * (kWg1x1SetFloats / 4) + (size_t)wave * 256 + lane;
+#pragma unroll
+    for (int gq = 0; gq < 4; ++gq) ps[gq * 64] = make_float4(acc[4 * gq], acc[4 * gq + 1], acc[4 * gq + 2], acc[4 * gq + 3]);
+  } else {
+    const int ci = tci * 32 + il;
+#pragma unroll
+    for (int r = 0; r < 16; ++r) {
+      const int row = tco * 32 + (r & 3) + 8 * (r >> 2) + 4 * kl;
+      atomicAdd(&dwp[(size_t)row * g.Cpad + ci], acc[r]);
+    }
+  }
+  if (dbias != nullptr) {
+#pragma unroll
+    for (int j = 0; j < AI; ++j) {
+      float v = bsum[j];
+      v += dpp_move<0xB1, 0xF>(0.f, v);
+      v += dpp_move<0x4E, 0xF>(0.f, v);
+      v += dpp_move<0x141, 0xF>(0.f, v);
+      v += dpp_move<0x140, 0xF>(0.f, v);
+      if ((tid & 15) == 0) {
+        const int ch = (tid >> 4) + j * 32;
+        if (part) part[(size_t)blockIdx.x * kWg1x1SetFloats + 8 * 1024 + ch] = v;
+        else atomicAdd(&dbias[ch], v);
+      }
+    }
+  }
+}
+
 constexpr int kWgS2SetFloats = 8 * 2 * 64 * 4 + 16;
 template <int WO>
 __host__ __device__ constexpr int wgs2_cip() { return (((256 / WO * 2 + 1) * (2 * WO)) / 16 | 1) * 16; }
@@ -746,7 +952,8 @@
   wgrad_reduce_partials_s2_body(part, S, cpad, dwp, dbias, (int)blockIdx.x, (int)blockIdx.y);
 }
 
-constexpr int kWgT4SetFloats = 8 * 4 * 64 * 4;
+constexpr int kWgT4TileFloats = 8 * 4 * 64 * 4;
+constexpr int kWgT4SetFloats = kWgT4TileFloats + 16;
 template <int WO>
 __host__ __device__ constexpr int wgt4_cip() { return (((256 / WO * 2 + 2) * (2 * WO)) / 16 | 1) * 16; }
 template <int SPLIT, int WO>
@@ -755,7 +962,7 @@
 template <int SPLIT, int WO>
 __global__ __launch_bounds__(512, 1) void convt4s2_wgrad_staged_kernel(
     const MtrssmConvGeom g, const float* __restrict__ a, const float* __restrict__ src, const int pre_act_a, float* __restrict__ dwp,
-    float* __restrict__ part, const int frames_per_wg) {
+    float* __restrict__ part, float* __restrict__ dsrcbias, const int frames_per_wg) {
   static_assert(SPLIT == 1 || SPLIT == 2, "one or two bf16 pieces");
   static_assert(WO == 16 || WO == 8, "input plane 16x16 or 32x8");
   constexpr int NT = 512, C = 16, CO = 32, HO = 256 / WO, HS = 2 * HO, WS = 2 * WO;
@@ -786,6 +993,10 @@
   const float4* const xsrc = reinterpret_cast<const float4*>(src) + tid;
   const float4* const asrc = reinterpret_cast<const float4*>(a) + tid;
   constexpr size_t xfr = (size_t)C * HS * WS / 4, afr = (size_t)CO * 256 / 4;
+  static_assert(HS * WS / 4 == 256 && XI == 8, "src item j of a thread is channel tid / 256 + 2 j");
+  float bsum[XI];
+#pragma unroll
+  for (int j = 0; j < XI; ++j) bsum[j] = 0.f;
   wg_f32x4 raw[3][NI];
   auto raw_load = [&](const int rs, const int n) __attribute__((always_inline)) {
 #pragma unroll
@@ -813,6 +1024,7 @@
         for (int p = 0; p < SPLIT; ++p) *reinterpret_cast<uint2*>(lds + o + p * APB) = make_uint2(d0[p], d1[p]);
       } else {
         unsigned de[SPLIT], dd[SPLIT];
+        bsum[it - AI] += (v.x + v.y) + (v.z + v.w);
         wg_split_pair<SPLIT>(v.x, v.z, de);
         wg_split_pair<SPLIT>(v.y, v.w, dd);
         const int f = tid + NT * (it - AI);
@@ -877,6 +1089,16 @@
   }
   asm volatile("s_waitcnt vmcnt(0)" ::: "memory");
 
+  float* const bred = reinterpret_cast<float*>(lds);
+  if (dsrcbias != nullptr) {
+    lds_barrier();
+#pragma unroll
+    for (int j = 0; j < XI; ++j) {
+      const float v = wave_sum(bsum[j]);
+      if (lane == 0) bred[j * 8 + wave] = v;
+    }
+    lds_barrier();
+  }
   if (part) {
     float4* const ps = reinterpret_cast<float4*>(part) + (size_t)blockIdx.x * (kWgT4SetFloats / 4) + (size_t)wave * 256 + lane;
 #pragma unroll
@@ -888,15 +1110,21 @@
       atomicAdd(&dwp[((size_t)row * 16 + tap) * g.Cpad + co], acc[r]);
     }
   }
+  if (dsrcbias != nullptr && tid < 16) {
+    const int j = tid >> 1, w0 = 4 * (tid & 1);
+    const float v = (bred[j * 8 + w0] + bred[j * 8 + w0 + 1]) + (bred[j * 8 + w0 + 2] + bred[j * 8 + w0 + 3]);
+    if (part) part[(size_t)blockIdx.x * kWgT4SetFloats + kWgT4TileFloats + tid] = v;
+    else atomicAdd(&dsrcbias[tid], v);
+  }
 }
 
 __device__ __forceinline__ void wgrad_reduce_partials_t4_body(const float4* __restrict__ part, const int S, const int cpad,
-                                                                       float* __restrict__ dwp, const int bx, const int by) {
-  constexpr int SET4 = kWgT4SetFloats / 4, NL = 8, NG = 32;
+                                                                       float* __restrict__ dwp, float* __restrict__ dbias, const int bx, const int by) {
+  constexpr int SET4 = kWgT4SetFloats / 4, TILE4 = kWgT4TileFloats / 4, NL = 8, NG = 32;
   __shared__ float4 red[NG][NL];
   const int li = threadIdx.x & (NL - 1), sg = threadIdx.x / NL;
   const int f = bx * NL + li;
-  const float4* const p = part + f;
+  const float4* const p = part + (f < SET4 ? f : SET4 - 1);
   float4 acc4[4];
 #pragma unroll
   for (int u = 0; u < 4; ++u) acc4[u] = make_float4(0.f, 0.f, 0.f, 0.f);
@@ -919,6 +1147,10 @@
     float4 v = red[0][li];
 #pragma unroll
     for (int k = 1; k < NG; ++k) { v.x += red[k][li].x; v.y += red[k][li].y; v.z += red[k][li].z; v.w += red[k][li].w; }
+    if (f >= TILE4) {
+      if (f < SET4) { float* const o = dbias + 4 * (f - TILE4); o[0] += v.x; o[1] += v.y; o[2] += v.z; o[3] += v.w; }
+      return;
+    }
     const int lane = f & 63, gq = (f >> 6) & 3, wave = f >> 8, il = lane & 31, kl = lane >> 5;
     const int col = wave * 32 + il, tap = col >> 4, co = col & 15, row = 8 * gq + 4 * kl;
     float* const o = dwp + ((size_t)row * 16 + tap) * cpad + co;
@@ -927,11 +1159,12 @@
   }
 }
 __global__ __launch_bounds__(256) void wgrad_reduce_partials_t4_kernel(const float4* __restrict__ part, const int S, const int cpad,
-                                                                       float* __restrict__ dwp) {
-  wgrad_reduce_partials_t4_body(part, S, cpad, dwp, (int)blockIdx.x, (int)blockIdx.y);
-}
-
-constexpr int kWgT4bSetFloats = 8 * 4 * 4 * 64 * 4;
+                                                                       float* __restrict__ dwp, float* __restrict__ dbias) {
+  wgrad_reduce_partials_t4_body(part, S, cpad, dwp, dbias, (int)blockIdx.x, (int)blockIdx.y);
+}
+
+constexpr int kWgT4bTileFloats = 8 * 4 * 4 * 64 * 4;
+constexpr int kWgT4bSetFloats = kWgT4bTileFloats + 32;
 template <int WO>
 __host__ __device__ constexpr int wgt4b_cip() { return (((64 / WO * 2 + 2) * (2 * WO)) / 16 | 1) * 16; }
 template <int SPLIT, int WO>
@@ -940,7 +1173,7 @@
 template <int SPLIT, int WO>
 __global__ __launch_bounds__(512, 1) void convt4s2b_wgrad_staged_kernel(
     const MtrssmConvGeom g, const float* __restrict__ a, const float* __restrict__ src, const int pre_act_a, float* __restrict__ dwp,
-    float* __restrict__ part, const int frames_per_wg) {
+    float* __restrict__ part, float* __restrict__ dsrcbias, const int frames_per_wg) {
   static_assert(SPLIT == 1 || SPLIT == 2, "one or two bf16 pieces");
   static_assert(WO == 8 || WO == 4, "input plane 8x8 or 16x4");
   constexpr int NT = 512, C = 32, CO = 64, HO = 64 / WO, HS = 2 * HO, WS = 2 * WO;
@@ -971,6 +1204,10 @@
   const float4* const xsrc = reinterpret_cast<const float4*>(src) + tid;
   const float4* const asrc = reinterpret_cast<const float4*>(a) + tid;
   constexpr size_t xfr = (size_t)C * HS * WS / 4, afr = (size_t)CO * 64 / 4;
+  static_assert(HS * WS / 4 == 64 && XI == 4, "src item j of a thread is channel wave + 8 j");
+  float bsum[XI];
+#pragma unroll
+  for (int j = 0; j < XI; ++j) bsum[j] = 0.f;
   wg_f32x4 raw[3][NI];
   auto raw_load = [&](const int rs, const int n) __attribute__((always_inline)) {
 #pragma unroll
@@ -997,6 +1234,7 @@
         for (int p = 0; p < SPLIT; ++p) *reinterpret_cast<uint2*>(lds + o + p * APB) = make_uint2(d0[p], d1[p]);
       } else {
         unsigned de[SPLIT], dd[SPLIT];
+        bsum[it - AI] += (v.x + v.y) + (v.z + v.w);
         wg_split_pair<SPLIT>(v.x, v.z, de);
         wg_split_pair<SPLIT>(v.y, v.w, dd);
         const int f = tid + NT * (it - AI);
@@ -1087,11 +1325,21 @@
         atomicAdd(&dwp[((size_t)row * 16 + 2 * wave + (t & 1)) * g.Cpad + il], acc[t][r]);
       }
   }
+  if (dsrcbias != nullptr) {
+#pragma unroll
+    for (int j = 0; j < XI; ++j) {
+      const float v = wave_sum(bsum[j]);
+      if (lane == 0) {
+        if (part) part[(size_t)blockIdx.x * kWgT4bSetFloats + kWgT4bTileFloats + wave + 8 * j] = v;
+        else atomicAdd(&dsrcbias[wave + 8 * j], v);
+      }
+    }
+  }
 }
 
 __device__ __forceinline__ void wgrad_reduce_partials_t4b_body(const float4* __restrict__ part, const int S, const int cpad,
-                                                                        float* __restrict__ dwp, const int bx, const int by) {
-  constexpr int SET4 = kWgT4bSetFloats / 4, NL = 8, NG = 32;
+                                                                        float* __restrict__ dwp, float* __restrict__ dbias, const int bx, const int by) {
+  constexpr int SET4 = kWgT4bSetFloats / 4, TILE4 = kWgT4bTileFloats / 4, NL = 8, NG = 32;
   __shared__ float4 red[NG][NL];
   const int li = threadIdx.x & (NL - 1), sg = threadIdx.x / NL;
   const int f = bx * NL + li;
@@ -1118,6 +1366,11 @@
     float4 v = red[0][li];
 #pragma unroll
     for (int k = 1; k < NG; ++k) { v.x += red[k][li].x; v.y += red[k][li].y; v.z += red[k][li].z; v.w += red[k][li].w; }
+    if (f >= TILE4) {
+      float* const o = dbias + 4 * (f - TILE4);
+      o[0] += v.x; o[1] += v.y; o[2] += v.z; o[3] += v.w;
+      return;
+    }
     const int lane = f & 63, gq = (f >> 6) & 3, t = (f >> 8) & 3, wave = f >> 10, il = lane & 31, kl = lane >> 5;
     const int tap = 2 * wave + (t & 1), row = (t >> 1) * 32 + 8 * gq + 4 * kl;
     float* const o = dwp + ((size_t)row * 16 + tap) * cpad + il;
@@ -1126,8 +1379,8 @@
   }
 }
 __global__ __launch_bounds__(256) void wgrad_reduce_partials_t4b_kernel(const float4* __restrict__ part, const int S, const int cpad,
-                                                                        float* __restrict__ dwp) {
-  wgrad_reduce_partials_t4b_body(part, S, cpad, dwp, (int)blockIdx.x, (int)blockIdx.y);
+                                                                        float* __restrict__ dwp, float* __restrict__ dbias) {
+  wgrad_reduce_partials_t4b_body(part, S, cpad, dwp, dbias, (int)blockIdx.x, (int)blockIdx.y);
 }
 
 constexpr int kWgThinSetFloats = 8 * 64 * 4 + 8;
@@ -1351,7 +1604,8 @@
   wgrad_reduce_partials_thin_body(part, S, cpad, dwp, dbias, (int)blockIdx.x, (int)blockIdx.y);
 }
 
-constexpr int kWgThinTSetFloats = 8 * 2 * 64 * 4;
+constexpr int kWgThinTTileFloats = 8 * 2 * 64 * 4;
+constexpr int kWgThinTSetFloats = kWgThinTTileFloats + 8;
 template <int WO>
 __host__ __device__ constexpr int wgthint_cip() { return (((1024 / WO * 2 + 2) * (2 * WO)) / 16 | 1) * 16; }
 template <int SPLIT, int WO>
@@ -1360,7 +1614,7 @@
 template <int SPLIT, int WO>
 __global__ __launch_bounds__(512, 1) void convt4s2_thin_wgrad_staged_kernel(
     const MtrssmConvGeom g, const float* __restrict__ a, const float* __restrict__ src, const int pre_act_a, float* __restrict__ dwp,
-    float* __restrict__ part, const int frames_per_wg) {
+    float* __restrict__ part, float* __restrict__ dsrcbias, const int frames_per_wg) {
   static_assert(SPLIT == 1 || SPLIT == 2, "one or two bf16 pieces");
   static_assert(WO == 32 || WO == 16, "input plane 32x32 or 64x16");
   constexpr int NT = 512, CO = 16, HO = 1024 / WO, HS = 2 * HO, WS = 2 * WO;
@@ -1390,6 +1644,7 @@
   const float4* const xsrc = reinterpret_cast<const float4*>(src) + tid;
   const float4* const asrc = reinterpret_cast<const float4*>(a) + tid;
   constexpr size_t xfr = (size_t)HS * WS / 4, afr = (size_t)CO * 1024 / 4;
+  float bsum = 0.f;
   wg_f32x4 raw[3][NI];
   auto raw_load = [&](const int rs, const int n) __attribute__((always_inline)) {
 #pragma unroll
@@ -1417,6 +1672,7 @@
         for (int p = 0; p < SPLIT; ++p) *reinterpret_cast<uint2*>(lds + o + p * APB) = make_uint2(d0[p], d1[p]);
       } else {
         unsigned de[SPLIT], dd[SPLIT];
+        bsum += (v.x + v.y) + (v.z + v.w);
         wg_split_pair<SPLIT>(v.x, v.z, de);
         wg_split_pair<SPLIT>(v.y, v.w, dd);
         const int f = tid + NT * (it - AI);
@@ -1488,13 +1744,34 @@
 #pragma unroll
     for (int r = 0; r < 8; ++r) atomicAdd(&dwp[((size_t)((r & 3) + 8 * (r >> 2) + 4 * kl) * 16 + tap) * g.Cpad], acc[r]);
   }
+  if (dsrcbias != nullptr) {
+    const float v = wave_sum(bsum);
+    if (lane == 0) {
+      if (part) part[(size_t)blockIdx.x * kWgThinTSetFloats + kWgThinTTileFloats + wave] = v;
+      else atomicAdd(&dsrcbias[0], v);
+    }
+  }
 }
 
 __device__ __forceinline__ void wgrad_reduce_partials_thint_body(const float4* __restrict__ part, const int S, const int cpad,
-                                                                          float* __restrict__ dwp, const int bx, const int by) {
+                                                                          float* __restrict__ dwp, float* __restrict__ dbias, const int bx, const int by) {
   constexpr int SET4 = kWgThinTSetFloats / 4, NL = 8, NG = 32;
   __shared__ float4 red[NG][NL];
   const int li = threadIdx.x & (NL - 1), sg = threadIdx.x / NL;
+  if (bx >= 16) {
+    const float* const pb = reinterpret_cast<const float*>(part) + kWgThinTTileFloats + li;
+    float t = 0.f;
+    for (int s = sg; s < S; s += NG) t += pb[(size_t)s * kWgThinTSetFloats];
+    red[sg][li].x = t;
+    __syncthreads();
+    if (threadIdx.x == 0) {
+      float v = 0.f;
+      for (int k = 0; k < NG; ++k)
+        for (int w = 0; w < NL; ++w) v += red[k][w].x;
+      dbias[0] += v;
+    }
+    return;
+  }
   const int f = bx * NL + li;
   const float4* const p = part + f;
   float4 acc4[2];
@@ -1528,8 +1805,8 @@
   }
 }
 __global__ __launch_bounds__(256) void wgrad_reduce_partials_thint_kernel(const float4* __restrict__ part, const int S, const int cpad,
-                                                                          float* __restrict__ dwp) {
-  wgrad_reduce_partials_thint_body(part, S, cpad, dwp, (int)blockIdx.x, (int)blockIdx.y);
+                                                                          float* __restrict__ dwp, float* __restrict__ dbias) {
+  wgrad_reduce_partials_thint_body(part, S, cpad, dwp, dbias, (int)blockIdx.x, (int)blockIdx.y);
 }
 
 constexpr int kWgS2cSetFloats = 8 * 4 * 64 * 4 + 32;
```

Result: faster. 370,900 seq-steps/s, median of 6 (+4.3%).
